# olydis/vlg_matching

Hardware: AMD Instinct MI355X
Metric: vlg_queries_per_sec (higher is better)
Workload: dtype u32

## Files before the change

### vlg_matching_amd/csrc/int_index.hpp

```cpp
#pragma once
#include "extract.hpp"
#include "select.hpp"
#include "sweep_kernels.hpp"

namespace {

void bind_int_view(vlg_index* idx)
{
    const uint8_t* b = reinterpret_cast<const uint8_t*>(idx->d_blob);
    const IntHeader& h = idx->ihdr;
    IntView& v = idx->iview;
    v.bv_kind = (uint32_t)h.bv_kind; v.sampling = (uint32_t)h.sampling;
    v.blocks = h.bv_kind == kBvPlain ? reinterpret_cast<const Block*>(b + h.off_levels) : nullptr;
    v.rrr_hdr = h.bv_kind == kBvRrr63 ? reinterpret_cast<const uint4*>(b + h.off_rrr_hdr) : nullptr;
    v.rrr_stream = h.bv_kind == kBvRrr63 ? reinterpret_cast<const uint64_t*>(b + h.off_rrr_stream) : nullptr;
    v.rrr_tables = h.bv_kind == kBvRrr63 ? reinterpret_cast<const RrrTables*>(b + h.off_binom) : nullptr;
    v.stride = h.bv_kind == kBvRrr63 ? h.n_sb : h.nb;
    v.Z = reinterpret_cast<const uint64_t*>(b + h.off_Z);
    v.D = reinterpret_cast<const uint64_t*>(b + h.off_D);
    v.C = reinterpret_cast<const uint64_t*>(b + h.off_C);
    v.comp2char = reinterpret_cast<const uint32_t*>(b + h.off_c2c);
    v.samples = reinterpret_cast<const uint32_t*>(b + h.off_samples);
    v.n = h.n; v.nb = h.nb; v.sigma = h.sigma; v.n_samples = h.n_samples; v.n_levels = h.levels; v.dens = h.dens;
    v.marked = h.sampling == kSamplingTextOrder ? reinterpret_cast<const Block*>(b + h.off_marked) : nullptr;
// ... 336 lines not shown

namespace {

vlg_status int_alloc_blob(vlg_index* idx, uint64_t n, uint64_t sigma, uint32_t dens)
{
    IntHeader& h = idx->ihdr;
    memset(&h, 0, sizeof h);
    h.magic = kIntBlobMagic; h.n = n; h.sigma = sigma; h.dens = dens; h.n_samples = (n + dens - 1) / dens; h.nb = n / kBlockBits + 1;
    h.levels = sigma > 1 ? bit_width64(sigma - 1) : 0;
    if (h.levels > kMaxIntLevels || (uint64_t)h.levels * h.nb >= 0xFFFFFFF0ull) return fail(VLG_E_UNSUPPORTED, "integer index too large for 32-bit block numbers");
    layout_int(h);
    DevBuf blob;
    VLG_HIP_TRY(blob.alloc(h.total_bytes));
    idx->d_blob = blob.take();
    idx->owns_blob = true;
    VLG_HIP_TRY(hipMemset(idx->d_blob, 0, h.total_bytes));
    VLG_HIP_TRY(hipMemcpy(idx->d_blob, &h, sizeof h, hipMemcpyHostToDevice));
    bind_int_view(idx);
    return VLG_OK;
}

vlg_status int_matrix_from_bwt(vlg_index* idx, uint32_t* d_cur, uint32_t* d_other, uint32_t* d_ka, uint32_t* d_kb, DevBuf& tmp)
{
    const IntHeader& h = idx->ihdr;
    const uint64_t n = h.n;
    uint8_t* b = reinterpret_cast<uint8_t*>(idx->d_blob);
    Block* lv = reinterpret_cast<Block*>(b + h.off_levels);
    uint64_t* d_Z = reinterpret_cast<uint64_t*>(b + h.off_Z);
    std::vector<uint64_t> Z(kMaxIntLevels, 0);
    uint32_t* cur = d_cur;
    uint32_t* other = d_other;
    DevBuf d_pops;
    VLG_HIP_TRY(d_pops.alloc((h.nb + 1) * 4));
    for (uint32_t l = 0; l < h.levels; ++l) {
        const uint32_t bit = h.levels - 1 - l;
        if (vlg_status s = wtsa_emit_level(cur, n, bit, lv + (uint64_t)l * h.nb, h.nb, d_pops.as<uint32_t>(), tmp)) return s;
        uint32_t ones = 0;
        VLG_HIP_TRY(hipMemcpy(&ones, d_pops.as<uint32_t>() + h.nb, 4, hipMemcpyDeviceToHost));
        Z[l] = n - ones;
        if (l + 1 < h.levels) {
            hipLaunchKernelGGL(int_bit_keys_kernel, launch_grid(n), dim3(256), 0, nullptr, cur, n, bit, d_ka);
            VLG_HIP_TRY(with_scratch(tmp, [&](void* t, size_t& tb) { return rocprim::radix_sort_pairs(t, tb, d_ka, d_kb, cur, other, n, 0, 1, nullptr); }));
            std::swap(cur, other);
        }
        VLG_HIP_TRY(hipGetLastError());
    }
    VLG_HIP_TRY(hipMemcpy(d_Z, Z.data(), kMaxIntLevels * 8, hipMemcpyHostToDevice));
    hipLaunchKernelGGL(int_D_kernel, launch_grid(h.sigma), dim3(256), 0, nullptr, idx->iview, reinterpret_cast<uint64_t*>(b + h.off_D));
    VLG_HIP_TRY(hipGetLastError());
    VLG_HIP_TRY(hipDeviceSynchronize());
    return VLG_OK;
}

}

extern "C" vlg_status vlg_index_build_int(const uint32_t* h_text, uint64_t n_symbols, uint32_t dens, vlg_index** out)
{
    if (!out || (n_symbols && !h_text)) return fail(VLG_E_INVALID, "null argument");
    *out = nullptr;
    int ndev = 0;
    if (hipGetDeviceCount(&ndev) != hipSuccess || ndev <= 0) return fail(VLG_E_NO_DEVICE, "no HIP device available (the VLG library has no CPU fallback)");
    if (!dens) dens = 32;
    if (n_symbols * 5 >= 0xFFFFFFF0ull) return fail(VLG_E_UNSUPPORTED, "integer text too long for the 32-bit suffix array of this index");
    release_cached_device_memory();
    const uint64_t n = n_symbols + 1;
    IndexPtr idx(new vlg_index());
    DevBuf text, flag, sa, arr_a, arr_b, ka, kb, tmp;
    VLG_HIP_TRY(text.alloc(n_symbols * 4));
    uint32_t* d_text = text.as<uint32_t>();
    if (n_symbols) VLG_HIP_TRY(hipMemcpy(d_text, h_text, n_symbols * 4, hipMemcpyHostToDevice));
    VLG_HIP_TRY(flag.alloc((n_symbols * 5 + 2) * 4));
    VLG_HIP_TRY(hipMemset(flag.p, 0, 4));
    if (n_symbols) hipLaunchKernelGGL(int_zero_check_kernel, launch_grid(n_symbols), dim3(256), 0, nullptr, d_text, n_symbols, flag.as<uint32_t>());
    uint32_t has_zero = 0;
    VLG_HIP_TRY(hipMemcpy(&has_zero, flag.p, 4, hipMemcpyDeviceToHost));
    if (has_zero) return fail(VLG_E_ZERO_BYTE, "the integer text contains the symbol 0 (reserved for the sentinel: construct.hpp:36-45)");
    if (vlg_status s = symbol_suffix_array(d_text, n_symbols, flag, sa)) return s;
    flag.release();
    uint32_t* d_sa = sa.as<uint32_t>();
    VLG_HIP_TRY(arr_a.alloc(n * 4));
    VLG_HIP_TRY(arr_b.alloc(n * 4));
    VLG_HIP_TRY(ka.alloc(n * 4));
    VLG_HIP_TRY(kb.alloc(n * 4));
    uint32_t *d_a = arr_a.as<uint32_t>(), *d_b = arr_b.as<uint32_t>(), *d_ka = ka.as<uint32_t>(), *d_kb = kb.as<uint32_t>();
    size_t sort_tb = 0, scan_tb = 0, pair_tb = 0;
    VLG_HIP_TRY(rocprim::radix_sort_keys(nullptr, sort_tb, d_a, d_b, n, 0, 32, nullptr));
    VLG_HIP_TRY(rocprim::inclusive_scan(nullptr, scan_tb, d_ka, d_kb, n, rocprim::plus<uint32_t>(), nullptr));
    VLG_HIP_TRY(rocprim::radix_sort_pairs(nullptr, pair_tb, d_ka, d_kb, d_a, d_b, n, 0, 1, nullptr));
    VLG_HIP_TRY(tmp.alloc(std::max(std::max(sort_tb, scan_tb), pair_tb)));
    uint64_t sigma = 1;
    if (n_symbols) {
        VLG_HIP_TRY(with_scratch(tmp, [&](void* t, size_t& tb) { return rocprim::radix_sort_keys(t, tb, d_text, d_b, n_symbols, 0, 32, nullptr); }));
        hipLaunchKernelGGL(int_heads_kernel, launch_grid(n_symbols), dim3(256), 0, nullptr, d_b, n_symbols, d_ka);
        VLG_HIP_TRY(with_scratch(tmp, [&](void* t, size_t& tb) { return rocprim::inclusive_scan(t, tb, d_ka, d_kb, n_symbols, rocprim::plus<uint32_t>(), nullptr); }));
        uint32_t distinct = 0;
        VLG_HIP_TRY(hipMemcpy(&distinct, d_kb + (n_symbols - 1), 4, hipMemcpyDeviceToHost));
        sigma = (uint64_t)distinct + 1;
    }
    if (vlg_status s = int_alloc_blob(idx.get(), n, sigma, dens)) return s;
    const IntHeader& h = idx->ihdr;
    uint8_t* b = reinterpret_cast<uint8_t*>(idx->d_blob);
    uint32_t* d_c2c = reinterpret_cast<uint32_t*>(b + h.off_c2c);
    uint64_t* d_C = reinterpret_cast<uint64_t*>(b + h.off_C);
    if (n_symbols) hipLaunchKernelGGL(int_alphabet_kernel, launch_grid(n_symbols), dim3(256), 0, nullptr, d_b, d_kb, n_symbols, d_c2c, d_C);
    VLG_HIP_TRY(hipMemcpy(d_C + sigma, &n, 8, hipMemcpyHostToDevice));
    hipLaunchKernelGGL(int_bwt_kernel, launch_grid(n), dim3(256), 0, nullptr, d_text, d_sa, n, d_c2c, sigma, d_a);
    VLG_HIP_TRY(hipGetLastError());
    if (vlg_status s = int_matrix_from_bwt(idx.get(), d_a, d_b, d_ka, d_kb, tmp)) return s;
    hipLaunchKernelGGL(int_samples_kernel, launch_grid(h.n_samples), dim3(256), 0, nullptr, d_sa, h.n_samples, dens, reinterpret_cast<uint32_t*>(b + h.off_samples));
    VLG_HIP_TRY(hipGetLastError());
    VLG_HIP_TRY(hipDeviceSynchronize());
    *out = idx.release();
    return VLG_OK;
}

extern "C" vlg_status vlg_index_export_int_alphabet(const vlg_index* idx, uint64_t* sigma, uint64_t* h_C, uint64_t* h_comp2char)
{
    if (!idx || !sigma) return fail(VLG_E_INVALID, "null argument");
    if (!idx->is_int) return fail(VLG_E_INVALID, "not an integer-alphabet index");
    *sigma = idx->ihdr.sigma;
    if (h_C) VLG_HIP_TRY(hipMemcpy(h_C, idx->iview.C, (idx->ihdr.sigma + 1) * 8, hipMemcpyDeviceToHost));
    if (h_comp2char) {
        std::vector<uint32_t> t(idx->ihdr.sigma);
        VLG_HIP_TRY(hipMemcpy(t.data(), idx->iview.comp2char, idx->ihdr.sigma * 4, hipMemcpyDeviceToHost));
        for (uint64_t i = 0; i < idx->ihdr.sigma; ++i) h_comp2char[i] = t[i];
    }
    return VLG_OK;
}

extern "C" vlg_status vlg_int_rank_batch(const vlg_index* idx, const uint64_t* d_i, const uint32_t* d_sym, uint64_t* d_out, uint64_t count, void* stream)
{
    if (!idx || (count && (!d_i || !d_sym || !d_out))) return fail(VLG_E_INVALID, "null argument");
    if (!idx->is_int) return fail(VLG_E_INVALID, "not an integer-alphabet index");
    if (!count) return VLG_OK;
    return on_bv(idx->iview.bv_kind, [&](auto bv) {
        return launch(int_rank_kernel<tag_t<decltype(bv)>>, launch_grid(count, 8192), (hipStream_t)stream, idx->iview, d_i, d_sym, d_out, count);
    });
}

namespace vlg {

vlg_status launch_int_backward_search(const IntView& v, const uint8_t* d_blob, const uint64_t* d_off, uint64_t n_pat, uint64_t* d_l, uint64_t* d_r,
                                      unsigned long long* d_stat_levels, hipStream_t st)
{
    if (!n_pat) return VLG_OK;
    return on_bv(v.bv_kind, [&](auto bv) {
        return launch(int_backward_search_kernel<tag_t<decltype(bv)>>, launch_grid(n_pat, 4096), st, v, d_blob, d_off, n_pat, d_l, d_r, d_stat_levels);
    });
}

vlg_status launch_int_locate_sweep(const IntView& v, const uint64_t* d_l, const uint64_t* d_out_off, uint64_t n_pat, uint64_t total, uint32_t* d_out,
                                   uint64_t* val_a, uint64_t* val_b, uint16_t* key_a, uint16_t* key_b, void* temp, size_t temp_bytes, unsigned long long* d_counter,
                                   unsigned long long* d_stats, uint64_t tail_threshold, hipStream_t stream, LaunchTimer* timer, Block* member,
                                   uint32_t n_member_lists, uint64_t* rec, const std::function<vlg_status()>* while_first_step)
{
    const bool text_order = shape(v).text_order;
    if (v.dens == 1 && !text_order && total)
        return sweep_dense_copy(timer, while_first_step, [&] { return launch_int_dense_copy(v, d_l, d_out_off, n_pat, total, d_out, stream); });
    if (!int_sweep_possible(v)) return fail(VLG_E_INTERNAL, "integer index: not for the sorted sweep");
    return on_bv(v.bv_kind, [&](auto bv) { return on_flag(text_order, [&](auto to) {
        const SweepKernels K = bind_sweep<IntWalk<tag_t<decltype(bv)>>, IntSampling<decltype(to)::value>, uint32_t, false>(v, d_l, d_out_off, n_pat, d_stats, stream, nullptr);
        return run_locate_sweep<uint32_t, false>(K, d_l, d_out_off, n_pat, total, d_out, val_a, val_b, key_a, key_b, temp, temp_bytes, d_counter, tail_threshold, stream, timer,
                                                 member, n_member_lists, rec, while_first_step);
    }); });
}

vlg_status launch_int_dense_copy(const IntView& v, const uint64_t* d_l, const uint64_t* d_out_off, uint64_t n_pat, uint64_t total, uint32_t* d_out, hipStream_t stream)
{
    if (v.dens != 1 || v.sampling != kSamplingSaOrder) return fail(VLG_E_INTERNAL, "integer index: the copy needs SA-order samples of density 1");
    return launch_sa_dense_copy(v.samples, d_l, d_out_off, n_pat, total, d_out, stream);
}

vlg_status launch_int_locate(const IntView& v, uint32_t* d_io, uint64_t total, unsigned long long* d_stats, hipStream_t st)
{
    if (!total) return VLG_OK;
    const LocateSlices sl = locate_slices(total);
    return on_bv(v.bv_kind, [&](auto bv) { return on_flag(shape(v).text_order, [&](auto to) {
        return launch(locate_kernel<IntWalk<tag_t<decltype(bv)>>, IntSampling<decltype(to)::value>, uint32_t>, dim3(sl.blocks), st, v, d_io, total, sl.per_wave, d_stats,
                      nullptr, 0u, nullptr, 0ull, nullptr);
    }); });
}

vlg_status launch_int_sa_expand(const IntView& v, uint32_t* d_sa, hipStream_t st)
{
    if (v.sampling != kSamplingSaOrder) return fail(VLG_E_INTERNAL, "integer index: expanding the suffix array needs SA-order samples");
    return on_bv(v.bv_kind, [&](auto bv) { return launch(int_sa_expand_kernel<tag_t<decltype(bv)>>, launch_grid(v.n_samples, 8192), st, v, d_sa); });
}

vlg_status launch_int_isa_samples(const IntView& v, uint32_t inv_dens, uint32_t* d_out, hipStream_t st)
{
    if (v.sampling != kSamplingSaOrder || !inv_dens) return fail(VLG_E_INTERNAL, "integer index: ISA samples need SA-order samples");
    return on_bv(v.bv_kind, [&](auto bv) { return launch(int_isa_samples_kernel<tag_t<decltype(bv)>>, launch_grid(v.n_samples, 8192), st, v, inv_dens, d_out); });
}

vlg_status launch_int_select(const IntView& v, const SelView& sv, const uint64_t* d_arg, const uint32_t* d_sym, uint64_t* d_out, uint64_t count, hipStream_t st)
{
    if (!count) return VLG_OK;
    return on_bv(v.bv_kind, [&](auto bv) { return launch(int_select_kernel<tag_t<decltype(bv)>>, launch_grid(count, 8192), st, v, sv, d_arg, d_sym, d_out, count); });
}
vlg_status launch_int_lf_bwt(const IntView& v, const uint64_t* d_i, uint64_t* d_lf, uint32_t* d_bwt, uint64_t count, hipStream_t st)
{
    if (!count) return VLG_OK;
    return on_bv(v.bv_kind, [&](auto bv) { return launch(int_lf_bwt_kernel<tag_t<decltype(bv)>>, launch_grid(count, 8192), st, v, d_i, d_lf, d_bwt, count); });
}
vlg_status launch_int_extract(const IntView& v, const ExtractJob& job, const uint32_t* d_isa, uint32_t* d_out, hipStream_t st)
{
    return on_bv(v.bv_kind, [&](auto bv) { return launch(int_extract_kernel<tag_t<decltype(bv)>>, launch_grid(job.n_segs, 8192), st, v, job, d_isa, d_out); });
}

vlg_status launch_int_isa(const IntView& v, uint32_t d, const uint32_t* d_isa, const uint64_t* d_i, uint64_t* d_out, uint64_t count,
                          unsigned long long* d_bad, hipStream_t st)
{
    return on_bv(v.bv_kind, [&](auto bv) { return launch(int_isa_kernel<tag_t<decltype(bv)>>, launch_grid(count, 8192), st, v, d, d_isa, d_i, d_out, count, d_bad); });
}

}

namespace {

inline uint32_t int_max_level(uint64_t largest) { return (uint32_t)bit_width64(std::max<uint64_t>(largest, 1)); }

struct TreeScratch {
    DevBuf tree, pay[2], first[2], split, end, pops, bad, tmp;
    uint64_t words = 0, max_nw = 0;
    vlg_status alloc(uint64_t n, uint64_t sigma, uint32_t L)
    {
        words = (n * L + 63) / 64;
        max_nw = n / 64 + 2;
        VLG_HIP_TRY(tree.alloc((words + 1) * 8));
        for (int k = 0; k < 2; ++k) {
            VLG_HIP_TRY(pay[k].alloc(n * 4));
            VLG_HIP_TRY(first[k].alloc(n * 4));
        }
        VLG_HIP_TRY(split.alloc((sigma + 1) * 4));
        VLG_HIP_TRY(end.alloc((sigma + 1) * 4));
        VLG_HIP_TRY(pops.alloc((max_nw + 1) * 4));
        VLG_HIP_TRY(bad.alloc(4));
        VLG_HIP_TRY(hipMemset(bad.p, 0, 4));
        size_t tb = 0;
        VLG_HIP_TRY(rocprim::exclusive_scan(nullptr, tb, pops.as<uint32_t>(), pops.as<uint32_t>(), 0u, max_nw, rocprim::plus<uint32_t>(), nullptr));
        VLG_HIP_TRY(tmp.alloc(tb));
        return VLG_OK;
    }
    vlg_status scan_pops(uint64_t nw)
    {
        uint32_t* p = pops.as<uint32_t>();
        VLG_HIP_TRY(with_scratch(tmp, [&](void* t, size_t& tb) { return rocprim::exclusive_scan(t, tb, p, p, 0u, nw, rocprim::plus<uint32_t>(), nullptr); }));
        return VLG_OK;
    }
};

inline void tree_level_words(uint64_t n, uint32_t l, uint64_t& base, uint64_t& g0, uint64_t& nw)
{
    base = (uint64_t)l * n;
    g0 = base >> 6;
    nw = ((base + n - 1) >> 6) - g0 + 1;
}

vlg_status int_tree_encode(TreeScratch& s, uint64_t n, uint64_t sigma, uint32_t L, const uint32_t* d_c2c, const uint64_t* d_C)
{
    uint64_t* tree = s.tree.as<uint64_t>();
    uint32_t *pops = s.pops.as<uint32_t>(), *split = s.split.as<uint32_t>(), *end = s.end.as<uint32_t>(), *bad_flag = s.bad.as<uint32_t>();
    VLG_HIP_TRY(hipMemset(tree, 0, (s.words + 1) * 8));
    VLG_HIP_TRY(hipMemset(s.first[0].p, 0, n * 4));
    int cur = 0;
    for (uint32_t l = 0; l < L; ++l) {
        uint64_t base, g0, nw;
        tree_level_words(n, l, base, g0, nw);
        hipLaunchKernelGGL(int_tree_emit_kernel, launch_grid(nw * 64), dim3(256), 0, nullptr, s.pay[cur].as<uint32_t>(), d_c2c, base, n, L - 1 - l, g0, nw, tree, pops);
        if (l + 1 == L) break;
        if (vlg_status st = s.scan_pops(nw)) return st;
        hipLaunchKernelGGL(int_tree_split_kernel, launch_grid(sigma + 1), dim3(256), 0, nullptr, d_c2c, sigma, L - l, split, end);
        hipLaunchKernelGGL(HIP_KERNEL_NAME(int_tree_step_kernel<false>), launch_grid(n), dim3(256), 0, nullptr, tree, pops, base, g0, n, d_C, split, end,
                           s.pay[cur].as<uint32_t>(), s.first[cur].as<uint32_t>(), s.pay[cur ^ 1].as<uint32_t>(), s.first[cur ^ 1].as<uint32_t>(), bad_flag);
        VLG_HIP_TRY(hipGetLastError());
        cur ^= 1;
    }
    VLG_HIP_TRY(hipGetLastError());
    uint32_t bad = 0;
    VLG_HIP_TRY(hipMemcpy(&bad, bad_flag, 4, hipMemcpyDeviceToHost));
    if (bad) return fail(VLG_E_INTERNAL, "integer index: the level-wise tree does not agree with the alphabet");
    return VLG_OK;
}

vlg_status int_tree_decode(TreeScratch& s, uint64_t n, uint64_t sigma, uint32_t L, const uint32_t* d_c2c, const uint64_t* d_C, int* bwt)
{
    const uint64_t* tree = s.tree.as<uint64_t>();
    uint32_t *pops = s.pops.as<uint32_t>(), *split = s.split.as<uint32_t>(), *end = s.end.as<uint32_t>(), *bad_flag = s.bad.as<uint32_t>();
    hipLaunchKernelGGL(int_iota_kernel, launch_grid(n), dim3(256), 0, nullptr, s.pay[0].as<uint32_t>(), n);
    VLG_HIP_TRY(hipMemset(s.first[0].p, 0, n * 4));
    int cur = 0;
    for (uint32_t l = 0; l < L; ++l) {
        uint64_t base, g0, nw;
        tree_level_words(n, l, base, g0, nw);
        hipLaunchKernelGGL(int_tree_pops_kernel, launch_grid(nw), dim3(256), 0, nullptr, tree, g0, nw, pops);
        if (vlg_status st = s.scan_pops(nw)) return st;
        hipLaunchKernelGGL(int_tree_split_kernel, launch_grid(sigma + 1), dim3(256), 0, nullptr, d_c2c, sigma, L - l, split, end);
        if (l + 1 < L)
            hipLaunchKernelGGL(HIP_KERNEL_NAME(int_tree_step_kernel<false>), launch_grid(n), dim3(256), 0, nullptr, tree, pops, base, g0, n, d_C, split, end,
                               s.pay[cur].as<uint32_t>(), s.first[cur].as<uint32_t>(), s.pay[cur ^ 1].as<uint32_t>(), s.first[cur ^ 1].as<uint32_t>(), bad_flag);
        else
            hipLaunchKernelGGL(HIP_KERNEL_NAME(int_tree_step_kernel<true>), launch_grid(n), dim3(256), 0, nullptr, tree, pops, base, g0, n, d_C, split, end,
                               s.pay[cur].as<uint32_t>(), s.first[cur].as<uint32_t>(), s.pay[cur ^ 1].as<uint32_t>(), (uint32_t*)nullptr, bad_flag);
        VLG_HIP_TRY(hipGetLastError());
        uint32_t bad = 0;
        VLG_HIP_TRY(hipMemcpy(&bad, bad_flag, 4, hipMemcpyDeviceToHost));
        if (bad) return fail(VLG_E_INVALID, "wt_int tree does not agree with the alphabet's C (level " + std::to_string(l) + ")");
        cur ^= 1;
    }
    *bwt = cur;
    return VLG_OK;
}

}

extern "C" vlg_status vlg_index_export_int_tree(const vlg_index* idx, uint32_t* max_level, uint64_t* h_words)
// ... 68 lines not shown
```

### vlg_matching_amd/csrc/kernels.hip

```cpp
#include <algorithm>
#include <cstring>
#include <string.h>
#include <vector>
#include "common.hpp"
#include "kernels.hpp"
#include "sweep_kernels.hpp"
#include "extract.hpp"
#include "select.hpp"
#include <rocprim/rocprim.hpp>

using namespace vlg;

struct vlg_bitvector {
    Block* d_blocks = nullptr;
    uint64_t nbits = 0;
    uint64_t n_blocks = 0;
};

namespace {

__global__ void bv_pack_kernel(const uint64_t* __restrict__ src, uint64_t src_words, uint64_t nbits, Block* __restrict__ blocks,
                               uint64_t n_blocks, uint32_t* __restrict__ pops)
{
    for (uint64_t b = (uint64_t)blockIdx.x * blockDim.x + threadIdx.x; b < n_blocks; b += (uint64_t)gridDim.x * blockDim.x) {
// ... 825 lines not shown
}

template <class BV, typename pos_t, typename out_t>
__global__ void __launch_bounds__(256) isa_samples_kernel(IndexView iv, uint32_t inv_dens, out_t* __restrict__ out)
{
    __shared__ WalkLds<BV> s;
    stage_walk(s, iv);
    const ByteWalk<BV, true> walk{iv, s};
    const pos_t* samples = reinterpret_cast<const pos_t*>(iv.samples);
    for (uint64_t j = (uint64_t)blockIdx.x * blockDim.x + threadIdx.x; j < iv.n_samples; j += (uint64_t)gridDim.x * blockDim.x) {
        uint64_t i = j * iv.dens, v = samples[j];
        do {
            if (v % inv_dens == 0) out[v / inv_dens] = (out_t)i;
            uint32_t c, n_lv = 0;
            i = walk.lf(i, c, n_lv);
            v = v ? v - 1 : iv.n - 1;
        } while (i % iv.dens);
    }
}

template <class BV, bool kWide, typename isa_t>
__global__ void __launch_bounds__(256) extract_kernel(IndexView iv, ExtractJob job, const isa_t* __restrict__ isa, const uint8_t* __restrict__ comp2char,
                                                      uint8_t* __restrict__ out)
{
    __shared__ WalkLds<BV> s;
    __shared__ uint8_t c2c[256];
    c2c[threadIdx.x] = comp2char[threadIdx.x];
    stage_walk(s, iv);
    extract_segments(job, isa, out, ByteWalk<BV, kWide>{iv, s, c2c});
}

template <class BV, bool kWide, typename isa_t>
__global__ void __launch_bounds__(256) isa_kernel(IndexView iv, uint32_t d, const isa_t* __restrict__ isa, const uint64_t* __restrict__ p,
                                                  uint64_t* __restrict__ out, uint64_t count, unsigned long long* __restrict__ bad)
{
    __shared__ WalkLds<BV> s;
    stage_walk(s, iv);
    isa_queries(p, out, count, iv.n, d, isa, ByteWalk<BV, kWide>{iv, s}, bad);
}

__global__ void comp2char_kernel(const uint8_t* __restrict__ char2comp, uint8_t* __restrict__ c2c)
{
    const uint32_t ch = threadIdx.x, c = char2comp[ch];
    if (ch == 0 || c != 0) c2c[c] = (uint8_t)ch;
}

__global__ void extract_check_kernel(const uint64_t* __restrict__ begin, const uint64_t* __restrict__ end, const uint64_t* __restrict__ out_off,
                                     uint64_t n_ranges, uint64_t n, uint64_t total, uint32_t d, uint64_t* __restrict__ seg,
                                     unsigned long long* __restrict__ bad)
{
    for (uint64_t r = (uint64_t)blockIdx.x * blockDim.x + threadIdx.x; r <= n_ranges; r += (uint64_t)gridDim.x * blockDim.x) {
        if (r == n_ranges) { seg[r] = 0; continue; }
        const uint64_t b = begin[r], e = end[r], o = out_off[r];
        const bool ok = b <= e && e < n && o <= total && e - b + 1 <= total - o;
        seg[r] = ok ? e / d - b / d + 1 : 0;
        if (!ok) atomicAdd(bad, 1ull);
    }
}

template <typename pos_t>
__global__ void widen_kernel(const pos_t* __restrict__ in, uint64_t* __restrict__ out, uint64_t count)
{
    for (uint64_t j = (uint64_t)blockIdx.x * blockDim.x + threadIdx.x; j < count; j += (uint64_t)gridDim.x * blockDim.x) out[j] = in[j];
}
template <typename pos_t>
__global__ void narrow_kernel(const uint64_t* __restrict__ in, pos_t* __restrict__ out, uint64_t count)
{
    for (uint64_t j = (uint64_t)blockIdx.x * blockDim.x + threadIdx.x; j < count; j += (uint64_t)gridDim.x * blockDim.x) out[j] = (pos_t)in[j];
}

template <bool kWide, bool kTextOrder>
using ByteSampling = typename std::conditional<kTextOrder, TextOrderSampling<typename std::conditional<kWide, uint64_t, uint32_t>::type>,
                                               SaOrderSampling<typename std::conditional<kWide, uint64_t, uint32_t>::type>>::type;

}

namespace vlg {

vlg_status launch_backward_search(const IndexView& iv, const uint8_t* d_blob, const uint64_t* d_off, uint64_t n_pat, uint64_t* d_l,
                                  uint64_t* d_r, unsigned long long* d_stat_levels, hipStream_t stream)
{
    if (!n_pat) return VLG_OK;
    return on_bv(iv.bv_kind, [&](auto bv) {
        return launch(backward_search_kernel<tag_t<decltype(bv)>>, launch_grid(n_pat, 4096), stream, iv, d_blob, d_off, n_pat, d_l, d_r, d_stat_levels);
    });
}

vlg_status launch_branching_search(const IndexView& iv, bool budget, const uint8_t* d_masks, const uint64_t* d_task, uint64_t n_tasks, uint32_t cap,
                                   uint64_t* d_frontier, uint32_t* d_count, unsigned long long* d_stat_levels, hipStream_t stream)
{
    if (!n_tasks) return VLG_OK;
    if (!cap || cap > kClassIntervalsMax) return fail(VLG_E_INTERNAL, std::string(budget ? "approximate" : "class") + " search: frontier cap out of range");
    const dim3 grid((uint32_t)std::min<uint64_t>((n_tasks + 3) / 4, 16384));
    return on_bv(iv.bv_kind, [&](auto bv) {
        const auto go = [&](auto kernel) {
            return launch(kernel, grid, stream, iv, d_masks, d_task, n_tasks, cap, reinterpret_cast<ulonglong2*>(d_frontier), d_count, d_stat_levels);
        };
        return budget ? go(branching_search_kernel<tag_t<decltype(bv)>, true>) : go(branching_search_kernel<tag_t<decltype(bv)>, false>);
    });
}

template <typename pos_t>
vlg_status launch_expand(const uint64_t* d_l, const uint64_t* d_out_off, uint64_t n_pat, uint64_t total, pos_t* d_io, uint32_t* d_seg,
                         hipStream_t stream)
{
    if (!total) return VLG_OK;
    hipLaunchKernelGGL(HIP_KERNEL_NAME(expand_kernel<pos_t>), launch_grid(total, 32768), dim3(256), 0, stream, d_l, d_out_off, n_pat,
                       total, d_io, d_seg);
    VLG_HIP_TRY(hipGetLastError());
    return VLG_OK;
}
template vlg_status launch_expand<uint32_t>(const uint64_t*, const uint64_t*, uint64_t, uint64_t, uint32_t*, uint32_t*, hipStream_t);
template vlg_status launch_expand<uint64_t>(const uint64_t*, const uint64_t*, uint64_t, uint64_t, uint64_t*, uint32_t*, hipStream_t);

template <typename pos_t>
vlg_status launch_locate(const IndexView& iv, pos_t* d_io, uint64_t total, unsigned long long* d_stats, hipStream_t stream)
{
    if (!total) return VLG_OK;
    const LocateSlices sl = locate_slices(total);
    if (iv.sample_bytes != sizeof(pos_t)) return fail(VLG_E_INTERNAL, "locate: sample width does not match the instantiation");
    constexpr bool kWide = sizeof(pos_t) == 8;
    return on_byte_walk<kWide>(iv, [&](auto walk) { return on_flag(shape(iv).text_order, [&](auto to) {
        return launch(locate_kernel<tag_t<decltype(walk)>, ByteSampling<kWide, decltype(to)::value>, pos_t, false, kWide>, dim3(sl.blocks), stream, iv, d_io,
                      total, sl.per_wave, d_stats, nullptr, 0u, nullptr, 0ull, nullptr);
    }); });
}
template vlg_status launch_locate<uint32_t>(const IndexView&, uint32_t*, uint64_t, unsigned long long*, hipStream_t);
template vlg_status launch_locate<uint64_t>(const IndexView&, uint64_t*, uint64_t, unsigned long long*, hipStream_t);


size_t sweep_temp_bytes(uint64_t total, uint32_t sigma, hipStream_t stream)
{
    size_t tb = 0;
    rocprim::double_buffer<uint16_t> k(nullptr, nullptr);
    rocprim::double_buffer<uint64_t> v(nullptr, nullptr);
    (void)rocprim::radix_sort_pairs(nullptr, tb, k, v, total, 0, bit_width64(sigma), stream);
    return tb;
}

void launch_sweep_chunk_lists(const uint64_t* d_out_off, uint64_t n_pat, uint64_t t0, uint64_t t1, uint32_t* chunk_list, hipStream_t stream)
{
    const uint64_t chunks = (t1 - t0 + kSweepChunk - 1) / kSweepChunk;
    if (!chunks) return;
    hipLaunchKernelGGL(sweep_chunk_lists_kernel, dim3((uint32_t)((chunks + 255) / 256)), dim3(256), 0, stream, d_out_off, n_pat, t0, t1, chunk_list);
}

template <typename pos_t, bool kWide>
vlg_status run_locate_sweep(const SweepKernels& K, const uint64_t* d_l, const uint64_t* d_out_off, uint64_t n_pat, uint64_t total,
                            pos_t* d_out, uint64_t* val_a, uint64_t* val_b, uint16_t* key_a, uint16_t* key_b, void* temp,
                            size_t temp_bytes, unsigned long long* d_counter, uint64_t tail_threshold,
                            hipStream_t stream, LaunchTimer* timer, Block* member ,
                            uint32_t n_member_lists ,
                            uint64_t* rec ,
                            const std::function<vlg_status()>* while_first_step )
{
    bool hook_due = while_first_step != nullptr;
    constexpr uint32_t kShift = kWide ? 33 : 32;
    if (K.n > (1ull << kShift)) return fail(VLG_E_UNSUPPORTED, "sorted sweep: text too long for the packed position");
    if (sizeof(pos_t) == 4 && K.n > (1ull << 32) + 1) return fail(VLG_E_INTERNAL, "sorted sweep: positions do not fit 32 bits");
    if (K.sigma >= 0xFFFFu) return fail(VLG_E_INTERNAL, "sorted sweep: alphabet too large for the 16-bit partition key");
    const unsigned bits = bit_width64(K.sigma);
    const uint64_t batch_max = sweep_batch_max<kWide>();
    if (member) {
        if (total > 0xFFFFFF00ull) return fail(VLG_E_INTERNAL, "member bit-vector: slots need 32 bits");
        if (timer) timer->begin(0);
        hipLaunchKernelGGL(member_build_kernel, launch_grid(member_blocks(K.n), 16384), dim3(256), 0, stream, d_l, d_out_off, n_member_lists,
                           member_blocks(K.n), member);
        if (timer) timer->end(0);
        VLG_HIP_TRY(hipGetLastError());
        if (total > batch_max) VLG_HIP_TRY(hipMemsetAsync(rec, 0xFF, total * 8, stream));
    }
    bool front_valid = K.front != nullptr && [] { const char* e = getenv("VLG_RESOLVE_GROUPED"); return !(e && e[0] == '0'); }();
    for (uint64_t t0 = 0; t0 < total; t0 += batch_max) {
        const uint64_t t1 = std::min(total, t0 + batch_max);
        const bool fused_first = t1 - t0 > tail_threshold;
        if (!fused_first) front_valid = false;
        static const bool ahead = [] { const char* e = getenv("VLG_SWEEP_LOOKAHEAD"); return !(e && e[0] == '0'); }();
        if (!fused_first) {
            if (member) VLG_HIP_TRY(hipMemsetAsync(rec + t0, 0xFF, (t1 - t0) * 8, stream));
            hipLaunchKernelGGL(HIP_KERNEL_NAME(sweep_init_kernel<kShift>), launch_grid((t1 - t0 + 7) / 8, 32768), dim3(256), 0, stream, d_l, d_out_off, n_pat,
                               t0, t1, val_a);
        }
        VLG_HIP_TRY(hipGetLastError());
        uint64_t alive = t1 - t0;
        uint32_t step = 0;
        pos_t* out = d_out + t0;
        while (alive > tail_threshold && step < 0xFFFFFFu) {
            VLG_HIP_TRY(hipMemsetAsync(d_counter, 0, 8, stream));
            if (timer) timer->begin(0);
            const vlg_status ks = fused_first && step == 0 ? K.first(t0, t1, val_a, key_a, out, d_counter, member, rec, ahead, reinterpret_cast<uint32_t*>(val_b))
                                                           : K.step(val_a, key_a, alive, step, out, d_counter, member, rec, t0, ahead && fused_first && step == 1);
            if (timer) timer->end(0);
            if (ks) return ks;
            size_t tb = temp_bytes;
            if (timer) timer->begin(1, 20ull * alive);
            rocprim::double_buffer<uint16_t> dk(key_a, key_b);
            rocprim::double_buffer<uint64_t> dv(val_a, val_b);
            hipError_t se = rocprim::radix_sort_pairs(temp, tb, dk, dv, alive, 0, bits, stream);
            if (timer) timer->end(1);
            VLG_HIP_TRY(se);
            unsigned long long done = 0;
            VLG_HIP_TRY(hipMemcpyAsync(&done, d_counter, 8, hipMemcpyDeviceToHost, stream));
            if (hook_due) { hook_due = false; if (vlg_status hs = (*while_first_step)()) return hs; }
            VLG_HIP_TRY(hipStreamSynchronize(stream));
            key_a = dk.current(); key_b = dk.alternate();
            val_a = dv.current(); val_b = dv.alternate();
            alive -= done;
            ++step;
            if (step > 1u << 20) return fail(VLG_E_INTERNAL, "locate sweep did not converge");
        }
        if (alive) {
            const LocateSlices sl = locate_slices(alive);
            if (timer) timer->begin(0);
            const vlg_status ks = K.tail(out, alive, sl.per_wave, val_a, step, member ? rec : nullptr, t0, member, sl.blocks);
            if (timer) timer->end(0);
            if (ks) return ks;
        }
    }
    if (hook_due) { hook_due = false; if (vlg_status hs = (*while_first_step)()) return hs; }
    if (member) {
        static const bool diag = [] { const char* e = getenv("VLG_RESOLVE_STATS"); return e && e[0] == '1'; }();
        for (uint32_t round = 0;; ++round) {
            VLG_HIP_TRY(hipMemsetAsync(d_counter, 0, diag ? 32 : 8, stream));
            if (timer) timer->begin(2, round == 0 ? total * (8ull + sizeof(pos_t)) : 0);
            if (round == 0 && front_valid && !diag)
                hipLaunchKernelGGL(HIP_KERNEL_NAME(trail_resolve_grouped_kernel<pos_t, kWide>), dim3((uint32_t)std::min<uint64_t>((total + kGroupChunk - 1) / kGroupChunk, 1u << 20)),
                                   dim3(256), 0, stream, rec, total, d_out, K.front, d_counter);
            else
                hipLaunchKernelGGL(HIP_KERNEL_NAME(trail_resolve_kernel<pos_t, kWide>), dim3((uint32_t)std::min<uint64_t>((total + kResolveChunk - 1) / kResolveChunk, 65536)),
                                   dim3(256), 0, stream, rec, total, d_out, d_counter, round, diag);
            if (timer) timer->end(2);
            VLG_HIP_TRY(hipGetLastError());
            unsigned long long open = 0;
            VLG_HIP_TRY(hipMemcpyAsync(&open, d_counter, 8, hipMemcpyDeviceToHost, stream));
            VLG_HIP_TRY(hipStreamSynchronize(stream));
            if (diag) {
                unsigned long long c[4] = {0, 0, 0, 0};
                VLG_HIP_TRY(hipMemcpy(c, d_counter, 32, hipMemcpyDeviceToHost));
                fprintf(stderr, "[vlg resolve] round %u: %llu records, %llu pointers, %llu hops, %llu distinct lines (per wave-wide hop), %llu still open\n", round,
                        (unsigned long long)total, c[3], c[1], c[2], c[0]);
            }
            if (!open) break;
            if (round > 64) return fail(VLG_E_INTERNAL, "trail records did not resolve");
        }
    }
    return VLG_OK;
}
template vlg_status run_locate_sweep<uint32_t, false>(const SweepKernels&, const uint64_t*, const uint64_t*, uint64_t, uint64_t, uint32_t*, uint64_t*, uint64_t*,
                                                      uint16_t*, uint16_t*, void*, size_t, unsigned long long*, uint64_t, hipStream_t, LaunchTimer*, Block*,
                                                      uint32_t, uint64_t*, const std::function<vlg_status()>*);

template <typename pos_t, bool kWide>
vlg_status launch_locate_sweep(const IndexView& iv, const uint64_t* d_l, const uint64_t* d_out_off, uint64_t n_pat, uint64_t total,
                               pos_t* d_out, uint64_t* val_a, uint64_t* val_b, uint16_t* key_a, uint16_t* key_b, void* temp,
                               size_t temp_bytes, unsigned long long* d_counter, unsigned long long* d_stats, uint64_t tail_threshold,
                               hipStream_t stream, LaunchTimer* timer, Block* member, uint32_t n_member_lists, uint64_t* rec,
                               const std::function<vlg_status()>* while_first_step, uint8_t* front)
{
    if (iv.sample_bytes != (kWide ? 8u : 4u)) return fail(VLG_E_INTERNAL, "sorted sweep: sample width does not match the instantiation");
    const bool text_order = shape(iv).text_order;
    if (iv.dens == 1 && !text_order && total) {
        using sample_t = typename std::conditional<kWide, uint64_t, uint32_t>::type;
        return sweep_dense_copy(timer, while_first_step, [&] {
            return launch(sa_dense_copy_kernel<pos_t, sample_t>, launch_grid((total + 7) / 8, 32768), stream, reinterpret_cast<const sample_t*>(iv.samples), d_l, d_out_off,
                          n_pat, total, d_out);
        });
    }
    return on_byte_walk<kWide>(iv, [&](auto walk) { return on_flag(text_order, [&](auto to) {
        const SweepKernels K = bind_sweep<tag_t<decltype(walk)>, ByteSampling<kWide, decltype(to)::value>, pos_t, kWide>(iv, d_l, d_out_off, n_pat, d_stats, stream,
                                                                                                                   rec ? front : nullptr);
        return run_locate_sweep<pos_t, kWide>(K, d_l, d_out_off, n_pat, total, d_out, val_a, val_b, key_a, key_b, temp, temp_bytes, d_counter, tail_threshold, stream, timer,
                                              member, n_member_lists, rec, while_first_step);
    }); });
}
constexpr uint32_t kUnsampleSync = 4;
template <bool kWide>
vlg_status launch_unsample(const IndexView& iv, const uint64_t* d_l, const uint64_t* d_out_off, uint64_t n_pat, uint64_t total, uint32_t* d_out,
                           uint32_t* sa_full, uint64_t* val_a, uint64_t* val_b, uint16_t* key_a, uint16_t* key_b, void* temp, size_t temp_bytes,
                           unsigned long long* d_counter, unsigned long long* h_done , unsigned long long* d_stats, uint64_t tail_threshold,
                           hipStream_t stream, LaunchTimer* timer, const std::function<vlg_status()>* while_first_step)
{
    bool hook_due = while_first_step != nullptr;
    if (iv.sampling != kSamplingSaOrder || iv.dens < 2) return fail(VLG_E_INTERNAL, "unsampling needs SA-order samples of density >= 2");
    if (iv.sample_bytes != (kWide ? 8u : 4u)) return fail(VLG_E_INTERNAL, "unsampling: sample width does not match the instantiation");
    if (iv.n > (1ull << 32) + 1 || (!kWide && iv.n > (1ull << 32))) return fail(VLG_E_UNSUPPORTED, "unsampling: text too long for 32-bit positions");
    if (iv.sigma >= 0x7FFFu) return fail(VLG_E_INTERNAL, "unsampling: alphabet too large for the key");
    const unsigned bits = bit_width64(iv.sigma);
    uint64_t alive = iv.n_samples, done_total = 0;
    const auto step_round = [&](bool first) {
        if (timer) timer->begin(0);
        const vlg_status ks = on_bv(iv.bv_kind, [&](auto bv) { return on_flag(first, [&](auto f) {
            return launch(unsample_step_kernel<tag_t<decltype(bv)>, kWide, decltype(f)::value>, launch_grid(alive, 8192), stream, iv, val_a, key_a, alive, sa_full, d_stats,
                          d_counter);
        }); });
        if (timer) timer->end(0);
        return ks;
    };
    VLG_HIP_TRY(hipMemsetAsync(d_counter, 0, 8, stream));
    uint32_t round = 0;
    while (alive > tail_threshold) {
        for (uint32_t r = 0; r < kUnsampleSync; ++r, ++round) {
            if (vlg_status ks = step_round(round == 0)) return ks;
            size_t tb = temp_bytes;
            if (timer) timer->begin(1, 20ull * alive);
            rocprim::double_buffer<uint16_t> dk(key_a, key_b);
            rocprim::double_buffer<uint64_t> dv(val_a, val_b);
            const hipError_t se = rocprim::radix_sort_pairs(temp, tb, dk, dv, alive, 0, bits, stream);
            if (timer) timer->end(1);
            VLG_HIP_TRY(se);
            key_a = dk.current(); key_b = dk.alternate();
            val_a = dv.current(); val_b = dv.alternate();
            if (hook_due) { hook_due = false; if (vlg_status hs = (*while_first_step)()) return hs; }
        }
        VLG_HIP_TRY(hipMemcpyAsync(h_done, d_counter, 8, hipMemcpyDeviceToHost, stream));
        VLG_HIP_TRY(hipStreamSynchronize(stream));
        done_total = *h_done;
        if (done_total > iv.n_samples) return fail(VLG_E_INTERNAL, "unsampling: more walkers arrived than were started");
        alive = iv.n_samples - done_total;
        if (round > (1u << 20)) return fail(VLG_E_INTERNAL, "unsampling did not converge");
    }
    if (round == 0 && iv.n_samples) {
        if (vlg_status ks = step_round(true)) return ks;
        ++round;
    }
    if (hook_due) { hook_due = false; if (vlg_status hs = (*while_first_step)()) return hs; }
    if (alive || round == 1) {
        const uint64_t span = round == 1 ? iv.n_samples : alive;
        const LocateSlices sl = locate_slices(span, 64 * 4);
        if (timer) timer->begin(0);
        const vlg_status ks = on_bv(iv.bv_kind, [&](auto bv) {
            return launch(unsample_tail_kernel<tag_t<decltype(bv)>, kWide>, dim3(sl.blocks), stream, iv, val_a, key_a, span, sl.per_wave, sa_full, d_stats);
        });
        if (timer) timer->end(0);
        if (ks) return ks;
    }
    if (total) {
        if (timer) timer->begin(0);
        const vlg_status ks = launch_sa_dense_copy(sa_full, d_l, d_out_off, n_pat, total, d_out, stream);
        if (timer) timer->end(0);
        if (ks) return ks;
    }
    return VLG_OK;
}
template vlg_status launch_unsample<false>(const IndexView&, const uint64_t*, const uint64_t*, uint64_t, uint64_t, uint32_t*, uint32_t*, uint64_t*, uint64_t*,
                                           uint16_t*, uint16_t*, void*, size_t, unsigned long long*, unsigned long long*, unsigned long long*, uint64_t, hipStream_t,
                                           LaunchTimer*, const std::function<vlg_status()>*);
template vlg_status launch_unsample<true>(const IndexView&, const uint64_t*, const uint64_t*, uint64_t, uint64_t, uint32_t*, uint32_t*, uint64_t*, uint64_t*,
                                          uint16_t*, uint16_t*, void*, size_t, unsigned long long*, unsigned long long*, unsigned long long*, uint64_t, hipStream_t,
                                          LaunchTimer*, const std::function<vlg_status()>*);

vlg_status launch_sa_dense_copy(const uint32_t* sa, const uint64_t* d_l, const uint64_t* d_out_off, uint64_t n_pat, uint64_t total, uint32_t* d_out,
                                hipStream_t stream)
{
    if (!total) return VLG_OK;
    return launch(sa_dense_copy_kernel<uint32_t, uint32_t>, launch_grid((total + 7) / 8, 32768), stream, sa, d_l, d_out_off, n_pat, total, d_out);
}

#define VLG_SWEEP_INST(P, W)                                                                                                          \
    template vlg_status launch_locate_sweep<P, W>(const IndexView&, const uint64_t*, const uint64_t*, uint64_t, uint64_t, P*, uint64_t*, \
                                                  uint64_t*, uint16_t*, uint16_t*, void*, size_t, unsigned long long*, unsigned long long*, \
                                                  uint64_t, hipStream_t, LaunchTimer*, Block*, uint32_t, uint64_t*,                       \
                                                  const std::function<vlg_status()>*, uint8_t*);
VLG_SWEEP_INST(uint32_t, false)
VLG_SWEEP_INST(uint32_t, true)
VLG_SWEEP_INST(uint64_t, true)
#undef VLG_SWEEP_INST

template <typename T>
vlg_status launch_narrow(const uint64_t* d_in, T* d_out, uint64_t count, hipStream_t stream)
{
    if (!count) return VLG_OK;
    return launch(narrow_kernel<T>, launch_grid(count), stream, d_in, d_out, count);
}
template vlg_status launch_narrow<uint32_t>(const uint64_t*, uint32_t*, uint64_t, hipStream_t);
template <typename T>
vlg_status launch_widen(const T* d_in, uint64_t* d_out, uint64_t count, hipStream_t stream)
{
    if (!count) return VLG_OK;
    return launch(widen_kernel<T>, launch_grid(count), stream, d_in, d_out, count);
}
template vlg_status launch_widen<uint32_t>(const uint32_t*, uint64_t*, uint64_t, hipStream_t);

KernelConstants kernel_constants()
{
    return KernelConstants{VLG_RESOLVE_HOPS, VLG_RESOLVE_CHUNK, VLG_GROUP_CHUNK, VLG_STAGE_LISTS, VLG_SWEEP_PAIRS};
}

}

extern "C" vlg_status vlg_wt_rank_batch(const vlg_index* idx, const uint64_t* d_i, const uint8_t* d_c, uint64_t* d_out, uint64_t count,
                                        void* stream)
{
    if (!idx || (count && (!d_i || !d_c || !d_out))) return fail(VLG_E_INVALID, "null argument");
    if (idx->is_int) return fail(VLG_E_INVALID, "integer-alphabet index: use vlg_int_rank_batch");
    if (!count) return VLG_OK;
    return on_bv(idx->view.bv_kind, [&](auto bv) {
        return launch(wt_rank_kernel<tag_t<decltype(bv)>>, launch_grid(count, 8192), (hipStream_t)stream, idx->view, d_i, d_c, d_out, count);
    });
}

extern "C" vlg_status vlg_backward_search_batch(const vlg_index* idx, const uint8_t* d_blob, const uint64_t* d_off, uint64_t n_patterns,
                                                uint64_t* d_l, uint64_t* d_r, void* stream)
{
    if (!idx || (n_patterns && (!d_off || !d_l || !d_r))) return fail(VLG_E_INVALID, "null argument");
    if (idx->is_int) return launch_int_backward_search(idx->iview, d_blob, d_off, n_patterns, d_l, d_r, nullptr, (hipStream_t)stream);
    return launch_backward_search(idx->view, d_blob, d_off, n_patterns, d_l, d_r, nullptr, (hipStream_t)stream);
}

namespace {
template <class Fill>
vlg_status locate_narrow(const vlg_index* idx, uint64_t count, uint64_t* d_out, hipStream_t st, const Fill& fill)
{
    DevBuf tmp_buf;
    VLG_HIP_TRY(tmp_buf.alloc(count * 4));
    uint32_t* tmp = tmp_buf.as<uint32_t>();
    vlg_status s = fill(tmp);
    if (!s) s = idx->is_int ? launch_int_locate(idx->iview, tmp, count, nullptr, st) : launch_locate<uint32_t>(idx->view, tmp, count, nullptr, st);
    if (!s) s = launch_widen<uint32_t>(tmp, d_out, count, st);
    const hipError_t e = hipStreamSynchronize(st);
    if (s) return s;
    VLG_HIP_TRY(e);
    return VLG_OK;
}
}

extern "C" vlg_status vlg_sa_batch(const vlg_index* idx, const uint64_t* d_i, uint64_t* d_out, uint64_t count, void* stream)
{
    if (!idx || (count && (!d_i || !d_out))) return fail(VLG_E_INVALID, "null argument");
    if (!count) return VLG_OK;
    hipStream_t st = (hipStream_t)stream;
    if (idx->hdr.sample_bytes == 8) {
        if (d_out != d_i) VLG_HIP_TRY(hipMemcpyAsync(d_out, d_i, count * 8, hipMemcpyDeviceToDevice, st));
        return launch_locate<uint64_t>(idx->view, d_out, count, nullptr, st);
    }
    return locate_narrow(idx, count, d_out, st, [&](uint32_t* tmp) { return launch_narrow<uint32_t>(d_i, tmp, count, st); });
}

extern "C" vlg_status vlg_locate_batch(const vlg_index* idx, const uint64_t* d_l, const uint64_t* d_r, const uint64_t* d_out_off,
                                       uint64_t n_patterns, uint64_t total, uint64_t* d_out, void* stream)
{
    (void)d_r;
    if (!idx || (n_patterns && (!d_l || !d_out_off)) || (total && !d_out)) return fail(VLG_E_INVALID, "null argument");
    if (!total) return VLG_OK;
    hipStream_t st = (hipStream_t)stream;
    if (idx->hdr.sample_bytes == 8) {
        if (vlg_status s = launch_expand<uint64_t>(d_l, d_out_off, n_patterns, total, d_out, nullptr, st)) return s;
        return launch_locate<uint64_t>(idx->view, d_out, total, nullptr, st);
    }
    return locate_narrow(idx, total, d_out, st, [&](uint32_t* tmp) { return launch_expand<uint32_t>(d_l, d_out_off, n_patterns, total, tmp, nullptr, st); });
}

namespace {
vlg_status isa_samples_device(const vlg_index* idx, uint32_t inv_dens, void* d_out, hipStream_t st)
{
    const uint64_t n = idx->hdr.n;
    if (idx->hdr.sampling != kSamplingSaOrder) return fail(VLG_E_UNSUPPORTED, "ISA samples are computed from an SA-order index");
    const uint64_t count = (n - 1) / inv_dens + 1;
    const uint32_t w = isa_sample_bytes(n);
    VLG_HIP_TRY(hipMemsetAsync(d_out, 0, count * w, st));
    if (idx->is_int)
        return launch_int_isa_samples(idx->iview, inv_dens, (uint32_t*)d_out, st);
    const IndexView& iv = idx->view;
    return on_bv(iv.bv_kind, [&](auto bv) { return on_isa_samples_shape(shape(iv).wide, w, [&](auto pos, auto out) {
        using out_t = tag_t<decltype(out)>;
        return launch(isa_samples_kernel<tag_t<decltype(bv)>, tag_t<decltype(pos)>, out_t>, launch_grid(iv.n_samples, 8192), st, iv, inv_dens, (out_t*)d_out);
    }); });
}
}

extern "C" vlg_status vlg_index_isa_samples(const vlg_index* idx, uint32_t inv_dens, uint64_t* h_out, uint64_t count)
{
    if (!idx || !h_out || !inv_dens) return fail(VLG_E_INVALID, "null argument");
    const uint64_t n = idx->hdr.n;
    if (count != (n - 1) / inv_dens + 1) return fail(VLG_E_INVALID, "ISA sample count must be (n-1)/inv_dens + 1");
    if (idx->hdr.sampling != kSamplingSaOrder) return fail(VLG_E_UNSUPPORTED, "ISA samples are computed from an SA-order index");
    const uint32_t w = isa_sample_bytes(n);
    DevBuf out_buf;
    VLG_HIP_TRY(out_buf.alloc(count * (8 + w)));
    uint64_t* d_out = out_buf.as<uint64_t>();
    void* d_smp = d_out + count;
    vlg_status s = isa_samples_device(idx, inv_dens, d_smp, nullptr);
    if (!s) s = w == 8 ? (hipMemcpyAsync(d_out, d_smp, count * 8, hipMemcpyDeviceToDevice, nullptr) == hipSuccess ? VLG_OK : VLG_E_NO_DEVICE)
                       : launch_widen<uint32_t>((const uint32_t*)d_smp, d_out, count, nullptr);
    hipError_t e = s ? hipSuccess : hipMemcpy(h_out, d_out, count * 8, hipMemcpyDeviceToHost);
    if (s) return s == VLG_E_NO_DEVICE ? fail(s, "ISA samples: device copy failed") : s;
    VLG_HIP_TRY(e);
    return VLG_OK;
}

extern "C" vlg_status vlg_text_access_create(const vlg_index* idx, uint32_t inv_dens, void* stream, vlg_text_access** out)
{
    if (!idx || !out) return fail(VLG_E_INVALID, "null argument");
    *out = nullptr;
    if (idx->hdr.sampling != kSamplingSaOrder)
        return fail(VLG_E_UNSUPPORTED, "text access needs an SA-order index (a text-order index derives its ISA through the marks)");
    const uint32_t d = inv_dens ? inv_dens : 64;
    hipStream_t st = (hipStream_t)stream;
    vlg_text_access* t = new (std::nothrow) vlg_text_access;
    if (!t) return fail(VLG_E_OOM, "text access handle");
    t->idx = idx;
    t->d = d;
    t->isa_bytes = isa_sample_bytes(idx->hdr.n);
    const uint64_t count = (idx->hdr.n - 1) / d + 1;
    vlg_status s = VLG_OK;
    if (hipMalloc(&t->d_isa, count * t->isa_bytes) != hipSuccess) { t->d_isa = nullptr; s = fail(VLG_E_OOM, "text access: ISA samples"); }
    if (!s) s = isa_samples_device(idx, d, t->d_isa, st);
    if (!s && !idx->is_int) {
        if (hipMalloc((void**)&t->d_c2c, 256) != hipSuccess) { t->d_c2c = nullptr; s = fail(VLG_E_OOM, "text access: comp2char"); }
        else if (hipMemsetAsync(t->d_c2c, 0, 256, st) != hipSuccess) s = fail(VLG_E_NO_DEVICE, "text access: comp2char");
        else hipLaunchKernelGGL(comp2char_kernel, dim3(1), dim3(256), 0, st, idx->view.char2comp, t->d_c2c);
    }
    if (!s) {
        hipError_t e = hipGetLastError();
        if (e == hipSuccess) e = hipStreamSynchronize(st);
        if (e != hipSuccess) s = fail(VLG_E_NO_DEVICE, std::string("text access: ") + hipGetErrorString(e));
    }
    if (s) { vlg_text_access_destroy(t); return s; }
    *out = t;
    return VLG_OK;
}

extern "C" void vlg_text_access_destroy(vlg_text_access* t)
{
    if (!t) return;
    if (t->d_isa) (void)hipFree(t->d_isa);
    if (t->d_c2c) (void)hipFree(t->d_c2c);
    delete t;
}

extern "C" vlg_status vlg_extract_batch(const vlg_text_access* t, const uint64_t* d_begin, const uint64_t* d_end, const uint64_t* d_out_off,
                                        uint64_t n_ranges, uint64_t total, void* d_out, void* stream)
{
    if (!t || (n_ranges && (!d_begin || !d_end || !d_out_off || !d_out))) return fail(VLG_E_INVALID, "null argument");
    if (!n_ranges) return VLG_OK;
    const vlg_index* idx = t->idx;
    hipStream_t st = (hipStream_t)stream;
    size_t tb = 0;
    uint64_t* seg = nullptr;
// ... 478 lines not shown
```

### vlg_matching_amd/csrc/kernels.hpp

```cpp
#pragma once
#include <algorithm>
#include <functional>
#include "common.hpp"

namespace vlg {

vlg_status launch_backward_search(const IndexView& iv, const uint8_t* d_blob, const uint64_t* d_off, uint64_t n_pat, uint64_t* d_l,
                                  uint64_t* d_r, unsigned long long* d_stat_levels, hipStream_t stream);
constexpr uint32_t kClassIntervalsMax = 1u << 20;
constexpr uint32_t kClassSearchOverflow = 0xFFFFFFFFu;
vlg_status launch_branching_search(const IndexView& iv, bool budget, const uint8_t* d_masks, const uint64_t* d_task, uint64_t n_tasks, uint32_t cap,
                                   uint64_t* d_frontier, uint32_t* d_count, unsigned long long* d_stat_levels, hipStream_t stream);
template <typename pos_t>
vlg_status launch_expand(const uint64_t* d_l, const uint64_t* d_out_off, uint64_t n_pat, uint64_t total, pos_t* d_io, uint32_t* d_seg,
                         hipStream_t stream);
template <typename pos_t>
vlg_status launch_locate(const IndexView& iv, pos_t* d_io, uint64_t total, unsigned long long* d_stats, hipStream_t stream);

struct KernelConstants { int64_t resolve_hops, resolve_chunk, group_chunk, stage_lists, sweep_pairs; };
KernelConstants kernel_constants();

struct LaunchTimer {
    virtual ~LaunchTimer() {}
    virtual void begin(int which, uint64_t algorithmic_bytes = 0) = 0;
    virtual void end(int which) = 0;
};

struct LocateSlices { uint32_t per_wave, blocks; };
inline LocateSlices locate_slices(uint64_t count, uint64_t min_per_wave = 64 * 16)
{
    const uint64_t target_waves = 256ull * 32 * 4;
    const uint64_t per_wave = std::min<uint64_t>(std::max<uint64_t>((count + target_waves - 1) / target_waves, min_per_wave), 1u << 20);
    const uint64_t waves = (count + per_wave - 1) / per_wave;
    return LocateSlices{(uint32_t)per_wave, (uint32_t)((waves + 3) / 4)};
}

size_t sweep_temp_bytes(uint64_t total, uint32_t sigma, hipStream_t stream);
template <bool kWide> constexpr uint64_t sweep_batch_max() { return kWide ? (1ull << 31) : 0xFFFFFF00ull; }
template <typename pos_t, bool kWide>
vlg_status launch_locate_sweep(const IndexView& iv, const uint64_t* d_l, const uint64_t* d_out_off, uint64_t n_pat, uint64_t total,
                               pos_t* d_out, uint64_t* val_a, uint64_t* val_b, uint16_t* key_a, uint16_t* key_b, void* temp,
                               size_t temp_bytes, unsigned long long* d_counter, unsigned long long* d_stats, uint64_t tail_threshold,
                               hipStream_t stream, LaunchTimer* timer, Block* member, uint32_t n_member_lists, uint64_t* rec,
                               const std::function<vlg_status()>* while_first_step = nullptr,
                               uint8_t* front = nullptr );
constexpr uint32_t kSweepChunk = 2048;
void launch_sweep_chunk_lists(const uint64_t* d_out_off, uint64_t n_pat, uint64_t t0, uint64_t t1, uint32_t* chunk_list, hipStream_t stream);
struct SweepKernels {
    uint8_t* front = nullptr;
    uint64_t n = 0;
    uint32_t sigma = 0;
    std::function<vlg_status(uint64_t t0, uint64_t t1, uint64_t* val, uint16_t* key, void* out, unsigned long long* n_done, const Block* member, uint64_t* rec, bool ahead,
                       uint32_t* chunk_list )> first;
    std::function<vlg_status(uint64_t* val, uint16_t* key, uint64_t alive, uint32_t step, void* out, unsigned long long* n_done, const Block* member, uint64_t* rec, uint64_t t0,
                       bool probed)> step;
    std::function<vlg_status(void* out, uint64_t alive, uint32_t per_wave, const uint64_t* val, uint32_t step, uint64_t* rec_or_null, uint64_t t0, const Block* member,
                       uint32_t blocks)> tail;
};
template <typename pos_t, bool kWide>
vlg_status run_locate_sweep(const SweepKernels& K, const uint64_t* d_l, const uint64_t* d_out_off, uint64_t n_pat, uint64_t total,
                            pos_t* d_out, uint64_t* val_a, uint64_t* val_b, uint16_t* key_a, uint16_t* key_b, void* temp,
                            size_t temp_bytes, unsigned long long* d_counter, uint64_t tail_threshold, hipStream_t stream, LaunchTimer* timer,
                            Block* member, uint32_t n_member_lists, uint64_t* rec, const std::function<vlg_status()>* while_first_step = nullptr);
inline uint64_t member_blocks(uint64_t n) { return n / kBlockBits + 1; }
template <bool kWide>
vlg_status launch_unsample(const IndexView& iv, const uint64_t* d_l, const uint64_t* d_out_off, uint64_t n_pat, uint64_t total, uint32_t* d_out,
                           uint32_t* sa_full, uint64_t* val_a, uint64_t* val_b, uint16_t* key_a, uint16_t* key_b, void* temp, size_t temp_bytes,
                           unsigned long long* d_counter, unsigned long long* h_done , unsigned long long* d_stats, uint64_t tail_threshold,
                           hipStream_t stream, LaunchTimer* timer, const std::function<vlg_status()>* while_first_step = nullptr);
template <typename T> vlg_status launch_narrow(const uint64_t* d_in, T* d_out, uint64_t count, hipStream_t stream);
template <typename T> vlg_status launch_widen(const T* d_in, uint64_t* d_out, uint64_t count, hipStream_t stream);

vlg_status launch_int_backward_search(const IntView& v, const uint8_t* d_blob, const uint64_t* d_off, uint64_t n_pat, uint64_t* d_l, uint64_t* d_r,
                                      unsigned long long* d_stat_levels, hipStream_t st);
vlg_status launch_int_locate(const IntView& v, uint32_t* d_io, uint64_t total, unsigned long long* d_stats, hipStream_t st);
vlg_status launch_int_locate_sweep(const IntView& v, const uint64_t* d_l, const uint64_t* d_out_off, uint64_t n_pat, uint64_t total, uint32_t* d_out,
                                   uint64_t* val_a, uint64_t* val_b, uint16_t* key_a, uint16_t* key_b, void* temp, size_t temp_bytes, unsigned long long* d_counter,
                                   unsigned long long* d_stats, uint64_t tail_threshold, hipStream_t stream, LaunchTimer* timer, Block* member,
                                   uint32_t n_member_lists, uint64_t* rec, const std::function<vlg_status()>* while_first_step = nullptr);
vlg_status launch_sa_dense_copy(const uint32_t* sa, const uint64_t* d_l, const uint64_t* d_out_off, uint64_t n_pat, uint64_t total, uint32_t* d_out,
                                hipStream_t stream);
vlg_status launch_int_dense_copy(const IntView& v, const uint64_t* d_l, const uint64_t* d_out_off, uint64_t n_pat, uint64_t total, uint32_t* d_out, hipStream_t stream);
vlg_status launch_int_sa_expand(const IntView& v, uint32_t* d_sa, hipStream_t st);
vlg_status launch_int_isa_samples(const IntView& v, uint32_t inv_dens, uint32_t* d_out, hipStream_t st);
struct ExtractJob;
vlg_status launch_int_extract(const IntView& v, const ExtractJob& job, const uint32_t* d_isa, uint32_t* d_out, hipStream_t st);
vlg_status launch_int_isa(const IntView& v, uint32_t d, const uint32_t* d_isa, const uint64_t* d_i, uint64_t* d_out, uint64_t count,
                          unsigned long long* d_bad, hipStream_t st);
struct SelView;
vlg_status launch_int_select(const IntView& v, const SelView& sv, const uint64_t* d_arg, const uint32_t* d_sym, uint64_t* d_out, uint64_t count, hipStream_t st);
vlg_status launch_int_lf_bwt(const IntView& v, const uint64_t* d_i, uint64_t* d_lf, uint32_t* d_bwt, uint64_t count, hipStream_t st);
inline bool int_sweep_possible(const IntView& v) { return v.sigma < 0xFFFFu && v.n_levels >= 1 && v.n <= (1ull << 32); }

}
```

### vlg_matching_amd/csrc/search.hip

```cpp
#include <algorithm>
#include <chrono>
#include <cstdio>
#include <cstdlib>
#include <cstring>
#include <mutex>
#include <numeric>
#include <thread>
#include <unordered_map>
#include <string.h>
#include <string>
#include <vector>
#include "common.hpp"
#include "kernels.hpp"
#include <rocprim/rocprim.hpp>

using namespace vlg;

#include "search_types.hpp"
#include "filter_shape.hpp"
#include "window_cut.hpp"
#include "shape_dispatch.hpp"

enum { KS_BSEARCH = 0, KS_EXPAND, KS_LOCATE, KS_LOCATE_PART, KS_LOCATE_RESOLVE, KS_SORT, KS_FILTER_LADDER, KS_FILTER_PIVOT, KS_FILTER_PASS, KS_FILTER_COMPACT,
       KS_JOIN_INIT, KS_JOIN_LINK, KS_JOIN_SCAN, KS_JOIN_CHAIN, KS_GATHER, KS_EXCHANGE, KS_WINDOW_CUT, KS_CLASS_SEARCH, KS_COUNT };
static const char* kKernelNames[KS_COUNT] = {"backward_search", "expand", "locate", "locate_partition", "locate_resolve", "sort", "filter_ladder", "filter_pivot",
                                             "filter_pass", "filter_compact", "join_init", "join_link", "join_scan", "join_chain", "gather", "exchange", "window_cut", "class_search"};

struct vlg_workspace {
    hipStream_t stream = nullptr;
    uint64_t cap_bytes = 0;
    uint8_t* arena = nullptr;
    uint64_t arena_bytes = 0;
    HostPool host;
    bool profile = false;
    bool dedup = true;
    bool sweep = true;
    bool tuples = true;
    bool trail = true;
    bool filter = true;
    uint64_t filter_min = 1ull << 12;
    uint64_t filter_stream_min = 1ull << 16;
    bool filter_pivot = true;
    uint64_t filter_group_bytes = 0;
    uint64_t filter_pivot_ratio = 3;
    uint64_t pivot_range_ratio = 16;
    uint32_t compact_dense_min = 256;
    uint32_t pivot_rungs = 1;
    int list_sort = 1;
    uint64_t global_sort_min = 1ull << 20;
    bool quad_walk = true;
    bool fuse_jump = true;
    uint64_t sweep_min = 1ull << 22;
    uint64_t sweep_tail = 1ull << 22;
    uint32_t unsample_pct = 0;
    uint64_t unsample_min = 1ull << 28;
    uint64_t unsample_tail = 1ull << 20;
    uint32_t class_intervals = 1024;
    uint64_t sample_reads = 0;
    uint8_t* head = nullptr;
    uint64_t head_bytes = 0;
    uint64_t tmp_key[6] = {0, 0, 0, 0, 0, 0};
    size_t tmp_bytes = 0;
    int x_ranks = 1, x_rank = 0;
    vlg_exchange_fn x_fn = nullptr;
    vlg_alltoall_fn x_a2a = nullptr;
    void* x_ctx = nullptr;
    void* x_comm = nullptr;
    bool exchange_all = false;
    uint64_t* x_status = nullptr;
    uint32_t x_agreed = 0;
    vlg_kernel_stat stats[KS_COUNT];
    std::vector<std::pair<hipEvent_t, hipEvent_t>> pending[KS_COUNT];
    std::vector<hipEvent_t> free_events;
};

namespace {

struct PhaseTrace {
    bool on, sync;
    hipStream_t st;
    std::chrono::steady_clock::time_point t0;
    explicit PhaseTrace(hipStream_t s) : on(getenv("VLG_TRACE") != nullptr), sync(!on || strcmp(getenv("VLG_TRACE"), "host") != 0), st(s), t0(std::chrono::steady_clock::now()) {}
    void mark(const char* what)
    {
        if (!on) return;
        if (sync) (void)hipStreamSynchronize(st);
        const auto t1 = std::chrono::steady_clock::now();
        fprintf(stderr, "[vlg trace] %-28s %9.3f ms\n", what, std::chrono::duration<double, std::milli>(t1 - t0).count());
        t0 = t1;
    }
};

hipEvent_t ws_event(vlg_workspace* ws)
{
    if (!ws->free_events.empty()) { hipEvent_t e = ws->free_events.back(); ws->free_events.pop_back(); return e; }
    hipEvent_t e;
    if (hipEventCreate(&e) != hipSuccess) return nullptr;
    return e;
}

struct Timed {
    vlg_workspace* ws; int k; hipEvent_t a = nullptr, b = nullptr;
    Timed(vlg_workspace* w, int kernel, uint64_t alg_bytes) : ws(w), k(kernel)
    {
        ws->stats[k].launches++;
        ws->stats[k].algorithmic_bytes += alg_bytes;
        if (ws->profile) { a = ws_event(ws); b = ws_event(ws); if (a) (void)hipEventRecord(a, ws->stream); }
    }
    ~Timed() { if (a && b) { (void)hipEventRecord(b, ws->stream); ws->pending[k].emplace_back(a, b); } }
};

struct SweepTimer : LaunchTimer {
    vlg_workspace* ws; hipEvent_t a = nullptr, b = nullptr;
    explicit SweepTimer(vlg_workspace* w) : ws(w) {}
    void begin(int which, uint64_t algorithmic_bytes) override
    {
        int k = which == 0 ? KS_LOCATE : (which == 1 ? KS_LOCATE_PART : KS_LOCATE_RESOLVE);
        ws->stats[k].launches++;
        ws->stats[k].algorithmic_bytes += algorithmic_bytes;
        a = b = nullptr;
        if (ws->profile) { a = ws_event(ws); b = ws_event(ws); if (a) (void)hipEventRecord(a, ws->stream); }
    }
    void end(int which) override
    {
        int k = which == 0 ? KS_LOCATE : (which == 1 ? KS_LOCATE_PART : KS_LOCATE_RESOLVE);
        if (a && b) { (void)hipEventRecord(b, ws->stream); ws->pending[k].emplace_back(a, b); }
    }
};

void ws_collect(vlg_workspace* ws)
{
    for (int k = 0; k < KS_COUNT; ++k) {
        for (auto& pr : ws->pending[k]) {
            float ms = 0;
            (void)hipEventSynchronize(pr.second);
            if (hipEventElapsedTime(&ms, pr.first, pr.second) == hipSuccess) ws->stats[k].total_ms += ms;
            ws->free_events.push_back(pr.first);
            ws->free_events.push_back(pr.second);
        }
        ws->pending[k].clear();
    }
}

void ws_reset_stats(vlg_workspace* ws)
{
    ws_collect(ws);
    for (int k = 0; k < KS_COUNT; ++k) {
        memset(&ws->stats[k], 0, sizeof(vlg_kernel_stat));
        strncpy(ws->stats[k].name, kKernelNames[k], sizeof(ws->stats[k].name) - 1);
    }
}

void drain_result_cache();

vlg_status ws_head(vlg_workspace* ws, uint64_t bytes, uint8_t** out)
{
    if (bytes > ws->head_bytes) {
        if (ws->head) { (void)hipFree(ws->head); ws->head = nullptr; ws->head_bytes = 0; }
        const uint64_t want = align_up(bytes + bytes / 4, 1 << 20);
        VLG_HIP_TRY(hipMalloc((void**)&ws->head, want));
        ws->head_bytes = want;
    }
    *out = ws->head;
    return VLG_OK;
}

vlg_status ws_reserve(vlg_workspace* ws, uint64_t bytes)
{
    if (bytes <= ws->arena_bytes) return VLG_OK;
    if (ws->arena) { (void)hipFree(ws->arena); ws->arena = nullptr; ws->arena_bytes = 0; }
    if (hipMalloc((void**)&ws->arena, bytes) != hipSuccess) {
        (void)hipGetLastError();
        ws->arena = nullptr;
        drain_result_cache();
        VLG_HIP_TRY(hipMalloc((void**)&ws->arena, bytes));
    }
    ws->arena_bytes = bytes;
    return VLG_OK;
}

}

extern "C" vlg_status vlg_workspace_create(uint64_t max_hbm_bytes, void* stream, vlg_workspace** out)
{
    if (!out) return fail(VLG_E_INVALID, "null argument");
    *out = nullptr;
    int ndev = 0;
    if (hipGetDeviceCount(&ndev) != hipSuccess || ndev <= 0) return fail(VLG_E_NO_DEVICE, "no HIP device available");
    vlg_workspace* ws = new vlg_workspace();
    ws->stream = (hipStream_t)stream;
    ws->cap_bytes = max_hbm_bytes ? max_hbm_bytes : (8ull << 30);
    ws_reset_stats(ws);
    *out = ws;
    return VLG_OK;
}

extern "C" void vlg_workspace_destroy(vlg_workspace* ws)
{
    if (!ws) return;
    ws_collect(ws);
    for (hipEvent_t e : ws->free_events) (void)hipEventDestroy(e);
    if (ws->arena) (void)hipFree(ws->arena);
    if (ws->head) (void)hipFree(ws->head);
    if (ws->x_status) (void)hipFree(ws->x_status);
    ws->host.release();
    delete ws;
}

extern "C" vlg_status vlg_workspace_profile(vlg_workspace* ws, int enable)
{
    if (!ws) return fail(VLG_E_INVALID, "null argument");
    ws_reset_stats(ws);
    ws->profile = enable != 0;
    return VLG_OK;
}

extern "C" vlg_status vlg_workspace_set_option(vlg_workspace* ws, const char* name, int64_t value)
{
    if (!ws || !name) return fail(VLG_E_INVALID, "null argument");
    if (!strcmp(name, "dedup")) { ws->dedup = value != 0; return VLG_OK; }
    if (!strcmp(name, "sweep")) { ws->sweep = value != 0; return VLG_OK; }
    if (!strcmp(name, "sweep_min")) { ws->sweep_min = (uint64_t)value; return VLG_OK; }
    if (!strcmp(name, "global_sort_min")) { ws->global_sort_min = (uint64_t)value; return VLG_OK; }
    if (!strcmp(name, "list_sort")) { ws->list_sort = value > 2 ? 1 : (int)value; return VLG_OK; }
    if (!strcmp(name, "trail")) { ws->trail = value != 0; return VLG_OK; }
    if (!strcmp(name, "quad_walk")) { ws->quad_walk = value != 0; return VLG_OK; }
    if (!strcmp(name, "tuples")) { ws->tuples = value != 0; return VLG_OK; }
    if (!strcmp(name, "fuse_jump")) { ws->fuse_jump = value != 0; return VLG_OK; }
    if (!strcmp(name, "filter")) { ws->filter = value != 0; return VLG_OK; }
    if (!strcmp(name, "filter_min")) { ws->filter_min = (uint64_t)value; return VLG_OK; }
    if (!strcmp(name, "filter_pivot")) { ws->filter_pivot = value != 0; return VLG_OK; }
    if (!strcmp(name, "filter_pivot_ratio")) { ws->filter_pivot_ratio = (uint64_t)value; return VLG_OK; }
    if (!strcmp(name, "pivot_range_ratio")) { ws->pivot_range_ratio = (uint64_t)std::max<int64_t>(0, value); return VLG_OK; }
    if (!strcmp(name, "compact_dense_min")) { ws->compact_dense_min = (uint32_t)std::max<int64_t>(0, std::min<int64_t>(value, 1 << 20)); return VLG_OK; }
    if (!strcmp(name, "pivot_rungs")) { ws->pivot_rungs = value <= 0 ? 0u : (value == 1 ? 1u : 2u); return VLG_OK; }
    if (!strcmp(name, "filter_stream_min")) { ws->filter_stream_min = (uint64_t)value; return VLG_OK; }
    if (!strcmp(name, "filter_group_bytes")) { ws->filter_group_bytes = (uint64_t)value; return VLG_OK; }
    if (!strcmp(name, "reserve")) {
        const uint64_t b = std::min<uint64_t>((uint64_t)value, ws->cap_bytes);
        return ws_reserve(ws, b + b / 96 + (256ull << 20));
    }
    if (!strcmp(name, "sweep_tail")) { ws->sweep_tail = (uint64_t)value; return VLG_OK; }
    if (!strcmp(name, "exchange_all")) { ws->exchange_all = value != 0; return VLG_OK; }
    if (!strcmp(name, "unsample_pct")) { ws->unsample_pct = (uint32_t)std::max<int64_t>(0, std::min<int64_t>(value, 1 << 20)); return VLG_OK; }
    if (!strcmp(name, "unsample_tail")) { ws->unsample_tail = (uint64_t)value; return VLG_OK; }
    if (!strcmp(name, "class_intervals")) {
        if (value < 1 || value > (int64_t)kClassIntervalsMax) return fail(VLG_E_INVALID, "class_intervals: 1 .. 2^20");
        ws->class_intervals = (uint32_t)value;
        return VLG_OK;
    }
    if (!strcmp(name, "unsample_min")) { ws->unsample_min = (uint64_t)value; return VLG_OK; }
    return fail(VLG_E_INVALID, std::string("unknown workspace option ") + name);
}

namespace {
vlg_status ws_exchange_reset(vlg_workspace* ws, int n_ranks)
{
    ws->x_comm = nullptr; ws->x_fn = nullptr; ws->x_a2a = nullptr; ws->x_ctx = nullptr; ws->x_ranks = 1; ws->x_rank = 0;
    if (n_ranks > 1 && !ws->x_status) VLG_HIP_TRY(hipMalloc((void**)&ws->x_status, 8 * 1024));
    return VLG_OK;
}
}

extern "C" vlg_status vlg_workspace_set_comm(vlg_workspace* ws, void* nccl_comm)
{
    if (!ws) return fail(VLG_E_INVALID, "null argument");
    if (vlg_status s = ws_exchange_reset(ws, 1)) return s;
    if (!nccl_comm) return VLG_OK;
    int n = 0, r = 0;
    if (vlg_status s = vlg_comm_info(nccl_comm, &n, &r)) return s;
    if (n > 1024) return fail(VLG_E_UNSUPPORTED, "more than 1024 ranks");
    if (vlg_status s = ws_exchange_reset(ws, n)) return s;
    ws->x_comm = nccl_comm; ws->x_ranks = n; ws->x_rank = r;
    return VLG_OK;
}

extern "C" vlg_status vlg_workspace_set_exchange(vlg_workspace* ws, int n_ranks, int rank, vlg_exchange_fn fn, void* ctx)
{
    if (!ws || n_ranks < 1 || n_ranks > 1024 || rank < 0 || rank >= n_ranks || (n_ranks > 1 && !fn)) return fail(VLG_E_INVALID, "bad exchange arguments");
    if (vlg_status s = ws_exchange_reset(ws, n_ranks)) return s;
    ws->x_fn = n_ranks > 1 ? fn : nullptr; ws->x_ctx = ctx; ws->x_ranks = n_ranks; ws->x_rank = rank;
    return VLG_OK;
}

extern "C" vlg_status vlg_workspace_set_exchange_alltoall(vlg_workspace* ws, int n_ranks, int rank, vlg_alltoall_fn fn, void* ctx)
{
    if (!ws || n_ranks < 1 || n_ranks > 1024 || rank < 0 || rank >= n_ranks || (n_ranks > 1 && !fn)) return fail(VLG_E_INVALID, "bad exchange arguments");
    if (vlg_status s = ws_exchange_reset(ws, n_ranks)) return s;
    ws->x_a2a = n_ranks > 1 ? fn : nullptr; ws->x_ctx = ctx; ws->x_ranks = n_ranks; ws->x_rank = rank;
    return VLG_OK;
}

extern "C" vlg_status vlg_workspace_kernel_stats(vlg_workspace* ws, vlg_kernel_stat* out, uint32_t cap, uint32_t* n)
{
    if (!ws || !n) return fail(VLG_E_INVALID, "null argument");
    ws_collect(ws);
    *n = KS_COUNT;
    for (uint32_t k = 0; k < KS_COUNT && k < cap && out; ++k) out[k] = ws->stats[k];
    return VLG_OK;
}

struct ResultPiece {
    uint64_t q0 = 0, q1 = 0;
    uint64_t matches = 0, tuple_vals = 0;
    void* d_first = nullptr;
    void* d_tuples = nullptr;
    uint32_t width = 8;
    uint64_t first_bytes = 0, tuple_bytes = 0;
};

struct vlg_result {
    vlg_result_summary sum;
    std::vector<uint64_t> counts;
    std::vector<uint32_t> k;
    std::vector<ResultPiece> pieces;
    std::vector<uint64_t> owned;
    std::vector<uint64_t> civ_off, civ_l, civ_r;
    bool has_class_intervals = false;
    std::vector<uint64_t> next;
    bool has_next = false;
};

namespace {
constexpr uint64_t kResultCacheBytes = 48ull << 30;
struct ResultCache {
    struct Entry { void* p; uint64_t size; int device; };
    std::mutex mu;
    std::vector<Entry> free_list;
    uint64_t bytes = 0;
    static int device() { int d = 0; (void)hipGetDevice(&d); return d; }
    void* take(uint64_t need, uint64_t* size)
    {
        const int dev = device();
        std::lock_guard<std::mutex> g(mu);
        size_t best = free_list.size();
        for (size_t i = 0; i < free_list.size(); ++i)
            if (free_list[i].device == dev && free_list[i].size >= need && free_list[i].size <= need + need / 4 + (1u << 20) &&
                (best == free_list.size() || free_list[i].size < free_list[best].size)) best = i;
        if (best == free_list.size()) return nullptr;
        void* p = free_list[best].p;
        *size = free_list[best].size;
        bytes -= free_list[best].size;
        free_list.erase(free_list.begin() + best);
        return p;
    }
    void give(void* p, uint64_t size)
    {
        {
            const int dev = device();
            std::lock_guard<std::mutex> g(mu);
            if (bytes + size <= kResultCacheBytes && free_list.size() < 64) { free_list.push_back(Entry{p, size, dev}); bytes += size; return; }
        }
        (void)hipFree(p);
    }
    void drain()
    {
        std::lock_guard<std::mutex> g(mu);
        for (auto& e : free_list) (void)hipFree(e.p);
        free_list.clear();
        bytes = 0;
    }
};
ResultCache& result_cache() { static ResultCache* c = new ResultCache(); return *c; }
void drain_result_cache() { result_cache().drain(); }

hipError_t result_alloc(void** out, uint64_t bytes, uint64_t* got)
{
    if (void* p = result_cache().take(bytes, got)) { *out = p; return hipSuccess; }
    hipError_t e = hipMalloc(out, bytes);
    if (e != hipSuccess) {
        (void)hipGetLastError();
        result_cache().drain();
        e = hipMalloc(out, bytes);
    }
    *got = bytes;
    return e;
}
}

namespace vlg {
void release_cached_device_memory() { result_cache().drain(); }
// ... 361 lines not shown
{
    constexpr uint32_t kPer = 8;
    __shared__ uint64_t s_first;
    for (uint64_t b0 = (uint64_t)blockIdx.x * 256 * kPer; b0 < total; b0 += (uint64_t)gridDim.x * 256 * kPer) {
        __syncthreads();
        if (threadIdx.x == 0) {
            uint64_t lo = 0, hi = n_seg;
            while (hi - lo > 1) { const uint64_t mid = (lo + hi) >> 1; if (dst_off[mid] <= b0) lo = mid; else hi = mid; }
            s_first = lo;
        }
        __syncthreads();
        uint64_t k = s_first;
#pragma unroll
        for (uint32_t i = 0; i < kPer; ++i) {
            const uint64_t t = b0 + i * 256 + threadIdx.x;
            if (t < total) {
                while (dst_off[k + 1] <= t) ++k;
                const uint64_t at = src_off[k] + (t - dst_off[k]);
                if (kGather) packed[t] = base[at]; else base[at] = packed[t];
            }
        }
    }
}

struct PhysChoice {
    uint32_t locate = VLG_LOCATE_WALKS;
    bool sweep = false;
    bool share_steps = false;
    bool list_sort = false;
    bool global_sort = false;
    unsigned pos_bits = 1;
};

template <typename pos_t>
PhysChoice choose_physical(const vlg_index* idx, const vlg_workspace* ws, uint64_t elems, uint64_t n_lists, bool wide, uint64_t unsample_elems,
                           uint64_t scratch_elems, const PhysChoice* sized)
{
    const BlobHeader& h = idx->hdr;
    const bool dense = h.dens == 1 && h.sampling == kSamplingSaOrder;
    PhysChoice c;
    c.pos_bits = std::max(1u, bit_width64(h.n >= 2 ? h.n - 2 : 0));
    c.sweep = ws->sweep && elems >= ws->sweep_min && h.n <= (1ull << (wide ? 33 : 32)) &&
              (!idx->is_int || (int_sweep_possible(idx->iview) && sizeof(pos_t) == 4 && !wide));
    const uint64_t n_walkers = idx->is_int ? 0 : idx->view.n_samples;
    const bool unsample = c.sweep && sizeof(pos_t) == 4 && ws->unsample_pct && ws->trail && ws->dedup && !idx->is_int && h.sampling == kSamplingSaOrder &&
                          h.dens >= 2 && h.n <= (1ull << 32) + 1 && h.sigma < 0x7FFFu && unsample_elems >= ws->sweep_min && unsample_elems >= ws->unsample_min &&
                          (__uint128_t)unsample_elems * 100 >= (__uint128_t)h.n * ws->unsample_pct &&
                          (!scratch_elems || align_up(h.n * 4, 256) + n_walkers * 20 + 1024 <= scratch_elems * kPhysScratchPerElem<pos_t>()) &&
                          (!sized || sized->locate == VLG_LOCATE_UNSAMPLE);
    c.locate = !c.sweep ? (idx->is_int && dense ? VLG_LOCATE_COPY : VLG_LOCATE_WALKS) : unsample ? VLG_LOCATE_UNSAMPLE : dense ? VLG_LOCATE_COPY : VLG_LOCATE_SWEEP;
    c.share_steps = c.sweep && !unsample && ws->trail && ws->dedup && !dense && elems <= 0xFFFFFF00ull && (!sized || sized->share_steps);
    c.list_sort = sizeof(pos_t) == 4 && ws->list_sort;
    c.global_sort = elems >= ws->global_sort_min && c.pos_bits + bit_width64(n_lists) <= 64;
    return c;
}

template <typename pos_t, typename word_t>
vlg_status expand_and_walk(vlg_workspace* ws, const IndexView& lview, const uint64_t* d_l, const uint64_t* d_off, uint64_t n_lists, uint64_t total, word_t* io,
                           pos_t* out, unsigned long long* d_stats)
{
    {
        Timed t(ws, KS_EXPAND, 0);
        if (vlg_status s = launch_expand<word_t>(d_l, d_off, n_lists, total, io, nullptr, ws->stream)) return s;
    }
    Timed t(ws, KS_LOCATE, 0);
    if (vlg_status s = launch_locate<word_t>(lview, io, total, d_stats, ws->stream)) return s;
    if constexpr (sizeof(word_t) != sizeof(pos_t)) return launch_narrow<pos_t>(io, out, total, ws->stream);
    return VLG_OK;
}

struct SuperChunk {
    uint64_t Q0 = 0, Q1 = 0, phys = 0;
    std::vector<uint32_t> dlist;
};

struct ChunkPlan {
    PhysChoice c;
    size_t sort_tmp = 0;
    bool want_rungs = false;
    uint64_t phys_bytes = 0, join_budget = 0;
    bool launch_first = false;
};

template <typename pos_t>
struct PhysicalPass {
    const vlg_index* idx; vlg_workspace* ws; vlg_result* res; const Plan& pl; const ChunkPlan& cp; bool wide; Arena& A;
    unsigned long long* d_stats; Lists<pos_t>& L;
    hipStream_t st = ws->stream;
    PhaseTrace bt{st};
    std::vector<uint32_t> dlist, cut;
    std::vector<uint64_t> xcounts;
    uint32_t gnd = 0, n_outer = 0, sl = 0, nd = 0;
    uint64_t gacc = 0, acc = 0;
    svec<uint64_t> goff64, off64, lh; svec<uint32_t> off32;
    PhysChoice c;
    pos_t* Pg = nullptr; pos_t* Pa = nullptr; pos_t* Pb = nullptr; uint8_t* scratch = nullptr; void* d_tmp = nullptr;
    uint64_t* d_goff64 = nullptr; uint64_t* d_off64 = nullptr; uint32_t* d_off32 = nullptr; uint64_t* d_lh = nullptr; unsigned long long* d_counter = nullptr;
    uint64_t* rec = nullptr; Block* member = nullptr; uint8_t* front = nullptr;
    uint64_t sort_mark = 0; ListSortPlan lsp;
    bool pairwise = false;

    void layout(const std::vector<uint32_t>& dlist_in)
    {
        gnd = (uint32_t)dlist_in.size();
        dlist = dlist_in;
        bool ascending = true;
        for (uint32_t i = 1; i < gnd && ascending; ++i) ascending = pl.dl[dlist[i - 1]] <= pl.dl[dlist[i]];
        if (!ascending)
            std::sort(dlist.begin(), dlist.end(), [&](uint32_t a, uint32_t b) { return pl.dl[a] != pl.dl[b] ? pl.dl[a] < pl.dl[b] : pl.docc[a] < pl.docc[b]; });
        std::vector<uint32_t> inner;
        uint64_t cover_end = 0;
        uint32_t w = 0;
        for (uint32_t i = 0; i < gnd;) {
            uint32_t j = i, longest = i;
            for (; j < gnd && pl.dl[dlist[j]] == pl.dl[dlist[i]]; ++j) if (pl.docc[dlist[j]] > pl.docc[dlist[longest]]) longest = j;
            const bool outer = pl.dl[dlist[i]] >= cover_end;
            for (uint32_t t = i; t < j; ++t) {
                if (t == longest && outer) continue;
                inner.push_back(dlist[t]);
            }
            if (outer) { const uint32_t d = dlist[longest]; cover_end = pl.dl[d] + pl.docc[d]; dlist[w++] = d; }
            i = j;
        }
        n_outer = w;
        for (uint32_t d : inner) dlist[w++] = d;
        goff64.resize(gnd + 1);
        for (uint32_t i = 0; i < gnd; ++i) {
            goff64[i] = gacc;
            L.doff[dlist[i]] = (uint32_t)gacc;
            gacc += pl.docc[dlist[i]];
        }
        goff64[gnd] = gacc;
        uint32_t sh = gnd;
        cut.assign(ws->x_ranks + 1, gnd);
        if (ws->x_ranks > 1) {
            cut[0] = 0;
            for (int r = 1; r < ws->x_ranks; ++r) {
                const uint64_t target = gacc / (uint64_t)ws->x_ranks * (uint64_t)r;
                const uint32_t at = (uint32_t)(std::lower_bound(goff64.begin(), goff64.end(), target) - goff64.begin());
                cut[r] = std::max(cut[r - 1], std::min(at, gnd));
            }
            xcounts.resize(ws->x_ranks);
            for (int r = 0; r < ws->x_ranks; ++r) xcounts[r] = goff64[cut[r + 1]] - goff64[cut[r]];
            sl = cut[ws->x_rank]; sh = cut[ws->x_rank + 1];
        }
        nd = sh - sl;
        off64.resize(nd + 1); lh.resize(std::max<uint32_t>(nd, 1)); off32.resize(nd + 1);
        for (uint32_t i = 0; i <= nd; ++i) { off64[i] = goff64[sl + i] - goff64[sl]; off32[i] = (uint32_t)off64[i]; }
        for (uint32_t i = 0; i < nd; ++i) lh[i] = pl.dl[dlist[sl + i]];
        acc = off64[nd];
        c = choose_physical<pos_t>(idx, ws, acc, nd, wide, acc, gacc, &cp.c);
    }

    vlg_status carve()
    {
        Pg = A.take<pos_t>(gacc);
        scratch = A.take<uint8_t>(gacc * kPhysScratchPerElem<pos_t>());
        Pa = Pg ? Pg + goff64[sl] : nullptr;
        d_goff64 = (ws->x_ranks > 1) ? A.take<uint64_t>(gnd + 1) : nullptr;
        d_off64 = A.take<uint64_t>(nd + 1);
        d_off32 = A.take<uint32_t>(nd + 1);
        d_lh = A.take<uint64_t>(nd);
        d_counter = A.take<unsigned long long>(4);
        d_tmp = A.take<uint8_t>(cp.sort_tmp + 256);
        if (A.failed) return fail(VLG_E_INTERNAL, "arena carve failed (physical)");
        Pb = reinterpret_cast<pos_t*>(scratch);
        VLG_HIP_TRY(hipMemcpyAsync(d_off64, off64.data(), (nd + 1) * 8, hipMemcpyHostToDevice, st));
        VLG_HIP_TRY(hipMemcpyAsync(d_off32, off32.data(), (nd + 1) * 4, hipMemcpyHostToDevice, st));
        if (nd) VLG_HIP_TRY(hipMemcpyAsync(d_lh, lh.data(), nd * 8, hipMemcpyHostToDevice, st));
        if (d_goff64) VLG_HIP_TRY(hipMemcpyAsync(d_goff64, goff64.data(), (gnd + 1) * 8, hipMemcpyHostToDevice, st));
        if (c.share_steps) {
            rec = A.take<uint64_t>(acc);
            member = A.take<Block>(member_blocks(idx->hdr.n));
            if (!idx->is_int) front = A.take<uint8_t>(acc);
            if (A.failed) return fail(VLG_E_INTERNAL, "arena carve failed (member bit-vector, records)");
        }
        sort_mark = A.used;
        return VLG_OK;
    }

    vlg_status plan_sort()
    {
        if (!c.list_sort) return VLG_OK;
        const vlg_status ls = list_sort_prepare(off64, nd, A, st, lsp);
        if (ls != VLG_OK && ls != VLG_E_WORKSPACE) return ls;
        if (ls != VLG_OK) A.used = sort_mark;
        return VLG_OK;
    }

    vlg_status locate(const std::function<vlg_status()>& hook )
    {
        if (!acc) return VLG_OK;
        const uint64_t n_walkers = idx->is_int ? 0 : idx->view.n_samples;
        vlg_status s = VLG_OK;
        const IndexView lview = ws->quad_walk ? idx->view : without_quad(idx->view);
        if (c.locate == VLG_LOCATE_UNSAMPLE) {
            uint32_t* sa_full = reinterpret_cast<uint32_t*>(scratch);
            uint64_t* val_a = reinterpret_cast<uint64_t*>(scratch + align_up(idx->hdr.n * 4, 256));
            uint64_t* val_b = val_a + n_walkers;
            uint16_t* key_a = reinterpret_cast<uint16_t*>(val_b + n_walkers);
            uint16_t* key_b = key_a + n_walkers;
            svec<unsigned long long> h_done(1, 0);
            SweepTimer timer(ws);
            bt.mark("  physical: tables + sort plan");
            if constexpr (sizeof(pos_t) == 4) {
                if (wide) s = launch_unsample<true>(idx->view, d_lh, d_off64, nd, acc, Pa, sa_full, val_a, val_b, key_a, key_b, d_tmp, cp.sort_tmp, d_counter, h_done.data(),
                                                    d_stats, ws->unsample_tail, st, &timer, &hook);
                else s = launch_unsample<false>(idx->view, d_lh, d_off64, nd, acc, Pa, sa_full, val_a, val_b, key_a, key_b, d_tmp, cp.sort_tmp, d_counter, h_done.data(),
                                                d_stats, ws->unsample_tail, st, &timer, &hook);
            }
            if (!s) bt.mark("  physical: unsampling");
        } else if (c.sweep) {
            const uint64_t cap = std::min<uint64_t>(acc, wide ? sweep_batch_max<true>() : sweep_batch_max<false>());
            uint64_t* val_a = reinterpret_cast<uint64_t*>(scratch);
            uint64_t* val_b = val_a + cap;
            uint16_t* key_a = reinterpret_cast<uint16_t*>(val_b + cap);
            uint16_t* key_b = key_a + cap;
            const uint32_t n_member_lists = n_outer > sl ? std::min(n_outer - sl, nd) : 0u;
            SweepTimer timer(ws);
            bt.mark("  physical: tables + sort plan");
            if (idx->is_int) {
                if constexpr (sizeof(pos_t) == 4)
                    s = launch_int_locate_sweep(idx->iview, d_lh, d_off64, nd, acc, Pa, val_a, val_b, key_a, key_b, d_tmp, cp.sort_tmp, d_counter, d_stats, ws->sweep_tail, st,
                                                &timer, member, n_member_lists, rec, &hook);
                else s = fail(VLG_E_INTERNAL, "integer-alphabet index with 64-bit positions");
            } else if (wide)
                s = launch_locate_sweep<pos_t, true>(lview, d_lh, d_off64, nd, acc, Pa, val_a, val_b, key_a, key_b, d_tmp, cp.sort_tmp, d_counter, d_stats,
                                                     ws->sweep_tail, st, &timer, member, n_member_lists, rec, &hook, front);
            else if constexpr (sizeof(pos_t) == 4)
                s = launch_locate_sweep<uint32_t, false>(lview, d_lh, d_off64, nd, acc, Pa, val_a, val_b, key_a, key_b, d_tmp, cp.sort_tmp, d_counter, d_stats,
                                                         ws->sweep_tail, st, &timer, member, n_member_lists, rec, &hook, front);
            else s = fail(VLG_E_INTERNAL, "64-bit positions with 32-bit SA indices");
            if (!s) bt.mark("  physical: sweep");
        } else if (idx->is_int) {
            if ((s = plan_sort())) return s;
            if constexpr (sizeof(pos_t) == 4) {
                if (c.locate == VLG_LOCATE_COPY) {
                    Timed t(ws, KS_LOCATE, 0);
                    s = launch_int_dense_copy(idx->iview, d_lh, d_off64, nd, acc, Pa, st);
                } else {
                    {
                        Timed t(ws, KS_EXPAND, 0);
                        if ((s = launch_expand<uint32_t>(d_lh, d_off64, nd, acc, Pa, nullptr, st))) return s;
                    }
                    Timed t(ws, KS_LOCATE, 0);
                    s = launch_int_locate(idx->iview, Pa, acc, d_stats, st);
                }
            } else s = fail(VLG_E_INTERNAL, "integer-alphabet index with 64-bit positions");
        } else if (wide && sizeof(pos_t) == 4) s = walks(reinterpret_cast<uint64_t*>(scratch), lview);
        else s = walks(Pa, lview);
        if (s) return s;
        ws->sample_reads += c.locate == VLG_LOCATE_UNSAMPLE ? n_walkers : acc;
        res->sum.locate_mode = c.locate;
        return VLG_OK;
    }

    template <typename word_t>
    vlg_status walks(word_t* io, const IndexView& lview)
    {
        if (vlg_status s = plan_sort()) return s;
        return expand_and_walk(ws, lview, d_lh, d_off64, nd, acc, io, Pa, d_stats);
    }

    vlg_status sort(pos_t*& P)
    {
        P = Pa;
        if (!acc) return VLG_OK;
        if (lsp.ready) {
            Timed t(ws, KS_SORT, 2ull * acc * sizeof(pos_t));
            if (vlg_status ls = list_sort_enqueue(lsp, reinterpret_cast<uint32_t*>(Pa), reinterpret_cast<uint32_t*>(scratch), d_off64, c.pos_bits, st, ws->list_sort == 1)) return ls;
            A.used = sort_mark;
        } else if (c.global_sort) {
            const unsigned bits = c.pos_bits, list_bits = bit_width64(nd);
            uint64_t* ka = reinterpret_cast<uint64_t*>(scratch);
            uint64_t* kb = ka + acc;
            Timed t(ws, KS_SORT, 2ull * acc * sizeof(pos_t));
            hipLaunchKernelGGL(HIP_KERNEL_NAME(sort_compose_kernel<pos_t>), launch_grid((acc + 7) / 8, 32768), dim3(256), 0, st, Pa, d_off64, (uint64_t)nd, acc, bits, ka);
            rocprim::double_buffer<uint64_t> keys(ka, kb);
            size_t tb = cp.sort_tmp;
            VLG_HIP_TRY(rocprim::radix_sort_keys(d_tmp, tb, keys, acc, 0, bits + list_bits, st));
            hipLaunchKernelGGL(HIP_KERNEL_NAME(sort_narrow_kernel<pos_t>), launch_grid(acc, 32768), dim3(256), 0, st, keys.current(), acc, bits, Pa);
            VLG_HIP_TRY(hipGetLastError());
        } else {
            Timed t(ws, KS_SORT, 2ull * acc * sizeof(pos_t));
            size_t tb = cp.sort_tmp;
            VLG_HIP_TRY(rocprim::segmented_radix_sort_keys(d_tmp, tb, Pa, Pb, (unsigned)acc, nd, d_off32, d_off32 + 1, 0, c.pos_bits, st));
            P = Pb;
            if (ws->x_ranks > 1) {
                VLG_HIP_TRY(hipMemcpyAsync(Pa, Pb, acc * sizeof(pos_t), hipMemcpyDeviceToDevice, st));
                P = Pa;
            }
        }
        return VLG_OK;
    }

    vlg_status exchange(pos_t*& P, const vlg_queries* q, const std::vector<uint64_t>* xq, Agreement* ag)
    {
        if (ws->x_ranks <= 1) return VLG_OK;
        if (ag) if (vlg_status as = ag->settle(VLG_OK)) return as;
        const int n = ws->x_ranks, me = ws->x_rank;
        pairwise = !ws->exchange_all && !ws->x_fn && (ws->x_a2a || ws->x_comm) && q && xq && (int)xq->size() == n + 1;
        P = Pg;
        if (!pairwise) {
            Timed t(ws, KS_EXCHANGE, (gacc - acc) * sizeof(pos_t));
            int rc = 0;
            if (ws->x_fn) rc = ws->x_fn(ws->x_ctx, Pg, xcounts.data(), (uint32_t)sizeof(pos_t), n, me, st);
            else if (ws->x_comm) rc = (int)vlg_comm_allgatherv(ws->x_comm, Pa, xcounts.data(), (uint32_t)sizeof(pos_t), Pg, st);
            else return fail(VLG_E_INTERNAL, "collective search without a communicator (or an all-to-all callback with \"exchange_all\")");
            if (rc) return ws->x_fn ? fail(VLG_E_INTERNAL, "the exchange callback failed with code " + std::to_string(rc)) : (vlg_status)rc;
            return VLG_OK;
        }
        std::vector<uint32_t> place(pl.dl.size(), 0);
        for (uint32_t i = 0; i < gnd; ++i) place[dlist[i]] = i;
        std::vector<uint8_t> need((size_t)n * gnd, 0);
        for (int r = 0; r < n; ++r) {
            uint8_t* nr = need.data() + (size_t)r * gnd;
            for (uint64_t qi = (*xq)[r]; qi < (*xq)[r + 1]; ++qi)
                for (uint64_t sidx = q->qsub[qi]; sidx < q->qsub[qi + 1]; ++sidx)
                    if (pl.occ[sidx]) nr[place[pl.did[sidx]]] = 1;
        }
        auto segments = [&](int from, int to, svec<uint64_t>& src, svec<uint64_t>& dst, uint64_t& at) {
            const uint8_t* nt = need.data() + (size_t)to * gnd;
            for (uint32_t i = cut[from]; i < cut[from + 1];) {
                if (!nt[i] || goff64[i + 1] == goff64[i]) { ++i; continue; }
                uint32_t j = i;
                while (j < cut[from + 1] && nt[j]) ++j;
                src.push_back(goff64[i]);
                dst.push_back(at);
                at += goff64[j] - goff64[i];
                i = j;
            }
        };
        svec<uint64_t> s_src, s_dst, r_src, r_dst;
        std::vector<uint64_t> scount((size_t)n, 0), rcount((size_t)n, 0);
        uint64_t s_at = 0, r_at = 0;
        for (int r = 0; r < n; ++r) {
            if (r == me) continue;
            uint64_t b = s_at;
            segments(me, r, s_src, s_dst, s_at);
            scount[r] = s_at - b;
            b = r_at;
            segments(r, me, r_src, r_dst, r_at);
            rcount[r] = r_at - b;
        }
        s_dst.push_back(s_at);
        r_dst.push_back(r_at);
        const uint64_t ns = s_src.size(), nr_ = r_src.size();
        pos_t* d_send = A.take<pos_t>(s_at + 1);
        pos_t* d_recv = A.take<pos_t>(r_at + 1);
        uint64_t* d_seg = A.take<uint64_t>(2 * (ns + nr_) + 4);
        if (A.failed) return fail(VLG_E_WORKSPACE, "collective search: no room for the exchange buffers");
        uint64_t* d_s_src = d_seg; uint64_t* d_s_dst = d_s_src + ns; uint64_t* d_r_src = d_s_dst + ns + 1; uint64_t* d_r_dst = d_r_src + nr_;
        if (ns) VLG_HIP_TRY(hipMemcpyAsync(d_s_src, s_src.data(), ns * 8, hipMemcpyHostToDevice, st));
        VLG_HIP_TRY(hipMemcpyAsync(d_s_dst, s_dst.data(), (ns + 1) * 8, hipMemcpyHostToDevice, st));
        if (nr_) VLG_HIP_TRY(hipMemcpyAsync(d_r_src, r_src.data(), nr_ * 8, hipMemcpyHostToDevice, st));
        VLG_HIP_TRY(hipMemcpyAsync(d_r_dst, r_dst.data(), (nr_ + 1) * 8, hipMemcpyHostToDevice, st));
        Timed t(ws, KS_EXCHANGE, r_at * sizeof(pos_t));
        if (s_at) hipLaunchKernelGGL(HIP_KERNEL_NAME(segments_copy_kernel<pos_t, true>), launch_grid((s_at + 7) / 8, 16384), dim3(256), 0, st, Pg, d_send, d_s_src, d_s_dst, ns, s_at);
        VLG_HIP_TRY(hipGetLastError());
        int rc = 0;
        if (ws->x_a2a) rc = ws->x_a2a(ws->x_ctx, d_send, scount.data(), d_recv, rcount.data(), (uint32_t)sizeof(pos_t), n, me, st);
        else rc = (int)vlg_comm_alltoallv(ws->x_comm, d_send, scount.data(), d_recv, rcount.data(), (uint32_t)sizeof(pos_t), st);
        if (rc) return ws->x_a2a ? fail(VLG_E_INTERNAL, "the exchange callback failed with code " + std::to_string(rc)) : (vlg_status)rc;
        if (r_at) hipLaunchKernelGGL(HIP_KERNEL_NAME(segments_copy_kernel<pos_t, false>), launch_grid((r_at + 7) / 8, 16384), dim3(256), 0, st, Pg, d_recv, d_r_src, d_r_dst, nr_, r_at);
        VLG_HIP_TRY(hipGetLastError());
        return VLG_OK;
    }

    vlg_status check_sort()
    {
        if (!check_sort_enabled()) return VLG_OK;
        const bool all = ws->x_ranks > 1 && !pairwise;
        unsigned long long* d_flags = A.take<unsigned long long>(2);
        if (!d_flags) return fail(VLG_E_INTERNAL, "arena carve failed (sort check)");
        unsigned long long flags[2] = {0, 0};
        VLG_HIP_TRY(hipMemsetAsync(d_flags, 0, 16, st));
        const uint64_t n = all ? gacc : acc;
        hipLaunchKernelGGL(HIP_KERNEL_NAME(lists_check_kernel<pos_t>), launch_grid((n + 7) / 8, 8192), dim3(256), 0, st, pairwise ? Pa : L.P, all ? d_goff64 : d_off64,
                           (uint64_t)(all ? gnd : nd), n, d_flags);
        VLG_HIP_TRY(hipGetLastError());
        VLG_HIP_TRY(hipMemcpyAsync(flags, d_flags, 16, hipMemcpyDeviceToHost, st));
        VLG_HIP_TRY(hipStreamSynchronize(st));
        if (flags[0]) return fail(VLG_E_INTERNAL, "an occurrence list is not ascending after the sort (VLG_CHECK_SORT)");
        return VLG_OK;
// ... 481 lines not shown
        }
    }
    jp.filter_need = filter_group_charge(filter_total, jp.group_cap, filter_runs);
    if (jp.filter_need >= join_budget || jp.logical_max_query > join_budget - jp.filter_need) {
        std::fill(jp.fbytes.begin(), jp.fbytes.end(), 0);
        jp.filter_need = 0;
    }
    const uint64_t cap_bytes = join_budget - jp.filter_need;
    if (jp.logical_max_query > cap_bytes)
        return fail(VLG_E_WORKSPACE, "a query needs " + std::to_string(jp.logical_max_query) + " bytes of join scratch; workspace cap allows " +
                                         std::to_string(cap_bytes));
    jp.want_bytes = std::min<uint64_t>(logical_total, cap_bytes);
    jp.meta = join_meta_bytes(q->qsub[Q1] - q->qsub[Q0], Q1 - Q0, jp.want_bytes);
    return VLG_OK;
}

template <typename pos_t>
vlg_status run_joins(uint64_t n_positions, const vlg_queries* q, vlg_workspace* ws, vlg_result* res, const Plan& pl, const Lists<pos_t>& L,
                     const Arena& A, uint64_t Q0, uint64_t Q1, const JoinPlan& jp, unsigned long long* d_stats, PhaseTrace& tr)
{
    const uint64_t max_chunk_slots = 0xF0000000ull;
    const uint64_t pc_cap = L.pc_cap;
    uint64_t g0 = Q0;
    while (g0 < Q1) {
        Arena GA = A;
        FilterGroup fg;
        fg.g0 = g0; fg.pc_cap = pc_cap;
        uint64_t fb = 0, g1 = g0;
        while (g1 < Q1) {
            const uint64_t b = pc_cap ? jp.fbytes[g1 - Q0] : 0;
            if (fb + b > jp.group_cap && g1 > g0) break;
            fb += b;
            fg.want.push_back(b > 0);
            ++g1;
        }
        fg.g1 = g1;
        const FilterGroup* fgp = nullptr;
        if (fb) {
            if (vlg_status s = filter_group<pos_t>(n_positions, q, ws, pl, L, GA, fg)) return s;
            if (fg.any) fgp = &fg;
            res->sum.filter_stream_segments += fg.n_stream; res->sum.filter_bit_segments += fg.n_bits; res->sum.filter_range_segments += fg.n_ranges;
            res->sum.filter_survivors += fg.survivors; res->sum.filter_overflows += fg.overflowed;
            tr.mark("filter group");
        }
        auto eff = [&](uint64_t s) -> uint64_t { return fgp ? fgp->eff[s - fgp->sub0] : pl.occ[s]; };
        auto compacted = [&](uint64_t s) -> bool { return fgp && !fgp->speculated && fgp->cidx[s - fgp->sub0] != kNone; };
        uint64_t q0 = g0;
        while (q0 < g1) {
            uint64_t T = 0, S = 0, C = 0, q1 = q0;
            while (q1 < g1) {
                const JoinCost c = join_cost(q, q1, eff, compacted);
                if (c.slots > max_chunk_slots) return fail(VLG_E_WORKSPACE, "a query has more than 2^32 join slots");
                if (((T + c.bytes > jp.want_bytes || S + c.slots > max_chunk_slots || C + c.survivors > pc_cap) && q1 > q0) || (q1 - q0) >= (1u << 22)) break;
                T += c.bytes; S += c.slots; C += c.survivors;
                ++q1;
            }
            vlg_status s = run_join_chunk<pos_t>(q, ws, res, q0, q1, pl, L, GA, d_stats, fgp);
            if (s) return s;
            tr.mark("join chunk");
            q0 = q1;
        }
        g0 = g1;
    }
    return VLG_OK;
}

vlg_status next_super_chunk(const vlg_queries* q, const Plan& pl, bool dedup, uint64_t phys_cap, uint64_t Q0, std::vector<uint32_t>& stamp, uint32_t& epoch,
                            SuperChunk& sc)
{
    std::vector<uint32_t>& dlist = sc.dlist;
    dlist.reserve(pl.dl.size());
    uint64_t phys = 0, Q1 = Q0;
    if (Q0 == 0 && dedup) {
        uint64_t all = 0;
        for (uint64_t d = 0; d < pl.docc.size() && all <= phys_cap; ++d) all += pl.docc[d];
        if (all <= phys_cap) {
            phys = all;
            Q1 = q->nq;
            dlist.resize(pl.dl.size());
            for (uint32_t d = 0; d < (uint32_t)pl.dl.size(); ++d) dlist[d] = d;
            std::fill(stamp.begin(), stamp.end(), epoch);
        }
    }
    while (Q1 < q->nq) {
        uint64_t add = 0;
        size_t mark = dlist.size();
        for (uint64_t s = q->qsub[Q1]; s < q->qsub[Q1 + 1]; ++s)
            if (pl.occ[s] && stamp[pl.did[s]] != epoch) { stamp[pl.did[s]] = epoch; dlist.push_back(pl.did[s]); add += pl.occ[s]; }
        if (phys + add > phys_cap) {
            for (size_t i = mark; i < dlist.size(); ++i) stamp[dlist[i]] = 0xFFFFFFFFu;
            dlist.resize(mark);
            if (Q1 == Q0)
                return fail(VLG_E_WORKSPACE, "query " + std::to_string(Q1) + " needs " + std::to_string(add) +
                                                 " occurrence slots; workspace cap allows " + std::to_string(phys_cap));
            break;
        }
        phys += add;
        ++Q1;
    }
    ++epoch;
    if (dlist.size() > 1) {
        if (dlist.size() * 8 >= pl.dl.size()) {
            size_t w = 0;
            for (uint32_t d = 0; d < (uint32_t)pl.dl.size(); ++d) if (stamp[d] == epoch - 1) dlist[w++] = d;
        } else std::sort(dlist.begin(), dlist.end());
    }
    sc.Q0 = Q0; sc.Q1 = Q1; sc.phys = phys;
    return VLG_OK;
}

template <typename pos_t>
vlg_status plan_super_chunk(const vlg_index* idx, const vlg_queries* q, const Plan& pl, vlg_workspace* ws, const SuperChunk& sc, bool wide,
                            uint64_t budget, uint64_t fixed, bool trace, ChunkPlan& cp)
{
    const uint64_t phys = sc.phys, Q0 = sc.Q0, Q1 = sc.Q1;
    const std::vector<uint32_t>& dlist = sc.dlist;
    cp.c = choose_physical<pos_t>(idx, ws, phys, dlist.size(), wide, phys / (uint64_t)std::max(1, ws->x_ranks), 0, nullptr);
    const uint64_t tmp_key[6] = {phys, dlist.size(), idx->hdr.n, ((uint64_t)idx->hdr.sigma << 8) | ((uint64_t)ws->sweep << 1) | (uint64_t)idx->is_int | (sizeof(pos_t) << 4),
                                 ws->global_sort_min, ws->sweep_min};
    if (phys && !memcmp(tmp_key, ws->tmp_key, sizeof tmp_key)) cp.sort_tmp = ws->tmp_bytes;
    else if (phys) {
        if (cp.c.global_sort) {
            rocprim::double_buffer<uint64_t> nk(nullptr, nullptr);
            VLG_HIP_TRY(rocprim::radix_sort_keys(nullptr, cp.sort_tmp, nk, phys, 0, 64, ws->stream));
        } else {
            pos_t* np = nullptr; uint32_t* nu = nullptr;
            VLG_HIP_TRY(rocprim::segmented_radix_sort_keys(nullptr, cp.sort_tmp, np, np, (unsigned)phys, (unsigned)dlist.size(), nu, nu, 0,
                                                           cp.c.pos_bits, ws->stream));
        }
        if (cp.c.sweep) cp.sort_tmp = std::max(cp.sort_tmp, sweep_temp_bytes(phys, idx->hdr.sigma, ws->stream));
        memcpy(ws->tmp_key, tmp_key, sizeof tmp_key);
        ws->tmp_bytes = cp.sort_tmp;
    }
    uint64_t logical_max_query = 0, pivot_elems = 0;
    {
        uint64_t part_max[kHostThreads] = {0}, part_piv[kHostThreads] = {0};
        const bool count_pivots = ws->filter && ws->filter_pivot && ws->pivot_rungs;
        const FilterOptions fo = filter_options(ws);
        parallel_slices(Q0, Q1, 1u << 16, [&](uint64_t a, uint64_t b, uint32_t t) {
            uint64_t mx = 0, pv_sum = 0;
            for (uint64_t qi = a; qi < b; ++qi) {
                mx = std::max(mx, join_cost(q, pl, qi).bytes);
                if (!count_pivots) continue;
                const FilterShape sh = query_shape(q, pl, fo, qi);
                if (sh.by_pivot()) pv_sum += sh.occ[sh.pivot];
            }
            part_max[t] = mx; part_piv[t] = pv_sum;
        });
        for (uint32_t t = 0; t < kHostThreads; ++t) { logical_max_query = std::max(logical_max_query, part_max[t]); pivot_elems += part_piv[t]; }
    }
    uint64_t trail_bytes = cp.c.share_steps ? member_blocks(idx->hdr.n) * sizeof(Block) + phys * 9 + 2048 : 0;
    cp.want_rungs = pivot_elems && (ws->pivot_rungs == 2 || (pivot_elems >= phys / 16 && pivot_elems >= 4096));
    const uint64_t rung_bytes = cp.want_rungs ? rung_layout(phys).entries * sizeof(pos_t) + 8192 : 0;
    const uint64_t phys_plain = phys * (sizeof(pos_t) + kPhysScratchPerElem<pos_t>()) + cp.sort_tmp + (dlist.size() + 2) * 24 + (8ull << 20) + phys + rung_bytes;
    if (trail_bytes) {
        const uint64_t left = budget > phys_plain + trail_bytes ? budget - phys_plain - trail_bytes : 0;
        if (left < std::max<uint64_t>(2 * logical_max_query, budget / 8)) trail_bytes = 0;
    }
    cp.c.share_steps = trail_bytes != 0;
    if (trace) {
        fprintf(stderr, "[vlg trace] super-chunk: %llu occurrences, %.1f GB physical, LF steps %s (%.1f GB), budget %.1f GB, largest join %.1f GB\n",
                (unsigned long long)phys, phys_plain / 1e9, cp.c.share_steps ? "shared" : "not shared",
                (member_blocks(idx->hdr.n) * sizeof(Block) + phys * 8) / 1e9, budget / 1e9, logical_max_query / 1e9);
        uint64_t cnt[40] = {0}, sum[40] = {0};
        for (uint32_t d : dlist) { const unsigned b = bit_width64(pl.docc[d]); cnt[b]++; sum[b] += pl.docc[d]; }
        fprintf(stderr, "[vlg trace] distinct lists by size (2^b: lists/occurrences):");
        for (unsigned b = 0; b < 40; ++b) if (cnt[b]) fprintf(stderr, " %u:%llu/%llu", b, (unsigned long long)cnt[b], (unsigned long long)sum[b]);
        fprintf(stderr, "\n");
    }
    cp.phys_bytes = phys_plain + trail_bytes;
    cp.join_budget = budget > cp.phys_bytes ? budget - cp.phys_bytes : 0;
    cp.launch_first = ws->arena_bytes >= budget + join_meta_bytes(q->qsub[Q1] - q->qsub[Q0], Q1 - Q0, budget) + 2 * fixed;
    return VLG_OK;
}

std::vector<uint64_t> cut_queries(const vlg_queries* q, const Plan& pl, uint64_t Q0, uint64_t Q1, int n_ranks)
{
    std::vector<uint64_t> cum(Q1 - Q0 + 1, 0);
    for (uint64_t qi = Q0; qi < Q1; ++qi)
        cum[qi - Q0 + 1] = cum[qi - Q0] + 1 + (pl.occ[q->qsub[qi]] ? join_cost(q, pl, qi).slots : 0);
    auto cut_at = [&](int r) -> uint64_t {
        if (r <= 0) return Q0;
        if (r >= n_ranks) return Q1;
        const uint64_t target = cum.back() / (uint64_t)n_ranks * (uint64_t)r;
        return Q0 + (uint64_t)(std::lower_bound(cum.begin(), cum.end(), target) - cum.begin());
    };
    std::vector<uint64_t> xq(n_ranks + 1);
    xq[0] = Q0;
    for (int r = 1; r <= n_ranks; ++r) xq[r] = std::max(xq[r - 1], std::min(cut_at(r), Q1));
    return xq;
}

template <typename pos_t>
__device__ __forceinline__ uint32_t fenced_lower_bound(const pos_t* __restrict__ P, const pos_t* __restrict__ F, uint32_t a, uint32_t b, uint64_t key)
{
    if (!F || b - a < 128) return lower_bound_dev(P, a, b, key);
    const uint64_t g0 = (uint64_t)lower_bound_dev(F, a >> 6, b >> 6, key) << 6;
    const uint32_t w0 = g0 < a ? a : (uint32_t)g0;
    const uint32_t w1 = g0 + 64 < b ? (uint32_t)(g0 + 64) : b;
    return lower_bound_dev(P, w0, w1, key);
}
template <typename pos_t>
__global__ void __launch_bounds__(256) window_cut_kernel(const pos_t* __restrict__ P, const pos_t* __restrict__ F, const uint32_t* __restrict__ a,
                                                         const uint32_t* __restrict__ len, const uint64_t* __restrict__ klo, const uint64_t* __restrict__ khi,
                                                         uint64_t nsub, uint32_t* __restrict__ cut)
{
    for (uint64_t t = (uint64_t)blockIdx.x * blockDim.x + threadIdx.x; t < 2 * nsub; t += (uint64_t)gridDim.x * blockDim.x) {
        const uint64_t s = t >> 1;
        const uint32_t la = a[s];
        cut[t] = fenced_lower_bound(P, F, la, la + len[s], (t & 1) ? khi[s] : klo[s]);
    }
}
__global__ void window_lengths_kernel(const uint64_t* __restrict__ qsub, uint64_t Q0, uint64_t Q1, uint64_t s0, const uint32_t* __restrict__ cut,
                                      uint64_t* __restrict__ occ)
{
    for (uint64_t qi = Q0 + (uint64_t)blockIdx.x * blockDim.x + threadIdx.x; qi < Q1; qi += (uint64_t)gridDim.x * blockDim.x) {
        const uint64_t sa = qsub[qi] - s0, sb = qsub[qi + 1] - s0;
        bool live = sb > sa;
        for (uint64_t s = sa; s < sb && live; ++s) live = cut[2 * s + 1] > cut[2 * s];
        for (uint64_t s = sa; s < sb; ++s) occ[s] = live ? (uint64_t)(cut[2 * s + 1] - cut[2 * s]) : 0;
    }
}

template <typename pos_t>
vlg_status cut_to_windows(const vlg_index* idx, const vlg_queries* q, vlg_workspace* ws, const Plan& pl, const SuperChunk& sc, Lists<pos_t>& L, Arena WA,
                          Plan& cut, uint64_t& logical)
{
    const uint64_t s0 = q->qsub[sc.Q0], ns = q->qsub[sc.Q1] - s0, n_text = idx->hdr.n - 1;
    hipStream_t st = ws->stream;
    if (cut.occ.size() != q->nsub) { cut.occ.resize(q->nsub); cut.did = pl.did; cut.dl = pl.dl; cut.docc = pl.docc; }
    if (!ns) return VLG_OK;
    svec<uint32_t> h_a(ns), h_len(ns), h_cut(2 * ns);
    svec<uint64_t> h_klo(ns), h_khi(ns);
    parallel_slices(sc.Q0, sc.Q1, 1u << 16, [&](uint64_t qa, uint64_t qb, uint32_t) {
        for (uint64_t qi = qa; qi < qb; ++qi)
            for (uint64_t s = q->qsub[qi]; s < q->qsub[qi + 1]; ++s) {
                const WindowKeys k = window_keys(q->win_begin[qi], q->win_end[qi], (q->suboff[s + 1] - q->suboff[s]) / q->sym_bytes, n_text);
                const bool none = k.empty || !pl.occ[s];
                h_a[s - s0] = none ? 0 : L.doff[pl.did[s]];
                h_len[s - s0] = none ? 0 : (uint32_t)pl.occ[s];
                h_klo[s - s0] = k.klo; h_khi[s - s0] = k.khi;
            }
    });
    uint32_t* d_a = WA.take<uint32_t>(ns);
    uint32_t* d_len = WA.take<uint32_t>(ns);
    uint64_t* d_klo = WA.take<uint64_t>(ns);
    uint64_t* d_khi = WA.take<uint64_t>(ns);
    uint32_t* d_cut = WA.take<uint32_t>(2 * ns);
    uint64_t* d_occ = WA.take<uint64_t>(ns);
    if (WA.failed) return fail(VLG_E_WORKSPACE, "no room behind the lists for the window cut of " + std::to_string(ns) + " sub-patterns");
    VLG_HIP_TRY(hipMemcpyAsync(d_a, h_a.data(), ns * 4, hipMemcpyHostToDevice, st));
    VLG_HIP_TRY(hipMemcpyAsync(d_len, h_len.data(), ns * 4, hipMemcpyHostToDevice, st));
    VLG_HIP_TRY(hipMemcpyAsync(d_klo, h_klo.data(), ns * 8, hipMemcpyHostToDevice, st));
    VLG_HIP_TRY(hipMemcpyAsync(d_khi, h_khi.data(), ns * 8, hipMemcpyHostToDevice, st));
    {
        Timed t(ws, KS_WINDOW_CUT, 2 * ns * 256);
        hipLaunchKernelGGL(HIP_KERNEL_NAME(window_cut_kernel<pos_t>), launch_grid(2 * ns, 4096), dim3(256), 0, st, (const pos_t*)L.P, (const pos_t*)L.F, d_a,
                           d_len, d_klo, d_khi, ns, d_cut);
        hipLaunchKernelGGL(window_lengths_kernel, launch_grid(sc.Q1 - sc.Q0, 2048), dim3(256), 0, st, q->d_qsub, sc.Q0, sc.Q1, s0, d_cut, d_occ);
    }
    VLG_HIP_TRY(hipGetLastError());
    VLG_HIP_TRY(hipMemcpyAsync(h_cut.data(), d_cut, 2 * ns * 4, hipMemcpyDeviceToHost, st));
    VLG_HIP_TRY(hipMemcpyAsync(cut.occ.data() + s0, d_occ, ns * 8, hipMemcpyDeviceToHost, st));
    VLG_HIP_TRY(hipStreamSynchronize(st));
    for (uint64_t s = 0; s < ns; ++s) { L.off[s0 + s] = cut.occ[s0 + s] ? h_cut[2 * s] : 0; logical += cut.occ[s0 + s]; }
    return VLG_OK;
}

template <typename pos_t>
vlg_status run_windowed_chunk(const vlg_index* idx, const vlg_queries* q, vlg_workspace* ws, vlg_result* res, const Plan& pl, const SuperChunk& sc,
                              const ChunkPlan& cp, bool wide, uint64_t fixed, unsigned long long* d_stats, Lists<pos_t>& L, Plan& cut, PhaseTrace& tr)
{
    const uint64_t subs = q->qsub[sc.Q1] - q->qsub[sc.Q0], queries = sc.Q1 - sc.Q0;
    if (!cp.launch_first) {
        JoinPlan full;
        const std::string keep = vlg_last_error();
        uint64_t join_bytes = cp.join_budget + join_meta_bytes(subs, queries, cp.join_budget);
        if (plan_joins(q, pl, ws, sc.Q0, sc.Q1, cp.join_budget, idx->hdr.n, full) == VLG_OK) join_bytes = full.filter_need + full.want_bytes + full.meta;
        else set_error(keep);
        if (vlg_status s = ws_reserve(ws, cp.phys_bytes + join_bytes + fixed)) return s;
    }
    Arena A{ws->arena, ws->arena_bytes};
    tr.mark("plan super-chunk");
    if (vlg_status s = build_physical<pos_t>(idx, ws, res, pl, sc, cp, wide, A, d_stats, L)) return s;
    tr.mark("locate + sort");
    if (vlg_status s = cut_to_windows<pos_t>(idx, q, ws, pl, sc, L, A, cut, res->sum.logical_occurrences)) return s;
    tr.mark("window cut");
    const uint64_t taken = cp.phys_bytes + fixed + join_meta_bytes(subs, queries, 0);
    const uint64_t room = ws->arena_bytes > taken ? ws->arena_bytes - taken : 0;
    JoinPlan jp;
    if (vlg_status s = plan_joins(q, cut, ws, sc.Q0, sc.Q1, std::min<uint64_t>(cp.join_budget, room - room / 128), idx->hdr.n, jp)) return s;
    return run_joins<pos_t>(idx->hdr.n, q, ws, res, cut, L, A, sc.Q0, sc.Q1, jp, d_stats, tr);
}

template <typename pos_t>
vlg_status run_batch(const vlg_index* idx, const vlg_queries* q, vlg_workspace* ws, vlg_result* res, const Plan& pl,
                     unsigned long long* d_stats, bool wide)
{
    const uint64_t fixed = 8ull << 20;
    if (ws->cap_bytes <= 2 * fixed) return fail(VLG_E_WORKSPACE, "workspace cap too small");
    const uint64_t budget = ws->cap_bytes - fixed;
    const uint64_t phys_cap = std::min<uint64_t>(budget / 2 / (sizeof(pos_t) + kPhysScratchPerElem<pos_t>() + 1), 0xFFFFFF00ull);
    std::vector<uint32_t> stamp(pl.dl.size(), 0xFFFFFFFFu);
    Lists<pos_t> L;
    L.doff.assign(pl.dl.size(), 0);
    L.off.assign(q->nsub, 0);
    uint32_t epoch = 0;
// ... 393 lines not shown
    const uint64_t total = h_off[n_lists];
    if (!total) return VLG_OK;
    if (total > 0xFFFFFF00ull) return fail(VLG_E_UNSUPPORTED, "more than 2^32 keys in one vlg_sort_lists_u32 call: split the batch");
    int ndev = 0;
    if (hipGetDeviceCount(&ndev) != hipSuccess || ndev <= 0) return fail(VLG_E_NO_DEVICE, "no HIP device available (the VLG library has no CPU fallback)");
    hipStream_t st = (hipStream_t)stream;
    HostPool pool;
    void* d_mem = nullptr;
    auto run = [&]() -> vlg_status {
        HostPoolScope scope(&pool);
        svec<uint64_t> off64(h_off, h_off + n_lists + 1);
        uint64_t n_long = 0, n_tiles = 0, n_chunks = 0;
        for (uint64_t l = 0; l < n_lists; ++l) {
            const uint64_t len = off64[l + 1] - off64[l];
            if (len > kSortTile) { const uint64_t t = (len + kSortTile - 1) / kSortTile; ++n_long; n_tiles += t; n_chunks += (t + kSortChunk - 1) / kSortChunk; }
        }
        const uint64_t bytes = align_up(total * 4, 256) + align_up((n_lists + 1) * 8, 256) + align_up(n_lists * 4, 256) + kSortClasses * 256 +
                               list_sort_scratch_bytes(n_long, n_tiles, n_chunks) + 16 * 256 + 8192;
        VLG_HIP_TRY(hipMalloc(&d_mem, bytes));
        Arena A{reinterpret_cast<uint8_t*>(d_mem), bytes};
        uint32_t* other = A.take<uint32_t>(total);
        uint64_t* d_off = A.take<uint64_t>(n_lists + 1);
        if (A.failed) return fail(VLG_E_INTERNAL, "arena carve failed (vlg_sort_lists_u32)");
        VLG_HIP_TRY(hipMemcpyAsync(d_off, off64.data(), (n_lists + 1) * 8, hipMemcpyHostToDevice, st));
        ListSortPlan lp;
        if (vlg_status s = list_sort_prepare(off64, (uint32_t)n_lists, A, st, lp)) return s;
        if (vlg_status s = list_sort_enqueue(lp, d_pos, other, d_off, position_bits, st, mode == 1)) return s;
        if (n_clustered && lp.n_long) {
            std::vector<SortList> back(lp.n_long);
            VLG_HIP_TRY(hipMemcpyAsync(back.data(), lp.d_longs, lp.n_long * sizeof(SortList), hipMemcpyDeviceToHost, st));
            VLG_HIP_TRY(hipStreamSynchronize(st));
            for (const SortList& L : back) *n_clustered += L.pad ? 1 : 0;
        }
        VLG_HIP_TRY(hipStreamSynchronize(st));
        return VLG_OK;
    };
    vlg_status s;
    try { s = run(); } catch (const std::bad_alloc&) { s = fail(VLG_E_OOM, "host memory (vlg_sort_lists_u32)"); }
    if (d_mem) { (void)hipStreamSynchronize(st); (void)hipFree(d_mem); }
    pool.release();
    return s;
}

extern "C" vlg_status vlg_join_batch(const uint64_t* d_lists, const uint64_t* h_list_off, uint64_t n_lists, const uint64_t* h_join_list,
                                     const uint64_t* h_lo, const uint64_t* h_hi, const uint64_t* h_end_len, uint64_t n_joins,
                                     vlg_workspace* ws, vlg_result** out)
{
    if (!ws || !out || !h_list_off || !h_join_list || (n_lists && (!h_lo || !h_hi)) || (n_joins && !h_end_len))
        return fail(VLG_E_INVALID, "null argument");
    *out = nullptr;
    int ndev = 0;
    if (hipGetDeviceCount(&ndev) != hipSuccess || ndev <= 0) return fail(VLG_E_NO_DEVICE, "no HIP device available");
    if (h_list_off[0] != 0 || h_join_list[0] != 0 || h_join_list[n_joins] > n_lists) return fail(VLG_E_INVALID, "bad list / join offsets");
    for (uint64_t t = 0; t < n_lists; ++t) if (h_list_off[t + 1] < h_list_off[t]) return fail(VLG_E_INVALID, "list offsets must ascend");
    const uint64_t total = h_list_off[n_lists];
    if (total && !d_lists) return fail(VLG_E_INVALID, "null argument");
    if (total > 0xFFFFFF00ull) return fail(VLG_E_UNSUPPORTED, "more than 2^32 list elements in one vlg_join_batch call: split the batch");
    vlg_queries qq;
    qq.nq = n_joins;
    qq.nsub = h_join_list[n_joins];
    qq.qsub.assign(h_join_list, h_join_list + n_joins + 1);
    qq.lo.assign(h_lo, h_lo + qq.nsub);
    qq.hi.assign(h_hi, h_hi + qq.nsub);
    qq.end_len.assign(h_end_len, h_end_len + n_joins);
    qq.kmax = 0; qq.kmin = 0xFFFFFFFFu;
    hipStream_t st = ws->stream;
    vlg_result* res = new_result(n_joins, qq.qsub);
    unsigned long long* d_stats = nullptr;
    auto run = [&]() -> vlg_status {
        Plan pl;
        pl.occ.assign(qq.nsub, 0);
        pl.did.assign(qq.nsub, 0);
        Lists<uint64_t> L;
        L.off.assign(qq.nsub, 0);
        for (uint64_t j = 0; j < n_joins; ++j) {
            if (qq.qsub[j + 1] < qq.qsub[j] || qq.qsub[j + 1] - qq.qsub[j] > VLG_MAX_SUBPATTERNS) return fail(VLG_E_INVALID, "bad join offsets");
            const uint32_t k = (uint32_t)(qq.qsub[j + 1] - qq.qsub[j]);
            qq.kmax = std::max(qq.kmax, k);
            if (k) qq.kmin = std::min(qq.kmin, k);
            if (k && h_end_len[j] == 0) return fail(VLG_E_INVALID, "end_len must be at least 1");
            if (h_end_len[j] >= (1ull << 63)) return fail(VLG_E_INVALID, "end_len out of range");
            bool live = k > 0;
            for (uint64_t s = qq.qsub[j]; s < qq.qsub[j + 1]; ++s) {
                if (s > qq.qsub[j] && (h_lo[s] > h_hi[s] || h_hi[s] >= (1ull << 63))) return fail(VLG_E_INVALID, "bad gap bounds");
                live = live && h_list_off[s + 1] > h_list_off[s];
            }
            if (live) for (uint64_t s = qq.qsub[j]; s < qq.qsub[j + 1]; ++s) { pl.occ[s] = h_list_off[s + 1] - h_list_off[s]; L.off[s] = (uint32_t)h_list_off[s]; }
        }
        if (qq.kmin == 0xFFFFFFFFu) qq.kmin = 0;
        for (uint64_t s = 0; s < qq.nsub; ++s) res->sum.logical_occurrences += pl.occ[s];
        VLG_HIP_TRY(hipMalloc((void**)&d_stats, kStatsWords * 8));
        VLG_HIP_TRY(hipMemsetAsync(d_stats, 0, kStatsWords * 8, st));
        PhaseTrace tr(st);
        const uint64_t fixed = 8ull << 20;
        if (ws->cap_bytes <= 2 * fixed) return fail(VLG_E_WORKSPACE, "workspace cap too small");
        const uint64_t budget = ws->cap_bytes - fixed;
        const ListRoom room(total, ws->filter);
        const uint64_t list_bytes = align_up(room.positions() * 8, 256) + align_up((n_lists + 1) * 8, 256) + align_up(room.fence_entries * 8, 256) + 4096;
        if (list_bytes >= budget) return fail(VLG_E_WORKSPACE, "the lists do not fit the workspace cap");
        unsigned long long flags[2] = {0, 0};
        uint64_t* d_off_in = nullptr;
        svec<uint64_t> off_stage(h_list_off, h_list_off + n_lists + 1);
        if (total) {
            VLG_HIP_TRY(hipMalloc((void**)&d_off_in, (n_lists + 1) * 8));
            hipError_t e = hipMemcpyAsync(d_off_in, off_stage.data(), (n_lists + 1) * 8, hipMemcpyHostToDevice, st);
            if (e == hipSuccess) {
                hipLaunchKernelGGL(HIP_KERNEL_NAME(lists_check_kernel<uint64_t>), launch_grid((total + 7) / 8, 8192), dim3(256), 0, st, d_lists, d_off_in, n_lists, total, d_stats + 4);
                e = hipGetLastError();
            }
            if (e == hipSuccess) e = hipMemcpyAsync(flags, d_stats + 4, sizeof flags, hipMemcpyDeviceToHost, st);
            if (e == hipSuccess) e = hipStreamSynchronize(st);
            (void)hipFree(d_off_in);
            VLG_HIP_TRY(e);
        }
        if (flags[0]) return fail(VLG_E_INVALID, "every list must be ascending");
        if (flags[1] > (1ull << 63)) return fail(VLG_E_INVALID, "positions above 2^63 are not supported");
        const uint64_t n_positions = flags[1] + 1;
        JoinPlan jp;
        if (vlg_status s = plan_joins(&qq, pl, ws, 0, n_joins, budget - list_bytes, n_positions, jp)) return s;
        if (vlg_status s = ws_reserve(ws, list_bytes + jp.filter_need + jp.want_bytes + jp.meta + fixed)) return s;
        Arena A{ws->arena, ws->arena_bytes};
        L.P = A.take<uint64_t>(room.positions());
        uint64_t* F = A.take<uint64_t>(room.fence_entries);
        if (A.failed) return fail(VLG_E_INTERNAL, "arena carve failed (join lists)");
        if (total) VLG_HIP_TRY(hipMemcpyAsync(L.P, d_lists, total * 8, hipMemcpyDeviceToDevice, st));
        if (vlg_status s = wire_room_and_fences(L, room, total, F, st)) return s;
        tr.mark("join lists copied + checked");
        if (vlg_status s = run_joins<uint64_t>(n_positions, &qq, ws, res, pl, L, A, 0, n_joins, jp, d_stats, tr)) return s;
        unsigned long long hs[kStatsWords];
        return read_checksum(ws, res, d_stats, hs);
    };
    vlg_status stt;
    {
        HostPoolScope staging(&ws->host);
        try { stt = run(); }
        catch (const std::bad_alloc&) { stt = fail(VLG_E_OOM, "out of host memory while planning the joins (pinned staging)"); }
    }
    if (d_stats) (void)hipFree(d_stats);
    if (stt) { vlg_result_destroy(res); return stt; }
    *out = res;
    return VLG_OK;
}

#include "wtsa.hpp"
#include "wtsa_sdsl.hpp"
#include "int_index.hpp"

extern "C" vlg_status vlg_build_constants(vlg_build_constant* out, uint32_t cap, uint32_t* n)
{
    if (!n) return fail(VLG_E_INVALID, "null argument");
    const vlg::KernelConstants kc = vlg::kernel_constants();
    const struct { const char* name; int64_t value; } all[] = {
        {"VLG_LINK_RUN", VLG_LINK_RUN}, {"VLG_COOP_WINDOWS2", VLG_COOP_WINDOWS2}, {"VLG_RUNG_SHIFT", VLG_RUNG_SHIFT},
        {"VLG_RESOLVE_HOPS", kc.resolve_hops}, {"VLG_RESOLVE_CHUNK", kc.resolve_chunk}, {"VLG_GROUP_CHUNK", kc.group_chunk},
        {"VLG_STAGE_LISTS", kc.stage_lists}, {"VLG_SWEEP_PAIRS", kc.sweep_pairs},
        {"VLG_PIVOT_GROUPS", VLG_PIVOT_GROUPS}, {"VLG_PIVOT_TURNS", VLG_PIVOT_TURNS}, {"VLG_COMPACT_RUNS", VLG_COMPACT_RUNS},
        {"VLG_SPARSE_TURN", VLG_SPARSE_TURN}, {"VLG_SORT_CLASSES", VLG_SORT_CLASSES}, {"VLG_BUCKET_SORT", VLG_BUCKET_SORT},
        {"VLG_WINDOW_SORT", VLG_WINDOW_SORT}, {"VLG_WINDOWS_PER_TILE", VLG_WINDOWS_PER_TILE}, {"VLG_WINDOW_RANK_LOOP", VLG_WINDOW_RANK_LOOP},
        {"VLG_WINDOW_THREADS", VLG_WINDOW_THREADS}, {"VLG_WINDOW_ITEMS", VLG_WINDOW_ITEMS}, {"VLG_FETCH_THREADS", VLG_FETCH_THREADS},
        {"VLG_DOCLIST_RUN", VLG_DOCLIST_RUN},
    };
    const uint32_t count = (uint32_t)(sizeof(all) / sizeof(all[0]));
    *n = count;
    for (uint32_t i = 0; i < count && i < cap && out; ++i) {
        memset(out[i].name, 0, sizeof(out[i].name));
        strncpy(out[i].name, all[i].name, sizeof(out[i].name) - 1);
        out[i].value = all[i].value;
    }
    return VLG_OK;
}
```

### vlg_matching_amd/csrc/sweep_kernels.hpp

```cpp
#pragma once
#include "lf_walk.hpp"
#include "kernels.hpp"
#include "shape_dispatch.hpp"

namespace vlg {

template <int N>
__device__ __forceinline__ void block_add(unsigned long long (&v)[N], unsigned long long* const (&dst)[N])
{
    __shared__ unsigned long long s_acc[N];
    if (threadIdx.x < N) s_acc[threadIdx.x] = 0;
    __syncthreads();
#pragma unroll
    for (int k = 0; k < N; ++k) {
        unsigned long long x = v[k];
        for (int o = 32; o > 0; o >>= 1) x += __shfl_down(x, o);
        if ((threadIdx.x & 63) == 0 && x) atomicAdd(&s_acc[k], x);
    }
    __syncthreads();
    if (threadIdx.x < N && s_acc[threadIdx.x] && dst[threadIdx.x]) atomicAdd(dst[threadIdx.x], s_acc[threadIdx.x]);
}

template <uint32_t kShift>
__device__ __forceinline__ uint64_t follow_owner(const uint64_t* rec, uint32_t owner, uint64_t delta)
{
    const uint64_t ro = rec[owner];
    if (ro == ~0ull) return (delta << kShift) | owner;
    if ((ro >> kShift) == 0) return ro + delta;
    return ro + (delta << kShift);
}

struct WaveSlice {
    uint32_t lane;
    uint64_t next, end;
    __device__ __forceinline__ WaveSlice(uint64_t total, uint32_t per_wave)
    {
        lane = threadIdx.x & 63;
        const uint64_t wave = ((uint64_t)blockIdx.x * blockDim.x + threadIdx.x) >> 6;
        next = wave * per_wave;
        end = next + per_wave < total ? next + per_wave : total;
    }
    template <class Take>
    __device__ __forceinline__ void refill(bool need, const Take& take)
    {
        const unsigned long long m = __ballot(need);
        if (m) {
            const uint32_t before = __popcll(m & ((1ull << lane) - 1ull));
            if (need) take(next + before);
            next += __popcll(m);
        }
    }
};

template <class Walk, class Sampling, typename pos_t, bool kTail = false, bool kWide = (sizeof(pos_t) == 8)>
__global__ void __launch_bounds__(256) locate_kernel(typename Walk::View iv, pos_t* __restrict__ io, uint64_t total, uint32_t per_wave,
                                                     unsigned long long* __restrict__ stats ,
                                                     const uint64_t* __restrict__ val = nullptr, uint32_t step = 0,
                                                     uint64_t* __restrict__ rec = nullptr, uint64_t slot0 = 0,
                                                     const Block* __restrict__ member = nullptr)
{
    static_assert(kTail || kWide == (sizeof(pos_t) == 8), "in place, io[] holds the SA index: its width is the index width");
    constexpr uint32_t kShift = kWide ? 33 : 32;
    constexpr uint64_t kPosMask = (1ull << kShift) - 1;
    __shared__ typename Walk::Lds s;
    Walk::stage(s, iv);
    const Walk walk{iv, s};
    WaveSlice slice(total, per_wave);
    const Sampling sampling(iv);

    uint64_t t = 0;
    uint64_t i = 0;
    typename Walk::Cursor k;
    uint32_t off = 0;
    bool active = false, need = true;
    uint32_t n_lf = 0, n_lv = 0;
    for (;;) {
        slice.refill(need, [&](uint64_t cand) {
            if (cand < slice.end) {
                if (kTail) { const uint64_t e = val[cand]; t = e >> kShift; i = e & kPosMask; off = step; }
                else { t = cand; i = io[cand]; off = 0; }
                k = typename Walk::Cursor();
                active = true;
            }
            else active = false;
            need = false;
        });
        if (!__any(active)) break;
        if (active) {
            uint64_t sv = 0;
            uint32_t owner = 0, c;
            if (k.at_root() && sampling.probe(i, sv)) {
                uint64_t r = sv + off;
                if (r >= walk.n()) r -= walk.n();
                if (kTail && rec) rec[slot0 + t] = r;
                else io[t] = (pos_t)r;
                need = true;
                active = false;
            } else if (kTail && member && k.at_root() && off != 0 && member_probe(member, i, owner)) {
                rec[slot0 + t] = follow_owner<kShift>(rec, owner, off);
                need = true;
                active = false;
            } else if (walk.degenerate()) {
                i = 0; ++off;
            } else if (walk.level(k, i, c, n_lv)) {
                ++off;
                ++n_lf;
            }
        }
    }
    if (stats) {
        unsigned long long v[2] = {n_lf, n_lv};
        unsigned long long* const dst[2] = {&stats[0], &stats[1]};
        block_add<2>(v, dst);
    }
}


#ifndef VLG_STAGE_LISTS
#define VLG_STAGE_LISTS 1
#endif
constexpr bool kStageLists = VLG_STAGE_LISTS != 0;
static_assert(VLG_STAGE_LISTS == 0 || VLG_STAGE_LISTS == 1, "VLG_STAGE_LISTS: 0 or 1");
constexpr uint32_t kListStage = 256;
struct ListStage { uint64_t off[kListStage + 1]; uint64_t l[kListStage]; };
__device__ __forceinline__ bool stage_lists(ListStage& ls, const uint64_t* __restrict__ out_off, const uint64_t* __restrict__ l, uint64_t n_pat,
                                            uint64_t first, uint64_t end)
{
    for (uint32_t j = threadIdx.x; j <= kListStage; j += blockDim.x) {
        const uint64_t p = first + j;
        ls.off[j] = out_off[p < n_pat ? p : n_pat];
        if (j < kListStage) ls.l[j] = l[p < n_pat ? p : n_pat - 1];
    }
    __syncthreads();
    return ls.off[kListStage] >= end;
}

template <class Walk, class Sampling, typename pos_t, bool kTrail, bool kWide, bool kFirst = false, bool kAhead = false>
__device__ __forceinline__ void sweep_element(const Walk& walk, const Sampling& sampling, uint64_t e, uint64_t v64,
                                              uint64_t* __restrict__ val, uint16_t* __restrict__ key, uint32_t step, pos_t* __restrict__ out,
                                              const Block* __restrict__ member, uint64_t* __restrict__ rec, uint64_t slot0,
                                              uint32_t& n_lv, uint32_t& n_lf, uint32_t& n_fin, bool probed = false, uint8_t* __restrict__ front = nullptr)
{
    constexpr uint32_t kShift = kWide ? 33 : 32;
    constexpr uint64_t kPosMask = (1ull << kShift) - 1;
    uint64_t i = v64 & kPosMask;
    uint8_t in_front = 0xFF;
    uint64_t sv = 0;
    uint32_t owner = 0;
    if (sampling.probe(i, sv)) {
        uint64_t r = sv + step;
        if (r >= walk.n()) r -= walk.n();
        if (kTrail) rec[slot0 + (v64 >> kShift)] = r;
        else out[v64 >> kShift] = (pos_t)r;
        key[e] = (uint16_t)walk.sigma();
        ++n_fin;
    } else if (kTrail && !kFirst && !probed && member_probe(member, i, owner)) {
        rec[slot0 + (v64 >> kShift)] = follow_owner<kShift>(rec, owner, step);
        key[e] = (uint16_t)walk.sigma();
        ++n_fin;
    } else {
        if (kTrail && kFirst) rec[slot0 + (v64 >> kShift)] = ~0ull;
        uint32_t c;
        const uint64_t j = walk.lf(i, c, n_lv);
        ++n_lf;
        if (kTrail && kAhead && member_probe(member, j, owner)) {
            rec[slot0 + (v64 >> kShift)] = ((uint64_t)(step + 1) << kShift) | owner;
            key[e] = (uint16_t)walk.sigma();
            ++n_fin;
            in_front = (uint8_t)c;
        } else {
            val[e] = (v64 & ~kPosMask) | j;
            key[e] = (uint16_t)c;
        }
    }
    if (kTrail && kFirst && front) front[slot0 + (v64 >> kShift)] = in_front;
}

#ifndef VLG_SWEEP_PAIRS
#define VLG_SWEEP_PAIRS 1
#endif
constexpr bool kSweepPairs = VLG_SWEEP_PAIRS != 0;
static_assert(VLG_SWEEP_PAIRS == 0 || VLG_SWEEP_PAIRS == 1, "VLG_SWEEP_PAIRS: 0 or 1");
template <class Walk, class Sampling, typename pos_t, bool kTrail, bool kWide>
__global__ void __launch_bounds__(256) sweep_step_kernel(typename Walk::View iv, uint64_t* __restrict__ val, uint16_t* __restrict__ key, uint64_t count,
                                                         uint32_t step, pos_t* __restrict__ out,
                                                         unsigned long long* __restrict__ stats ,
                                                         unsigned long long* __restrict__ n_done, const Block* __restrict__ member,
                                                         uint64_t* __restrict__ rec, uint64_t slot0, bool probed)
{
    __shared__ typename Walk::Lds s;
    Walk::stage(s, iv);
    const Walk walk{iv, s};
    const Sampling sampling(iv);
    uint32_t n_lv = 0, n_lf = 0, n_fin = 0;
    for (uint64_t e = (uint64_t)blockIdx.x * blockDim.x + threadIdx.x; e < count; e += (uint64_t)gridDim.x * blockDim.x)
        sweep_element<Walk, Sampling, pos_t, kTrail, kWide>(walk, sampling, e, val[e], val, key, step, out, member, rec, slot0, n_lv, n_lf, n_fin, probed);
    unsigned long long v[3] = {n_lf, n_lv, n_fin};
    unsigned long long* const dst[3] = {&stats[0], &stats[1], n_done};
    block_add<3>(v, dst);
}

template <typename pos_t, bool kTrail, bool kWide, bool kAhead, class Sampling>
__device__ __forceinline__ void sweep_first_pair(const IndexView& iv, const WalkLds<PlainBV>& s, const Sampling& sampling, bool onA, uint64_t eA, uint64_t wA,
                                                 bool onB, uint64_t eB, uint64_t wB, uint64_t* __restrict__ val, uint16_t* __restrict__ key,
                                                 pos_t* __restrict__ out, const Block* __restrict__ member, uint64_t* __restrict__ rec, uint64_t slot0,
                                                 uint32_t& n_lv, uint32_t& n_lf, uint32_t& n_fin, uint8_t* __restrict__ front)
{
    constexpr uint32_t kShift = kWide ? 33 : 32;
    constexpr uint64_t kPosMask = (1ull << kShift) - 1;
    using walk_t = typename std::conditional<kWide, uint64_t, uint32_t>::type;
    const uint64_t iA = wA & kPosMask, iB = wB & kPosMask;
    const bool hadA = onA, hadB = onB;
    uint64_t sv = 0;
    if (onA && sampling.probe(iA, sv)) {
        if (kTrail) rec[slot0 + (wA >> kShift)] = sv; else out[wA >> kShift] = (pos_t)sv;
        key[eA] = (uint16_t)iv.sigma; ++n_fin; onA = false;
    }
    if (onB && sampling.probe(iB, sv)) {
        if (kTrail) rec[slot0 + (wB >> kShift)] = sv; else out[wB >> kShift] = (pos_t)sv;
        key[eB] = (uint16_t)iv.sigma; ++n_fin; onB = false;
    }
    if (kTrail) {
        if (onA) rec[slot0 + (wA >> kShift)] = ~0ull;
        if (onB) rec[slot0 + (wB >> kShift)] = ~0ull;
    }
    uint32_t vA = 0, vB = 0, cA = 0, cB = 0;
    walk_t pA = (walk_t)iA, pB = (walk_t)iB;
    bool a = onA, b = onB;
    while (a || b) {
        const DNode ndA = s.nodes[vA], ndB = s.nodes[vB];
        uint32_t blkA, offA, blkB, offB;
        split224((uint64_t)pA, blkA, offA);
        split224((uint64_t)pB, blkB, offB);
        BlockRegs rA, rB;
        if (a) rA = load_block(iv.blocks, ndA.base + blkA);
        if (b) rB = load_block(iv.blocks, ndB.base + blkB);
        if (a) {
            uint32_t bit;
            const walk_t r1 = (walk_t)block_rank_bit(rA, offA, bit);
            ++n_lv;
            pA = bit ? r1 : pA - r1;
            const uint32_t ch = bit ? ndA.child[1] : ndA.child[0];
            if (ch & kLeafFlag) { cA = ch & ~kLeafFlag; a = false; } else vA = ch;
        }
        if (b) {
            uint32_t bit;
            const walk_t r1 = (walk_t)block_rank_bit(rB, offB, bit);
            ++n_lv;
            pB = bit ? r1 : pB - r1;
            const uint32_t ch = bit ? ndB.child[1] : ndB.child[0];
            if (ch & kLeafFlag) { cB = ch & ~kLeafFlag; b = false; } else vB = ch;
        }
    }
    const uint64_t jA = s.C[cA] + (uint64_t)pA, jB = s.C[cB] + (uint64_t)pB;
    n_lf += (onA ? 1u : 0u) + (onB ? 1u : 0u);
    bool stopA = false, stopB = false;
    uint32_t ownA = 0, ownB = 0;
    if (kTrail && kAhead) {
        uint32_t blkA, offA, blkB, offB, bit;
        split224(jA, blkA, offA);
        split224(jB, blkB, offB);
        BlockRegs rA, rB;
        if (onA) rA = load_block(member, blkA);
        if (onB) rB = load_block(member, blkB);
        if (onA) { ownA = block_rank_bit(rA, offA, bit); stopA = bit != 0; }
        if (onB) { ownB = block_rank_bit(rB, offB, bit); stopB = bit != 0; }
    }
    if (onA) {
        if (stopA) { rec[slot0 + (wA >> kShift)] = (1ull << kShift) | ownA; key[eA] = (uint16_t)iv.sigma; ++n_fin; }
        else { val[eA] = (wA & ~kPosMask) | jA; key[eA] = (uint16_t)cA; }
    }
    if (onB) {
        if (stopB) { rec[slot0 + (wB >> kShift)] = (1ull << kShift) | ownB; key[eB] = (uint16_t)iv.sigma; ++n_fin; }
        else { val[eB] = (wB & ~kPosMask) | jB; key[eB] = (uint16_t)cB; }
    }
    if (kTrail && front) {
        if (hadA) front[slot0 + (wA >> kShift)] = (onA && stopA) ? (uint8_t)cA : (uint8_t)0xFF;
        if (hadB) front[slot0 + (wB >> kShift)] = (onB && stopB) ? (uint8_t)cB : (uint8_t)0xFF;
    }
}

template <class Walk, class Sampling, typename pos_t, bool kTrail, bool kWide, bool kAhead>
__global__ void __launch_bounds__(256) sweep_first_kernel(typename Walk::View iv, const uint64_t* __restrict__ l, const uint64_t* __restrict__ out_off, uint64_t n_pat,
                                                          uint64_t t0, uint64_t total, uint64_t* __restrict__ val, uint16_t* __restrict__ key,
                                                          pos_t* __restrict__ out, unsigned long long* __restrict__ stats,
                                                          unsigned long long* __restrict__ n_done, const Block* __restrict__ member,
                                                          uint64_t* __restrict__ rec, const uint32_t* __restrict__ chunk_list, uint8_t* __restrict__ front)
{
    constexpr bool kStage = kStageLists && Walk::kStageLists;
    __shared__ typename Walk::Lds s;
    __shared__ ListStage s_lists;
    Walk::stage(s, iv);
    const Walk walk{iv, s};
    const Sampling sampling(iv);
    constexpr uint32_t kShift = kWide ? 33 : 32;
    constexpr uint32_t kPer = kSweepChunk / 256;
    uint32_t n_lv = 0, n_lf = 0, n_fin = 0;
    for (uint64_t base = t0 + (uint64_t)blockIdx.x * kSweepChunk; base < total; base += (uint64_t)gridDim.x * kSweepChunk) {
        __syncthreads();
        uint64_t p = chunk_list[(base - t0) / kSweepChunk];
        const uint64_t end = base + 256 * kPer < total ? base + 256 * kPer : total;
        const bool staged = kStage && stage_lists(s_lists, out_off, l, n_pat, p, end);
        uint32_t q = 0;
        auto word_of = [&](uint64_t t) -> uint64_t {
            uint64_t sai;
            if (staged) {
                while (s_lists.off[q + 1] <= t) ++q;
                sai = s_lists.l[q] + (t - s_lists.off[q]);
            } else {
                while (out_off[p + 1] <= t) ++p;
                sai = l[p] + (t - out_off[p]);
            }
            return ((t - t0) << kShift) | sai;
        };
        if constexpr (Walk::kPlainTree && kSweepPairs && kWide) {
            static_assert(kPer % 2 == 0, "elements are taken in pairs");
#pragma unroll 1
            for (uint32_t i = 0; i < kPer; i += 2) {
                const uint64_t tA = base + i * 256 + threadIdx.x, tB = tA + 256;
                const bool onA = tA < total, onB = tB < total;
                const uint64_t wA = onA ? word_of(tA) : 0, wB = onB ? word_of(tB) : 0;
                sweep_first_pair<pos_t, kTrail, kWide, kAhead>(iv, s, sampling, onA, tA - t0, wA, onB, tB - t0, wB, val, key, out, member, rec, t0, n_lv, n_lf, n_fin, front);
            }
        } else {
#pragma unroll 1
            for (uint32_t i = 0; i < kPer; ++i) {
                const uint64_t t = base + i * 256 + threadIdx.x;
                if (t < total)
                    sweep_element<Walk, Sampling, pos_t, kTrail, kWide, true, kAhead>(walk, sampling, t - t0, word_of(t), val, key, 0u, out, member, rec, t0, n_lv, n_lf, n_fin, false, front);
            }
        }
    }
    unsigned long long v[3] = {n_lf, n_lv, n_fin};
    unsigned long long* const dst[3] = {&stats[0], &stats[1], n_done};
    block_add<3>(v, dst);
}

template <class Walk, class Sampling, typename pos_t, bool kWide>
SweepKernels bind_sweep(const typename Walk::View& iv, const uint64_t* d_l, const uint64_t* d_out_off, uint64_t n_pat, unsigned long long* d_stats,
                        hipStream_t stream, uint8_t* front)
{
    SweepKernels K;
    K.n = iv.n;
    K.sigma = (uint32_t)iv.sigma;
    K.front = front;
    K.first = [=](uint64_t t0, uint64_t t1, uint64_t* val, uint16_t* key, void* out, unsigned long long* counter, const Block* mem, uint64_t* rc, bool ahead,
                  uint32_t* chunk_list) {
        launch_sweep_chunk_lists(d_out_off, n_pat, t0, t1, chunk_list, stream);
        return on_trails_ahead(mem != nullptr, ahead, [&](auto tr, auto ah) {
            return launch(sweep_first_kernel<Walk, Sampling, pos_t, decltype(tr)::value, kWide, decltype(ah)::value>, launch_grid((t1 - t0 + 7) / 8, 8192), stream, iv,
                          d_l, d_out_off, n_pat, t0, t1, val, key, static_cast<pos_t*>(out), d_stats, counter, mem, rc, chunk_list, front);
        });
    };
    K.step = [=](uint64_t* val, uint16_t* key, uint64_t alive, uint32_t step, void* out, unsigned long long* counter, const Block* mem, uint64_t* rc, uint64_t t0, bool probed) {
        return on_flag(mem != nullptr, [&](auto tr) {
            return launch(sweep_step_kernel<Walk, Sampling, pos_t, decltype(tr)::value, kWide>, launch_grid(alive, 4096), stream, iv, val, key, alive, step,
                          static_cast<pos_t*>(out), d_stats, counter, mem, rc, t0, probed);
        });
    };
    K.tail = [=](void* out, uint64_t alive, uint32_t per_wave, const uint64_t* val, uint32_t step, uint64_t* rc, uint64_t t0, const Block* mem, uint32_t blocks) {
        return launch(locate_kernel<Walk, Sampling, pos_t, true, kWide>, dim3(blocks), stream, iv, static_cast<pos_t*>(out), alive, per_wave, d_stats, val, step, rc, t0, mem);
    };
    return K;
}

template <class Copy>
vlg_status sweep_dense_copy(LaunchTimer* timer, const std::function<vlg_status()>* while_first_step, const Copy& copy)
{
    if (timer) timer->begin(0);
    const vlg_status s = copy();
    if (timer) timer->end(0);
    if (s) return s;
    return while_first_step ? (*while_first_step)() : VLG_OK;
}

}
```

### vlg_matching_amd/variants.py

```python
import os
import subprocess
from concurrent.futures import ThreadPoolExecutor

_HERE = os.path.dirname(os.path.abspath(__file__))
ROOT = os.path.dirname(_HERE)
CSRC = os.path.join(_HERE, "csrc")

DEFAULTS = {
    "VLG_LINK_RUN": 2048, "VLG_COOP_WINDOWS2": 4, "VLG_RUNG_SHIFT": 2, "VLG_RESOLVE_HOPS": 4096, "VLG_RESOLVE_CHUNK": 4096,
    "VLG_GROUP_CHUNK": 2048, "VLG_STAGE_LISTS": 1, "VLG_SWEEP_PAIRS": 1, "VLG_PIVOT_GROUPS": 2, "VLG_PIVOT_TURNS": 1,
    "VLG_COMPACT_RUNS": 16, "VLG_SPARSE_TURN": 8, "VLG_SORT_CLASSES": 5, "VLG_BUCKET_SORT": 1, "VLG_WINDOW_SORT": 1,
    "VLG_WINDOWS_PER_TILE": 2, "VLG_WINDOW_RANK_LOOP": 0, "VLG_WINDOW_THREADS": 256, "VLG_WINDOW_ITEMS": 12, "VLG_FETCH_THREADS": 16,
    "VLG_DOCLIST_RUN": 2048,
}

VARIANTS = {
    "small": {"VLG_LINK_RUN": 192, "VLG_RESOLVE_CHUNK": 256, "VLG_GROUP_CHUNK": 256, "VLG_RESOLVE_HOPS": 2, "VLG_COMPACT_RUNS": 1,
              "VLG_SPARSE_TURN": 1, "VLG_PIVOT_GROUPS": 1, "VLG_COOP_WINDOWS2": 1, "VLG_DOCLIST_RUN": 192},
    "alternates": {"VLG_SORT_CLASSES": 3, "VLG_SWEEP_PAIRS": 0, "VLG_STAGE_LISTS": 0, "VLG_WINDOW_RANK_LOOP": 1, "VLG_WINDOWS_PER_TILE": 4,
                   "VLG_PIVOT_TURNS": 4, "VLG_RUNG_SHIFT": 4},
    "radix": {"VLG_BUCKET_SORT": 0, "VLG_RUNG_SHIFT": 3},
}

ENV_RUNS = {
    "env_paths": {"VLG_RESOLVE_GROUPED": "0", "VLG_SWEEP_LOOKAHEAD": "0", "VLG_NO_SPECULATIVE_COMPACT": "1", "VLG_WINDOW_SORT": "0",
                  "VLG_FUSE_JUMP": "0"},
}


def constants(name):
    c = dict(DEFAULTS)
    if name is not None:
        c.update(VARIANTS[name])
    return c


def extra_defs(name):
    return " ".join("-D%s=%d" % kv for kv in sorted(VARIANTS[name].items()))


def library(name):
    return os.path.join(ROOT, "build", "variants", name, "libvlg_hip.so")


def build(name, jobs=4):
    subprocess.check_call(["make", "-C", CSRC, "-j%d" % jobs, "variant", "VARIANT=" + name, "EXTRA_DEFS=" + extra_defs(name)],
                          stdout=subprocess.DEVNULL)


def build_all(jobs=None):
    jobs = jobs or max(1, min(8, (os.cpu_count() or 4) // len(VARIANTS)))
    with ThreadPoolExecutor(len(VARIANTS)) as ex:
        for f in [ex.submit(build, n, jobs) for n in VARIANTS]:
            f.result()
```

Baseline: 801,800.

## Compact finished elements in the first sweep step to shrink the following radix sort

The first sweep kernel gains a compacting mode. Workgroups draw turns from a ticket counter and commit each turn's survivors in order, so finished elements are dropped before the partition sort. The first full-width radix sort is skipped, and only the surviving count is then sorted with one fewer key bit. This costs a larger control-word memset, ticket-based ordering between workgroups, and a new stall check.

```diff
diff --git a/vlg_matching_amd/csrc/int_index.hpp b/vlg_matching_amd/csrc/int_index.hpp
--- a/vlg_matching_amd/csrc/int_index.hpp
+++ b/vlg_matching_amd/csrc/int_index.hpp
@@ -512,7 +512,7 @@
 vlg_status launch_int_locate_sweep(const IntView& v, const uint64_t* d_l, const uint64_t* d_out_off, uint64_t n_pat, uint64_t total, uint32_t* d_out,
                                    uint64_t* val_a, uint64_t* val_b, uint16_t* key_a, uint16_t* key_b, void* temp, size_t temp_bytes, unsigned long long* d_counter,
                                    unsigned long long* d_stats, uint64_t tail_threshold, hipStream_t stream, LaunchTimer* timer, Block* member,
-                                   uint32_t n_member_lists, uint64_t* rec, const std::function<vlg_status()>* while_first_step)
+                                   uint32_t n_member_lists, uint64_t* rec, const std::function<vlg_status()>* while_first_step, SweepCompaction compaction)
 {
     const bool text_order = shape(v).text_order;
     if (v.dens == 1 && !text_order && total)
@@ -521,7 +521,7 @@
     return on_bv(v.bv_kind, [&](auto bv) { return on_flag(text_order, [&](auto to) {
         const SweepKernels K = bind_sweep<IntWalk<tag_t<decltype(bv)>>, IntSampling<decltype(to)::value>, uint32_t, false>(v, d_l, d_out_off, n_pat, d_stats, stream, nullptr);
         return run_locate_sweep<uint32_t, false>(K, d_l, d_out_off, n_pat, total, d_out, val_a, val_b, key_a, key_b, temp, temp_bytes, d_counter, tail_threshold, stream, timer,
-                                                 member, n_member_lists, rec, while_first_step);
+                                                 member, n_member_lists, rec, while_first_step, compaction);
     }); });
 }
 
diff --git a/vlg_matching_amd/csrc/kernels.hip b/vlg_matching_amd/csrc/kernels.hip
--- a/vlg_matching_amd/csrc/kernels.hip
+++ b/vlg_matching_amd/csrc/kernels.hip
@@ -1001,7 +1001,8 @@
                             hipStream_t stream, LaunchTimer* timer, Block* member ,
                             uint32_t n_member_lists ,
                             uint64_t* rec ,
-                            const std::function<vlg_status()>* while_first_step )
+                            const std::function<vlg_status()>* while_first_step ,
+                            SweepCompaction compaction)
 {
     bool hook_due = while_first_step != nullptr;
     constexpr uint32_t kShift = kWide ? 33 : 32;
@@ -1009,6 +1010,8 @@
     if (sizeof(pos_t) == 4 && K.n > (1ull << 32) + 1) return fail(VLG_E_INTERNAL, "sorted sweep: positions do not fit 32 bits");
     if (K.sigma >= 0xFFFFu) return fail(VLG_E_INTERNAL, "sorted sweep: alphabet too large for the 16-bit partition key");
     const unsigned bits = bit_width64(K.sigma);
+    const unsigned live_bits = std::max(1u, bit_width64(K.sigma ? K.sigma - 1 : 0));
+    unsigned long long* const h_done = compaction.h_done;
     const uint64_t batch_max = sweep_batch_max<kWide>();
     if (member) {
         if (total > 0xFFFFFF00ull) return fail(VLG_E_INTERNAL, "member bit-vector: slots need 32 bits");
@@ -1035,26 +1038,36 @@
         uint32_t step = 0;
         pos_t* out = d_out + t0;
         while (alive > tail_threshold && step < 0xFFFFFFu) {
-            VLG_HIP_TRY(hipMemsetAsync(d_counter, 0, 8, stream));
+            const bool first = fused_first && step == 0;
+            const bool compact = first && h_done != nullptr;
+            VLG_HIP_TRY(hipMemsetAsync(d_counter, 0, compact ? sweep_control_words(alive) * 8 : 8, stream));
             if (timer) timer->begin(0);
-            const vlg_status ks = fused_first && step == 0 ? K.first(t0, t1, val_a, key_a, out, d_counter, member, rec, ahead, reinterpret_cast<uint32_t*>(val_b))
-                                                           : K.step(val_a, key_a, alive, step, out, d_counter, member, rec, t0, ahead && fused_first && step == 1);
+            const vlg_status ks = first ? K.first(t0, t1, val_a, key_a, out, d_counter, member, rec, ahead, reinterpret_cast<uint32_t*>(val_b), compact)
+                                        : K.step(val_a, key_a, alive, step, out, d_counter, member, rec, t0, ahead && fused_first && step == 1);
             if (timer) timer->end(0);
             if (ks) return ks;
-            size_t tb = temp_bytes;
-            if (timer) timer->begin(1, 20ull * alive);
-            rocprim::double_buffer<uint16_t> dk(key_a, key_b);
-            rocprim::double_buffer<uint64_t> dv(val_a, val_b);
-            hipError_t se = rocprim::radix_sort_pairs(temp, tb, dk, dv, alive, 0, bits, stream);
-            if (timer) timer->end(1);
-            VLG_HIP_TRY(se);
-            unsigned long long done = 0;
-            VLG_HIP_TRY(hipMemcpyAsync(&done, d_counter, 8, hipMemcpyDeviceToHost, stream));
+            const auto partition = [&](uint64_t count, unsigned key_bits) -> vlg_status {
+                size_t tb = temp_bytes;
+                if (timer) timer->begin(1, 20ull * count);
+                rocprim::double_buffer<uint16_t> dk(key_a, key_b);
+                rocprim::double_buffer<uint64_t> dv(val_a, val_b);
+                hipError_t se = rocprim::radix_sort_pairs(temp, tb, dk, dv, count, 0, key_bits, stream);
+                if (timer) timer->end(1);
+                VLG_HIP_TRY(se);
+                key_a = dk.current(); key_b = dk.alternate();
+                val_a = dv.current(); val_b = dv.alternate();
+                return VLG_OK;
+            };
+            if (!compact) if (vlg_status ps = partition(alive, bits)) return ps;
+            unsigned long long done_here[2] = {0, 0};
+            unsigned long long* done = compact ? h_done : done_here;
+            VLG_HIP_TRY(hipMemcpyAsync(done, d_counter, compact ? 16 : 8, hipMemcpyDeviceToHost, stream));
             if (hook_due) { hook_due = false; if (vlg_status hs = (*while_first_step)()) return hs; }
             VLG_HIP_TRY(hipStreamSynchronize(stream));
-            key_a = dk.current(); key_b = dk.alternate();
-            val_a = dv.current(); val_b = dv.alternate();
-            alive -= done;
+            if (compact && done[kSweepStalled]) return fail(VLG_E_INTERNAL, "sweep compaction stalled");
+            if (done[kSweepDone] > alive) return fail(VLG_E_INTERNAL, "locate sweep: more elements finished than were walking");
+            alive -= done[kSweepDone];
+            if (compact && alive > tail_threshold) if (vlg_status ps = partition(alive, live_bits)) return ps;
             ++step;
             if (step > 1u << 20) return fail(VLG_E_INTERNAL, "locate sweep did not converge");
         }
@@ -1097,14 +1110,14 @@
 }
 template vlg_status run_locate_sweep<uint32_t, false>(const SweepKernels&, const uint64_t*, const uint64_t*, uint64_t, uint64_t, uint32_t*, uint64_t*, uint64_t*,
                                                       uint16_t*, uint16_t*, void*, size_t, unsigned long long*, uint64_t, hipStream_t, LaunchTimer*, Block*,
-                                                      uint32_t, uint64_t*, const std::function<vlg_status()>*);
+                                                      uint32_t, uint64_t*, const std::function<vlg_status()>*, SweepCompaction);
 
 template <typename pos_t, bool kWide>
 vlg_status launch_locate_sweep(const IndexView& iv, const uint64_t* d_l, const uint64_t* d_out_off, uint64_t n_pat, uint64_t total,
                                pos_t* d_out, uint64_t* val_a, uint64_t* val_b, uint16_t* key_a, uint16_t* key_b, void* temp,
                                size_t temp_bytes, unsigned long long* d_counter, unsigned long long* d_stats, uint64_t tail_threshold,
                                hipStream_t stream, LaunchTimer* timer, Block* member, uint32_t n_member_lists, uint64_t* rec,
-                               const std::function<vlg_status()>* while_first_step, uint8_t* front)
+                               const std::function<vlg_status()>* while_first_step, uint8_t* front, SweepCompaction compaction)
 {
     if (iv.sample_bytes != (kWide ? 8u : 4u)) return fail(VLG_E_INTERNAL, "sorted sweep: sample width does not match the instantiation");
     const bool text_order = shape(iv).text_order;
@@ -1119,7 +1132,7 @@
         const SweepKernels K = bind_sweep<tag_t<decltype(walk)>, ByteSampling<kWide, decltype(to)::value>, pos_t, kWide>(iv, d_l, d_out_off, n_pat, d_stats, stream,
                                                                                                                    rec ? front : nullptr);
         return run_locate_sweep<pos_t, kWide>(K, d_l, d_out_off, n_pat, total, d_out, val_a, val_b, key_a, key_b, temp, temp_bytes, d_counter, tail_threshold, stream, timer,
-                                              member, n_member_lists, rec, while_first_step);
+                                              member, n_member_lists, rec, while_first_step, compaction);
     }); });
 }
 constexpr uint32_t kUnsampleSync = 4;
@@ -1209,7 +1222,7 @@
     template vlg_status launch_locate_sweep<P, W>(const IndexView&, const uint64_t*, const uint64_t*, uint64_t, uint64_t, P*, uint64_t*, \
                                                   uint64_t*, uint16_t*, uint16_t*, void*, size_t, unsigned long long*, unsigned long long*, \
                                                   uint64_t, hipStream_t, LaunchTimer*, Block*, uint32_t, uint64_t*,                       \
-                                                  const std::function<vlg_status()>*, uint8_t*);
+                                                  const std::function<vlg_status()>*, uint8_t*, SweepCompaction);
 VLG_SWEEP_INST(uint32_t, false)
 VLG_SWEEP_INST(uint32_t, true)
 VLG_SWEEP_INST(uint64_t, true)
@@ -1232,7 +1245,7 @@
 
 KernelConstants kernel_constants()
 {
-    return KernelConstants{VLG_RESOLVE_HOPS, VLG_RESOLVE_CHUNK, VLG_GROUP_CHUNK, VLG_STAGE_LISTS, VLG_SWEEP_PAIRS};
+    return KernelConstants{VLG_RESOLVE_HOPS, VLG_RESOLVE_CHUNK, VLG_GROUP_CHUNK, VLG_STAGE_LISTS, VLG_SWEEP_PAIRS, VLG_SWEEP_CHUNK};
 }
 
 }
diff --git a/vlg_matching_amd/csrc/kernels.hpp b/vlg_matching_amd/csrc/kernels.hpp
--- a/vlg_matching_amd/csrc/kernels.hpp
+++ b/vlg_matching_amd/csrc/kernels.hpp
@@ -17,7 +17,7 @@
 template <typename pos_t>
 vlg_status launch_locate(const IndexView& iv, pos_t* d_io, uint64_t total, unsigned long long* d_stats, hipStream_t stream);
 
-struct KernelConstants { int64_t resolve_hops, resolve_chunk, group_chunk, stage_lists, sweep_pairs; };
+struct KernelConstants { int64_t resolve_hops, resolve_chunk, group_chunk, stage_lists, sweep_pairs, sweep_chunk; };
 KernelConstants kernel_constants();
 
 struct LaunchTimer {
@@ -36,6 +36,18 @@
 }
 
 size_t sweep_temp_bytes(uint64_t total, uint32_t sigma, hipStream_t stream);
+#ifndef VLG_SWEEP_CHUNK
+#define VLG_SWEEP_CHUNK 2048
+#endif
+constexpr uint32_t kSweepChunk = VLG_SWEEP_CHUNK;
+static_assert(kSweepChunk >= 256 && kSweepChunk % 256 == 0, "VLG_SWEEP_CHUNK: whole rows of the 256-thread workgroup");
+static_assert(kSweepChunk <= 4096, "VLG_SWEEP_CHUNK: one wave scans a turn's (row, wave) survivor counts, 64 at most");
+constexpr uint32_t kSweepDone = 0, kSweepStalled = 1, kSweepTicket = 2, kSweepStatus = 4;
+inline uint64_t sweep_turns(uint64_t elements) { return (elements + kSweepChunk - 1) / kSweepChunk; }
+inline uint64_t sweep_control_words(uint64_t elements) { return kSweepStatus + ((sweep_turns(elements) + 1) & ~1ull); }
+struct SweepCompaction {
+    unsigned long long* h_done = nullptr;
+};
 template <bool kWide> constexpr uint64_t sweep_batch_max() { return kWide ? (1ull << 31) : 0xFFFFFF00ull; }
 template <typename pos_t, bool kWide>
 vlg_status launch_locate_sweep(const IndexView& iv, const uint64_t* d_l, const uint64_t* d_out_off, uint64_t n_pat, uint64_t total,
@@ -43,15 +55,15 @@
                                size_t temp_bytes, unsigned long long* d_counter, unsigned long long* d_stats, uint64_t tail_threshold,
                                hipStream_t stream, LaunchTimer* timer, Block* member, uint32_t n_member_lists, uint64_t* rec,
                                const std::function<vlg_status()>* while_first_step = nullptr,
-                               uint8_t* front = nullptr );
-constexpr uint32_t kSweepChunk = 2048;
+                               uint8_t* front = nullptr ,
+                               SweepCompaction compaction = SweepCompaction());
 void launch_sweep_chunk_lists(const uint64_t* d_out_off, uint64_t n_pat, uint64_t t0, uint64_t t1, uint32_t* chunk_list, hipStream_t stream);
 struct SweepKernels {
     uint8_t* front = nullptr;
     uint64_t n = 0;
     uint32_t sigma = 0;
     std::function<vlg_status(uint64_t t0, uint64_t t1, uint64_t* val, uint16_t* key, void* out, unsigned long long* n_done, const Block* member, uint64_t* rec, bool ahead,
-                       uint32_t* chunk_list )> first;
+                       uint32_t* chunk_list , bool compact)> first;
     std::function<vlg_status(uint64_t* val, uint16_t* key, uint64_t alive, uint32_t step, void* out, unsigned long long* n_done, const Block* member, uint64_t* rec, uint64_t t0,
                        bool probed)> step;
     std::function<vlg_status(void* out, uint64_t alive, uint32_t per_wave, const uint64_t* val, uint32_t step, uint64_t* rec_or_null, uint64_t t0, const Block* member,
@@ -61,7 +73,8 @@
 vlg_status run_locate_sweep(const SweepKernels& K, const uint64_t* d_l, const uint64_t* d_out_off, uint64_t n_pat, uint64_t total,
                             pos_t* d_out, uint64_t* val_a, uint64_t* val_b, uint16_t* key_a, uint16_t* key_b, void* temp,
                             size_t temp_bytes, unsigned long long* d_counter, uint64_t tail_threshold, hipStream_t stream, LaunchTimer* timer,
-                            Block* member, uint32_t n_member_lists, uint64_t* rec, const std::function<vlg_status()>* while_first_step = nullptr);
+                            Block* member, uint32_t n_member_lists, uint64_t* rec, const std::function<vlg_status()>* while_first_step = nullptr,
+                            SweepCompaction compaction = SweepCompaction());
 inline uint64_t member_blocks(uint64_t n) { return n / kBlockBits + 1; }
 template <bool kWide>
 vlg_status launch_unsample(const IndexView& iv, const uint64_t* d_l, const uint64_t* d_out_off, uint64_t n_pat, uint64_t total, uint32_t* d_out,
@@ -77,7 +90,8 @@
 vlg_status launch_int_locate_sweep(const IntView& v, const uint64_t* d_l, const uint64_t* d_out_off, uint64_t n_pat, uint64_t total, uint32_t* d_out,
                                    uint64_t* val_a, uint64_t* val_b, uint16_t* key_a, uint16_t* key_b, void* temp, size_t temp_bytes, unsigned long long* d_counter,
                                    unsigned long long* d_stats, uint64_t tail_threshold, hipStream_t stream, LaunchTimer* timer, Block* member,
-                                   uint32_t n_member_lists, uint64_t* rec, const std::function<vlg_status()>* while_first_step = nullptr);
+                                   uint32_t n_member_lists, uint64_t* rec, const std::function<vlg_status()>* while_first_step = nullptr,
+                                   SweepCompaction compaction = SweepCompaction());
 vlg_status launch_sa_dense_copy(const uint32_t* sa, const uint64_t* d_l, const uint64_t* d_out_off, uint64_t n_pat, uint64_t total, uint32_t* d_out,
                                 hipStream_t stream);
 vlg_status launch_int_dense_copy(const IntView& v, const uint64_t* d_l, const uint64_t* d_out_off, uint64_t n_pat, uint64_t total, uint32_t* d_out, hipStream_t stream);
diff --git a/vlg_matching_amd/csrc/search.hip b/vlg_matching_amd/csrc/search.hip
--- a/vlg_matching_amd/csrc/search.hip
+++ b/vlg_matching_amd/csrc/search.hip
@@ -50,6 +50,7 @@
     uint64_t global_sort_min = 1ull << 20;
     bool quad_walk = true;
     bool fuse_jump = true;
+    bool sweep_compact = true;
     uint64_t sweep_min = 1ull << 22;
     uint64_t sweep_tail = 1ull << 22;
     uint32_t unsample_pct = 0;
@@ -227,6 +228,7 @@
     if (!strcmp(name, "quad_walk")) { ws->quad_walk = value != 0; return VLG_OK; }
     if (!strcmp(name, "tuples")) { ws->tuples = value != 0; return VLG_OK; }
     if (!strcmp(name, "fuse_jump")) { ws->fuse_jump = value != 0; return VLG_OK; }
+    if (!strcmp(name, "sweep_compact")) { ws->sweep_compact = value != 0; return VLG_OK; }
     if (!strcmp(name, "filter")) { ws->filter = value != 0; return VLG_OK; }
     if (!strcmp(name, "filter_min")) { ws->filter_min = (uint64_t)value; return VLG_OK; }
     if (!strcmp(name, "filter_pivot")) { ws->filter_pivot = value != 0; return VLG_OK; }
@@ -894,6 +896,8 @@
         c = choose_physical<pos_t>(idx, ws, acc, nd, wide, acc, gacc, &cp.c);
     }
 
+    uint64_t sweep_cap() const { return std::min<uint64_t>(acc, wide ? sweep_batch_max<true>() : sweep_batch_max<false>()); }
+
     vlg_status carve()
     {
         Pg = A.take<pos_t>(gacc);
@@ -903,7 +907,7 @@
         d_off64 = A.take<uint64_t>(nd + 1);
         d_off32 = A.take<uint32_t>(nd + 1);
         d_lh = A.take<uint64_t>(nd);
-        d_counter = A.take<unsigned long long>(4);
+        d_counter = A.take<unsigned long long>(std::max<uint64_t>(4, c.sweep && ws->sweep_compact ? sweep_control_words(sweep_cap()) : 0));
         d_tmp = A.take<uint8_t>(cp.sort_tmp + 256);
         if (A.failed) return fail(VLG_E_INTERNAL, "arena carve failed (physical)");
         Pb = reinterpret_cast<pos_t*>(scratch);
@@ -953,7 +957,9 @@
             }
             if (!s) bt.mark("  physical: unsampling");
         } else if (c.sweep) {
-            const uint64_t cap = std::min<uint64_t>(acc, wide ? sweep_batch_max<true>() : sweep_batch_max<false>());
+            const uint64_t cap = sweep_cap();
+            svec<unsigned long long> h_round(2, 0);
+            const SweepCompaction compaction{ws->sweep_compact ? h_round.data() : nullptr};
             uint64_t* val_a = reinterpret_cast<uint64_t*>(scratch);
             uint64_t* val_b = val_a + cap;
             uint16_t* key_a = reinterpret_cast<uint16_t*>(val_b + cap);
@@ -964,14 +970,14 @@
             if (idx->is_int) {
                 if constexpr (sizeof(pos_t) == 4)
                     s = launch_int_locate_sweep(idx->iview, d_lh, d_off64, nd, acc, Pa, val_a, val_b, key_a, key_b, d_tmp, cp.sort_tmp, d_counter, d_stats, ws->sweep_tail, st,
-                                                &timer, member, n_member_lists, rec, &hook);
+                                                &timer, member, n_member_lists, rec, &hook, compaction);
                 else s = fail(VLG_E_INTERNAL, "integer-alphabet index with 64-bit positions");
             } else if (wide)
                 s = launch_locate_sweep<pos_t, true>(lview, d_lh, d_off64, nd, acc, Pa, val_a, val_b, key_a, key_b, d_tmp, cp.sort_tmp, d_counter, d_stats,
-                                                     ws->sweep_tail, st, &timer, member, n_member_lists, rec, &hook, front);
+                                                     ws->sweep_tail, st, &timer, member, n_member_lists, rec, &hook, front, compaction);
             else if constexpr (sizeof(pos_t) == 4)
                 s = launch_locate_sweep<uint32_t, false>(lview, d_lh, d_off64, nd, acc, Pa, val_a, val_b, key_a, key_b, d_tmp, cp.sort_tmp, d_counter, d_stats,
-                                                         ws->sweep_tail, st, &timer, member, n_member_lists, rec, &hook, front);
+                                                         ws->sweep_tail, st, &timer, member, n_member_lists, rec, &hook, front, compaction);
             else s = fail(VLG_E_INTERNAL, "64-bit positions with 32-bit SA indices");
             if (!s) bt.mark("  physical: sweep");
         } else if (idx->is_int) {
@@ -1759,7 +1765,8 @@
     uint64_t trail_bytes = cp.c.share_steps ? member_blocks(idx->hdr.n) * sizeof(Block) + phys * 9 + 2048 : 0;
     cp.want_rungs = pivot_elems && (ws->pivot_rungs == 2 || (pivot_elems >= phys / 16 && pivot_elems >= 4096));
     const uint64_t rung_bytes = cp.want_rungs ? rung_layout(phys).entries * sizeof(pos_t) + 8192 : 0;
-    const uint64_t phys_plain = phys * (sizeof(pos_t) + kPhysScratchPerElem<pos_t>()) + cp.sort_tmp + (dlist.size() + 2) * 24 + (8ull << 20) + phys + rung_bytes;
+    const uint64_t sweep_ctl = cp.c.sweep && ws->sweep_compact ? sweep_control_words(phys) * 8 + 256 : 0;
+    const uint64_t phys_plain = phys * (sizeof(pos_t) + kPhysScratchPerElem<pos_t>()) + sweep_ctl + cp.sort_tmp + (dlist.size() + 2) * 24 + (8ull << 20) + phys + rung_bytes;
     if (trail_bytes) {
         const uint64_t left = budget > phys_plain + trail_bytes ? budget - phys_plain - trail_bytes : 0;
         if (left < std::max<uint64_t>(2 * logical_max_query, budget / 8)) trail_bytes = 0;
@@ -2459,7 +2466,7 @@
     const vlg::KernelConstants kc = vlg::kernel_constants();
     const struct { const char* name; int64_t value; } all[] = {
         {"VLG_LINK_RUN", VLG_LINK_RUN}, {"VLG_COOP_WINDOWS2", VLG_COOP_WINDOWS2}, {"VLG_RUNG_SHIFT", VLG_RUNG_SHIFT},
-        {"VLG_RESOLVE_HOPS", kc.resolve_hops}, {"VLG_RESOLVE_CHUNK", kc.resolve_chunk}, {"VLG_GROUP_CHUNK", kc.group_chunk},
+        {"VLG_RESOLVE_HOPS", kc.resolve_hops}, {"VLG_RESOLVE_CHUNK", kc.resolve_chunk}, {"VLG_GROUP_CHUNK", kc.group_chunk}, {"VLG_SWEEP_CHUNK", kc.sweep_chunk},
         {"VLG_STAGE_LISTS", kc.stage_lists}, {"VLG_SWEEP_PAIRS", kc.sweep_pairs},
         {"VLG_PIVOT_GROUPS", VLG_PIVOT_GROUPS}, {"VLG_PIVOT_TURNS", VLG_PIVOT_TURNS}, {"VLG_COMPACT_RUNS", VLG_COMPACT_RUNS},
         {"VLG_SPARSE_TURN", VLG_SPARSE_TURN}, {"VLG_SORT_CLASSES", VLG_SORT_CLASSES}, {"VLG_BUCKET_SORT", VLG_BUCKET_SORT},
diff --git a/vlg_matching_amd/csrc/sweep_kernels.hpp b/vlg_matching_amd/csrc/sweep_kernels.hpp
--- a/vlg_matching_amd/csrc/sweep_kernels.hpp
+++ b/vlg_matching_amd/csrc/sweep_kernels.hpp
@@ -135,9 +135,146 @@
     return ls.off[kListStage] >= end;
 }
 
-template <class Walk, class Sampling, typename pos_t, bool kTrail, bool kWide, bool kFirst = false, bool kAhead = false>
+struct ArraySink {
+    uint64_t* __restrict__ val;
+    uint16_t* __restrict__ key;
+    uint16_t sigma;
+    __device__ __forceinline__ void emit(uint64_t e, uint64_t word, uint32_t c) const { val[e] = word; key[e] = (uint16_t)c; }
+    __device__ __forceinline__ void finish(uint64_t e) const { key[e] = sigma; }
+};
+
+constexpr uint32_t kNoKey = 0xFFFF;
+constexpr uint32_t kSweepRows = kSweepChunk / 256;
+constexpr uint32_t kTurnSpins = 1u << 21;
+struct TurnShared {
+    uint16_t key[kSweepChunk];
+    uint32_t cnt[kSweepRows * 4];
+    uint64_t base;
+    uint32_t turn, stalled;
+};
+template <bool kHigh>
+struct TurnRegs {
+    TurnShared& st;
+    uint32_t low[kSweepRows];
+    uint32_t high[kHigh ? kSweepRows : 1];
+    __device__ __forceinline__ void emit(uint64_t row, uint64_t word, uint32_t c)
+    {
+#pragma unroll
+        for (uint32_t r = 0; r < kSweepRows; ++r) {
+            low[r] = row == r ? (uint32_t)word : low[r];
+            if (kHigh) high[r] = row == r ? (uint32_t)(word >> 32) : high[r];
+        }
+        st.key[row * 256 + threadIdx.x] = (uint16_t)c;
+    }
+    __device__ __forceinline__ void finish(uint64_t row) { st.key[row * 256 + threadIdx.x] = (uint16_t)kNoKey; }
+    __device__ __forceinline__ uint32_t key_of(uint32_t r) const { return st.key[r * 256 + threadIdx.x]; }
+};
+using gu64 = __attribute__((address_space(1))) unsigned long long;
+__device__ __forceinline__ void status_store(unsigned long long* p, unsigned long long x)
+{
+    __hip_atomic_store((gu64*)p, x, __ATOMIC_RELAXED, __HIP_MEMORY_SCOPE_AGENT);
+}
+__device__ __forceinline__ unsigned long long status_load(unsigned long long* p)
+{
+    return __hip_atomic_load((gu64*)p, __ATOMIC_RELAXED, __HIP_MEMORY_SCOPE_AGENT);
+}
+
+__device__ __forceinline__ uint32_t draw_turn(TurnShared& st, unsigned long long* ctl)
+{
+    __syncthreads();
+    if (threadIdx.x == 0) st.turn = (uint32_t)atomicAdd(&ctl[kSweepTicket], 1ull);
+    __syncthreads();
+    return __builtin_amdgcn_readfirstlane(st.turn);
+}
+
+template <bool kHigh>
+__device__ __forceinline__ bool commit_turn(const TurnRegs<kHigh>& regs, TurnShared& st, unsigned long long* ctl, uint32_t turn, uint64_t first_slot,
+                                            uint64_t* __restrict__ val, uint16_t* __restrict__ key)
+{
+    constexpr unsigned long long kValue = (1ull << 62) - 1;
+    const uint32_t lane = threadIdx.x & 63, wave = threadIdx.x >> 6;
+#pragma unroll
+    for (uint32_t r = 0; r < kSweepRows; ++r) {
+        const unsigned long long m = __ballot(regs.key_of(r) != kNoKey);
+        if (lane == 0) st.cnt[r * 4 + wave] = (uint32_t)__popcll(m);
+    }
+    __syncthreads();
+    const uint32_t mine = lane < kSweepRows * 4 ? st.cnt[lane] : 0u;
+    uint32_t incl = mine;
+#pragma unroll
+    for (uint32_t o = 1; o < 64; o <<= 1) {
+        const uint32_t y = __shfl_up(incl, o);
+        if (lane >= o) incl += y;
+    }
+    const uint32_t total = __shfl(incl, 63);
+    const uint32_t excl = incl - mine;
+    if (wave == 0) {
+        unsigned long long* status = ctl + kSweepStatus;
+        if (lane == 0) status_store(&status[turn], ((turn ? 1ull : 2ull) << 62) | total);
+        unsigned long long before = 0;
+        bool stalled = false;
+        if (turn) {
+            long long hi = (long long)turn - 1;
+            uint32_t spins = 0;
+            for (;;) {
+                const long long j = hi - (long long)lane;
+                const unsigned long long w = j >= 0 ? status_load(&status[j]) : (2ull << 62);
+                const uint32_t tag = (uint32_t)(w >> 62);
+                const unsigned long long ready = __ballot(tag != 0), prefixed = __ballot(tag == 2);
+                unsigned long long need = ~0ull;
+                if (prefixed) {
+                    const uint32_t f = (uint32_t)__ffsll((long long)prefixed) - 1;
+                    need = f == 63 ? ~0ull : (1ull << (f + 1)) - 1;
+                    if ((ready & need) == need) {
+                        unsigned long long x = lane <= f ? (w & kValue) : 0ull;
+                        for (int o = 32; o > 0; o >>= 1) x += __shfl_xor(x, o);
+                        before += x;
+                        break;
+                    }
+                } else if (ready == ~0ull) {
+                    unsigned long long x = w & kValue;
+                    for (int o = 32; o > 0; o >>= 1) x += __shfl_xor(x, o);
+                    before += x;
+                    hi -= 64;
+                    spins = 0;
+                    continue;
+                }
+                const long long late = hi - (long long)((uint32_t)__ffsll((long long)(~ready & need)) - 1);
+                while ((status_load(&status[late]) >> 62) == 0) {
+                    if (++spins > kTurnSpins) { stalled = true; break; }
+                    __builtin_amdgcn_s_sleep(16);
+                }
+                if (stalled) break;
+            }
+            if (lane == 0) {
+                if (stalled) status_store(&ctl[kSweepStalled], 1ull);
+                else status_store(&status[turn], (2ull << 62) | (before + total));
+            }
+        }
+        if (lane == 0) { st.base = before; st.stalled = stalled ? 1u : 0u; }
+    }
+    __syncthreads();
+    if (__builtin_amdgcn_readfirstlane(st.stalled)) return false;
+    const uint64_t base = ((uint64_t)__builtin_amdgcn_readfirstlane((uint32_t)(st.base >> 32)) << 32) | __builtin_amdgcn_readfirstlane((uint32_t)st.base);
+#pragma unroll
+    for (uint32_t r = 0; r < kSweepRows; ++r) {
+        const uint32_t k = regs.key_of(r);
+        const unsigned long long m = __ballot(k != kNoKey);
+        const uint32_t pre = __shfl(excl, r * 4 + wave);
+        if (k != kNoKey) {
+            const uint64_t to = base + pre + (uint32_t)__popcll(m & ((1ull << lane) - 1ull));
+            const uint64_t high = kHigh ? (uint64_t)regs.high[kHigh ? r : 0] : first_slot + r * 256 + threadIdx.x;
+            val[to] = (high << 32) | regs.low[r];
+            key[to] = (uint16_t)k;
+        }
+        __builtin_amdgcn_sched_barrier(0);
+    }
+    return true;
+}
+
+template <class Walk, class Sampling, typename pos_t, bool kTrail, bool kWide, bool kFirst = false, bool kAhead = false, class Sink = ArraySink>
 __device__ __forceinline__ void sweep_element(const Walk& walk, const Sampling& sampling, uint64_t e, uint64_t v64,
-                                              uint64_t* __restrict__ val, uint16_t* __restrict__ key, uint32_t step, pos_t* __restrict__ out,
+                                              Sink& sink, uint32_t step, pos_t* __restrict__ out,
                                               const Block* __restrict__ member, uint64_t* __restrict__ rec, uint64_t slot0,
                                               uint32_t& n_lv, uint32_t& n_lf, uint32_t& n_fin, bool probed = false, uint8_t* __restrict__ front = nullptr)
 {
@@ -152,11 +289,11 @@
         if (r >= walk.n()) r -= walk.n();
         if (kTrail) rec[slot0 + (v64 >> kShift)] = r;
         else out[v64 >> kShift] = (pos_t)r;
-        key[e] = (uint16_t)walk.sigma();
+        sink.finish(e);
         ++n_fin;
     } else if (kTrail && !kFirst && !probed && member_probe(member, i, owner)) {
         rec[slot0 + (v64 >> kShift)] = follow_owner<kShift>(rec, owner, step);
-        key[e] = (uint16_t)walk.sigma();
+        sink.finish(e);
         ++n_fin;
     } else {
         if (kTrail && kFirst) rec[slot0 + (v64 >> kShift)] = ~0ull;
@@ -165,12 +302,11 @@
         ++n_lf;
         if (kTrail && kAhead && member_probe(member, j, owner)) {
             rec[slot0 + (v64 >> kShift)] = ((uint64_t)(step + 1) << kShift) | owner;
-            key[e] = (uint16_t)walk.sigma();
+            sink.finish(e);
             ++n_fin;
             in_front = (uint8_t)c;
         } else {
-            val[e] = (v64 & ~kPosMask) | j;
-            key[e] = (uint16_t)c;
+            sink.emit(e, (v64 & ~kPosMask) | j, c);
         }
     }
     if (kTrail && kFirst && front) front[slot0 + (v64 >> kShift)] = in_front;
@@ -193,16 +329,17 @@
     const Walk walk{iv, s};
     const Sampling sampling(iv);
     uint32_t n_lv = 0, n_lf = 0, n_fin = 0;
+    ArraySink sink{val, key, (uint16_t)walk.sigma()};
     for (uint64_t e = (uint64_t)blockIdx.x * blockDim.x + threadIdx.x; e < count; e += (uint64_t)gridDim.x * blockDim.x)
-        sweep_element<Walk, Sampling, pos_t, kTrail, kWide>(walk, sampling, e, val[e], val, key, step, out, member, rec, slot0, n_lv, n_lf, n_fin, probed);
+        sweep_element<Walk, Sampling, pos_t, kTrail, kWide>(walk, sampling, e, val[e], sink, step, out, member, rec, slot0, n_lv, n_lf, n_fin, probed);
     unsigned long long v[3] = {n_lf, n_lv, n_fin};
     unsigned long long* const dst[3] = {&stats[0], &stats[1], n_done};
     block_add<3>(v, dst);
 }
 
-template <typename pos_t, bool kTrail, bool kWide, bool kAhead, class Sampling>
+template <typename pos_t, bool kTrail, bool kWide, bool kAhead, class Sampling, class Sink>
 __device__ __forceinline__ void sweep_first_pair(const IndexView& iv, const WalkLds<PlainBV>& s, const Sampling& sampling, bool onA, uint64_t eA, uint64_t wA,
-                                                 bool onB, uint64_t eB, uint64_t wB, uint64_t* __restrict__ val, uint16_t* __restrict__ key,
+                                                 bool onB, uint64_t eB, uint64_t wB, Sink& sink,
                                                  pos_t* __restrict__ out, const Block* __restrict__ member, uint64_t* __restrict__ rec, uint64_t slot0,
                                                  uint32_t& n_lv, uint32_t& n_lf, uint32_t& n_fin, uint8_t* __restrict__ front)
 {
@@ -214,11 +351,11 @@
     uint64_t sv = 0;
     if (onA && sampling.probe(iA, sv)) {
         if (kTrail) rec[slot0 + (wA >> kShift)] = sv; else out[wA >> kShift] = (pos_t)sv;
-        key[eA] = (uint16_t)iv.sigma; ++n_fin; onA = false;
+        sink.finish(eA); ++n_fin; onA = false;
     }
     if (onB && sampling.probe(iB, sv)) {
         if (kTrail) rec[slot0 + (wB >> kShift)] = sv; else out[wB >> kShift] = (pos_t)sv;
-        key[eB] = (uint16_t)iv.sigma; ++n_fin; onB = false;
+        sink.finish(eB); ++n_fin; onB = false;
     }
     if (kTrail) {
         if (onA) rec[slot0 + (wA >> kShift)] = ~0ull;
@@ -267,12 +404,12 @@
         if (onB) { ownB = block_rank_bit(rB, offB, bit); stopB = bit != 0; }
     }
     if (onA) {
-        if (stopA) { rec[slot0 + (wA >> kShift)] = (1ull << kShift) | ownA; key[eA] = (uint16_t)iv.sigma; ++n_fin; }
-        else { val[eA] = (wA & ~kPosMask) | jA; key[eA] = (uint16_t)cA; }
+        if (stopA) { rec[slot0 + (wA >> kShift)] = (1ull << kShift) | ownA; sink.finish(eA); ++n_fin; }
+        else sink.emit(eA, (wA & ~kPosMask) | jA, cA);
     }
     if (onB) {
-        if (stopB) { rec[slot0 + (wB >> kShift)] = (1ull << kShift) | ownB; key[eB] = (uint16_t)iv.sigma; ++n_fin; }
-        else { val[eB] = (wB & ~kPosMask) | jB; key[eB] = (uint16_t)cB; }
+        if (stopB) { rec[slot0 + (wB >> kShift)] = (1ull << kShift) | ownB; sink.finish(eB); ++n_fin; }
+        else sink.emit(eB, (wB & ~kPosMask) | jB, cB);
     }
     if (kTrail && front) {
         if (hadA) front[slot0 + (wA >> kShift)] = (onA && stopA) ? (uint8_t)cA : (uint8_t)0xFF;
@@ -280,7 +417,7 @@
     }
 }
 
-template <class Walk, class Sampling, typename pos_t, bool kTrail, bool kWide, bool kAhead>
+template <class Walk, class Sampling, typename pos_t, bool kTrail, bool kWide, bool kAhead, bool kCompact>
 __global__ void __launch_bounds__(256) sweep_first_kernel(typename Walk::View iv, const uint64_t* __restrict__ l, const uint64_t* __restrict__ out_off, uint64_t n_pat,
                                                           uint64_t t0, uint64_t total, uint64_t* __restrict__ val, uint16_t* __restrict__ key,
                                                           pos_t* __restrict__ out, unsigned long long* __restrict__ stats,
@@ -294,10 +431,9 @@
     const Walk walk{iv, s};
     const Sampling sampling(iv);
     constexpr uint32_t kShift = kWide ? 33 : 32;
-    constexpr uint32_t kPer = kSweepChunk / 256;
+    constexpr uint32_t kPer = kSweepRows;
     uint32_t n_lv = 0, n_lf = 0, n_fin = 0;
-    for (uint64_t base = t0 + (uint64_t)blockIdx.x * kSweepChunk; base < total; base += (uint64_t)gridDim.x * kSweepChunk) {
-        __syncthreads();
+    auto take_turn = [&](uint64_t base, auto& sink, auto place) {
         uint64_t p = chunk_list[(base - t0) / kSweepChunk];
         const uint64_t end = base + 256 * kPer < total ? base + 256 * kPer : total;
         const bool staged = kStage && stage_lists(s_lists, out_off, l, n_pat, p, end);
@@ -314,21 +450,40 @@
             return ((t - t0) << kShift) | sai;
         };
         if constexpr (Walk::kPlainTree && kSweepPairs && kWide) {
-            static_assert(kPer % 2 == 0, "elements are taken in pairs");
+            static_assert(kPer % 2 == 0, "VLG_SWEEP_CHUNK: elements are taken in pairs of rows");
 #pragma unroll 1
             for (uint32_t i = 0; i < kPer; i += 2) {
                 const uint64_t tA = base + i * 256 + threadIdx.x, tB = tA + 256;
                 const bool onA = tA < total, onB = tB < total;
                 const uint64_t wA = onA ? word_of(tA) : 0, wB = onB ? word_of(tB) : 0;
-                sweep_first_pair<pos_t, kTrail, kWide, kAhead>(iv, s, sampling, onA, tA - t0, wA, onB, tB - t0, wB, val, key, out, member, rec, t0, n_lv, n_lf, n_fin, front);
+                if (kCompact) { if (!onA) sink.finish(place(tA, i)); if (!onB) sink.finish(place(tB, i + 1)); }
+                sweep_first_pair<pos_t, kTrail, kWide, kAhead>(iv, s, sampling, onA, place(tA, i), wA, onB, place(tB, i + 1), wB, sink, out, member, rec, t0, n_lv, n_lf, n_fin, front);
             }
         } else {
 #pragma unroll 1
             for (uint32_t i = 0; i < kPer; ++i) {
                 const uint64_t t = base + i * 256 + threadIdx.x;
                 if (t < total)
-                    sweep_element<Walk, Sampling, pos_t, kTrail, kWide, true, kAhead>(walk, sampling, t - t0, word_of(t), val, key, 0u, out, member, rec, t0, n_lv, n_lf, n_fin, false, front);
-            }
+                    sweep_element<Walk, Sampling, pos_t, kTrail, kWide, true, kAhead>(walk, sampling, place(t, i), word_of(t), sink, 0u, out, member, rec, t0, n_lv, n_lf, n_fin, false, front);
+                else if (kCompact) sink.finish(place(t, i));
+            }
+        }
+    };
+    if constexpr (kCompact) {
+        __shared__ TurnShared st;
+        TurnRegs<kWide> regs{st, {}, {}};
+        const uint64_t turns = (total - t0 + kSweepChunk - 1) / kSweepChunk;
+        for (;;) {
+            const uint32_t turn = draw_turn(st, n_done);
+            if (turn >= turns) break;
+            take_turn(t0 + (uint64_t)turn * kSweepChunk, regs, [](uint64_t, uint32_t row) -> uint64_t { return row; });
+            if (!commit_turn(regs, st, n_done, turn, (uint64_t)turn * kSweepChunk, val, key)) return;
+        }
+    } else {
+        ArraySink sink{val, key, (uint16_t)walk.sigma()};
+        for (uint64_t base = t0 + (uint64_t)blockIdx.x * kSweepChunk; base < total; base += (uint64_t)gridDim.x * kSweepChunk) {
+            __syncthreads();
+            take_turn(base, sink, [t0](uint64_t t, uint32_t) -> uint64_t { return t - t0; });
         }
     }
     unsigned long long v[3] = {n_lf, n_lv, n_fin};
@@ -345,12 +500,13 @@
     K.sigma = (uint32_t)iv.sigma;
     K.front = front;
     K.first = [=](uint64_t t0, uint64_t t1, uint64_t* val, uint16_t* key, void* out, unsigned long long* counter, const Block* mem, uint64_t* rc, bool ahead,
-                  uint32_t* chunk_list) {
+                  uint32_t* chunk_list, bool compact) {
         launch_sweep_chunk_lists(d_out_off, n_pat, t0, t1, chunk_list, stream);
-        return on_trails_ahead(mem != nullptr, ahead, [&](auto tr, auto ah) {
-            return launch(sweep_first_kernel<Walk, Sampling, pos_t, decltype(tr)::value, kWide, decltype(ah)::value>, launch_grid((t1 - t0 + 7) / 8, 8192), stream, iv,
+        const dim3 grid((uint32_t)std::max<uint64_t>(1, std::min<uint64_t>(sweep_turns(t1 - t0), 8192)));
+        return on_trails_ahead(mem != nullptr, ahead, [&](auto tr, auto ah) { return on_flag(compact, [&](auto cm) {
+            return launch(sweep_first_kernel<Walk, Sampling, pos_t, decltype(tr)::value, kWide, decltype(ah)::value, decltype(cm)::value>, grid, stream, iv,
                           d_l, d_out_off, n_pat, t0, t1, val, key, static_cast<pos_t*>(out), d_stats, counter, mem, rc, chunk_list, front);
-        });
+        }); });
     };
     K.step = [=](uint64_t* val, uint16_t* key, uint64_t alive, uint32_t step, void* out, unsigned long long* counter, const Block* mem, uint64_t* rc, uint64_t t0, bool probed) {
         return on_flag(mem != nullptr, [&](auto tr) {
diff --git a/vlg_matching_amd/variants.py b/vlg_matching_amd/variants.py
--- a/vlg_matching_amd/variants.py
+++ b/vlg_matching_amd/variants.py
@@ -11,12 +11,12 @@
     "VLG_GROUP_CHUNK": 2048, "VLG_STAGE_LISTS": 1, "VLG_SWEEP_PAIRS": 1, "VLG_PIVOT_GROUPS": 2, "VLG_PIVOT_TURNS": 1,
     "VLG_COMPACT_RUNS": 16, "VLG_SPARSE_TURN": 8, "VLG_SORT_CLASSES": 5, "VLG_BUCKET_SORT": 1, "VLG_WINDOW_SORT": 1,
     "VLG_WINDOWS_PER_TILE": 2, "VLG_WINDOW_RANK_LOOP": 0, "VLG_WINDOW_THREADS": 256, "VLG_WINDOW_ITEMS": 12, "VLG_FETCH_THREADS": 16,
-    "VLG_DOCLIST_RUN": 2048,
+    "VLG_DOCLIST_RUN": 2048, "VLG_SWEEP_CHUNK": 2048,
 }
 
 VARIANTS = {
     "small": {"VLG_LINK_RUN": 192, "VLG_RESOLVE_CHUNK": 256, "VLG_GROUP_CHUNK": 256, "VLG_RESOLVE_HOPS": 2, "VLG_COMPACT_RUNS": 1,
-              "VLG_SPARSE_TURN": 1, "VLG_PIVOT_GROUPS": 1, "VLG_COOP_WINDOWS2": 1, "VLG_DOCLIST_RUN": 192},
+              "VLG_SPARSE_TURN": 1, "VLG_PIVOT_GROUPS": 1, "VLG_COOP_WINDOWS2": 1, "VLG_DOCLIST_RUN": 192, "VLG_SWEEP_CHUNK": 512},
     "alternates": {"VLG_SORT_CLASSES": 3, "VLG_SWEEP_PAIRS": 0, "VLG_STAGE_LISTS": 0, "VLG_WINDOW_RANK_LOOP": 1, "VLG_WINDOWS_PER_TILE": 4,
                    "VLG_PIVOT_TURNS": 4, "VLG_RUNG_SHIFT": 4},
     "radix": {"VLG_BUCKET_SORT": 0, "VLG_RUNG_SHIFT": 3},
```

After: 820,800, median of 6. 1.02x the previous value.
